# HKUDS/GPT-ST

Hardware: AMD Instinct MI355X
Metric: pretrain steps/sec at (B=32,T=12,N=170,C=64) (higher is better)
Workload: dtype f32; 1 GPU; BASELINE configs[1]: PEMS08-shape synthetic pretrain step, per-GPU B=32 T=12 N=170 C=64 base=1, epoch 200/300 (adaptive mask + KL), fwd+loss+bwd+clip+Adam, hipGraph=True, 4 full optimiser steps on 4 different resident batches per graph replay; global_batch=32, parallelism=dp1

## Files before the change

gpt-st_amd/csrc/abi.hip:

```cpp
#include "common.h"
#include "gptst_hip.h"

extern "C" int gptst_abi_version(void) { return GPTST_ABI_VERSION; }

thread_local int g_deterministic = 0;
extern "C" int gptst_set_deterministic(int on) { g_deterministic = on ? 1 : 0; return GPTST_OK; }
extern "C" int gptst_deterministic_state(void) { return g_deterministic; }

GPTST_INTERNAL int gptst_handoff_lost_capmfma(unsigned* out);
GPTST_INTERNAL int gptst_handoff_lost_hypertem(unsigned* out);
GPTST_INTERNAL int gptst_handoff_lost_masksel(unsigned* out);
extern "C" int gptst_handoff_timeouts(int* out) {
    if (!out) return GPTST_EARG;
    unsigned a = 0u, b = 0u, c = 0u;
    if (gptst_handoff_lost_capmfma(&a) || gptst_handoff_lost_hypertem(&b) || gptst_handoff_lost_masksel(&c)) return -5;
    *out = (int)(a + b + c);
    return GPTST_OK;
}

GPTST_INTERNAL int gptst_handoff_clear_capmfma(unsigned to);
GPTST_INTERNAL int gptst_handoff_clear_hypertem(unsigned to);
GPTST_INTERNAL int gptst_handoff_clear_masksel(unsigned to);
GPTST_INTERNAL int gptst_adam_skipped_clear(void);
extern "C" int gptst_handoff_reset(void) {
    if (hipDeviceSynchronize() != hipSuccess) return -5;
    return (gptst_handoff_clear_capmfma(0u) || gptst_handoff_clear_hypertem(0u) || gptst_handoff_clear_masksel(0u) || gptst_adam_skipped_clear()) ? -5 : GPTST_OK;
}
extern "C" int gptst_handoff_inject(int n) {
    if (n < 0) return GPTST_EARG;
    if (hipDeviceSynchronize() != hipSuccess) return -5;
    return gptst_handoff_clear_capmfma((unsigned)n) ? -5 : GPTST_OK;
}
```

gpt-st_amd/csrc/apply.hip:

```cpp
#include "mfma_tile.h"
#include "wgrad64.h"
#include "kl_guest.h"
#ifdef GPTST_DEBUG
__device__ long long g_ap_ts[64];
static thread_local int g_ap_dbg = 0;
extern "C" int gptst_ap_dbg(int v) { g_ap_dbg = v; return 0; }
extern "C" int gptst_ap_ts(long long* out) { return (int)hipMemcpyFromSymbol(out, HIP_SYMBOL(g_ap_ts), sizeof(long long) * 64); }
#else
static constexpr int g_ap_dbg = 0;
#endif
thread_local int g_apply_tpw = 0;
thread_local int g_apply128_minwg = 768;
thread_local int g_apply128_v1 = 0;

template <int C, int PRO, int EPI>
__global__ __launch_bounds__(256) void apply_kernel(const float* __restrict__ A, const float* __restrict__ A2,
                                                    const float* __restrict__ W, long w_gstride, int transw,
                                                    const float* __restrict__ bias, const float* __restrict__ resid,
                                                    const float* __restrict__ resid2, float* __restrict__ out, float* __restrict__ colsum, RowMap rm, int dbg) {
    using T = Tile<C>;
    int tsi = 0;
#ifdef GPTST_DEBUG
#define TS() do { if (dbg && blockIdx.x == 100 && blockIdx.y == 0 && threadIdx.x == 0) g_ap_ts[tsi] = clock64(); ++tsi; } while (0)
#else
#define TS() do { } while (0)
#endif
    TS();
    extern __shared__ __attribute__((aligned(16))) float smem[];
    float* Wl = smem;
    const int tid = threadIdx.x, lane = tid & 63, wave = tid >> 6;
    float* tile = smem + C * C + wave * T::TILE_FLOATS;
    const int g = blockIdx.x;
    const int ntiles = (rm.M + 31) / 32;
    float cs[C / 64];
#pragma unroll
    for (int u = 0; u < C / 64; ++u) cs[u] = 0.f;
    const int tstride = gridDim.y * 4;
    int t = blockIdx.y * 4 + wave;

    float4 av[T::F4_PER_LANE], ov[T::F4_PER_LANE];
    auto fetch_a = [&](int tt) {
        const int m0 = tt * 32;
#pragma unroll
        for (int it = 0; it < T::F4_PER_LANE; ++it) {
            const int f = it * 64 + lane;
            const int r = f / T::F4_PER_ROW, c4 = f % T::F4_PER_ROW;
            av[it] = f4zero(); ov[it] = make_float4(1.f, 1.f, 1.f, 1.f);
            if (tt < ntiles && m0 + r < rm.M) {
                const size_t off = ((size_t)g * rm.rs_g + (size_t)(m0 + r) * rm.rs_m) * C + 4 * c4;
                av[it] = ld4(A + off);
                if (PRO == PRO_DPRE) ov[it] = ld4(A2 + off);
            }
        }
    };
    fetch_a(t);
    TS();
    load_w_lds<C, 256>(Wl, W + (size_t)g * w_gstride, transw, tid);
    __syncthreads();
    TS();

    for (; t < ntiles; t += tstride) {
        const int m0 = t * 32;
#pragma unroll
        for (int it = 0; it < T::F4_PER_LANE; ++it) {
            const int f = it * 64 + lane;
            const int r = f / T::F4_PER_ROW, c4 = f % T::F4_PER_ROW;
            float4 v = av[it];
            if (PRO == PRO_DPRE) {
                const float4 o = ov[it];
                v.x *= lrelu_grad_from_out(o.x); v.y *= lrelu_grad_from_out(o.y);
                v.z *= lrelu_grad_from_out(o.z); v.w *= lrelu_grad_from_out(o.w);
            }
            st4(tile + r * T::PITCH + 4 * c4, v);
        }
        float4 rv[T::F4_PER_LANE], rv2[T::F4_PER_LANE];
#pragma unroll
        for (int it = 0; it < T::F4_PER_LANE; ++it) {
            const int f = it * 64 + lane;
            const int r = f / T::F4_PER_ROW, c4 = f % T::F4_PER_ROW;
            rv[it] = f4zero(); rv2[it] = f4zero();
            if ((EPI == EPI_RES_LRELU || EPI == EPI_ADD_DPRE) && m0 + r < rm.M) {
                const size_t off = ((size_t)g * rm.rs_g + (size_t)(m0 + r) * rm.rs_m) * C + 4 * c4;
                rv[it] = ld4(resid + off);
                if (EPI == EPI_ADD_DPRE) rv2[it] = ld4(resid2 + off);
            }
        }
        TS();
        if (colsum != nullptr) {
#pragma unroll
            for (int u = 0; u < C / 64; ++u) {
                float s = 0.f;
#pragma unroll 8
                for (int r = 0; r < 32; ++r) s += tile[r * T::PITCH + u * 64 + lane];
                cs[u] += s;
            }
        }
        f32x16 acc[T::NCT];
        TS();
        mfma_tile<C>(tile, Wl, acc, lane);
        TS();
        acc_to_tile<C>(tile, acc, lane);
        TS();
        if (t + tstride < ntiles) fetch_a(t + tstride);
#pragma unroll
        for (int it = 0; it < T::F4_PER_LANE; ++it) {
            const int f = it * 64 + lane;
            const int r = f / T::F4_PER_ROW, c4 = f % T::F4_PER_ROW;
            if (m0 + r < rm.M) {
                const size_t off = ((size_t)g * rm.rs_g + (size_t)(m0 + r) * rm.rs_m) * C + 4 * c4;
                float4 y = ld4(tile + r * T::PITCH + 4 * c4);
                if (bias != nullptr) y = f4add(y, ld4(bias + (size_t)g * C + 4 * c4));
                if (EPI == EPI_RES_LRELU) {
                    y = f4add(y, rv[it]);
                    y.x = lrelu(y.x); y.y = lrelu(y.y); y.z = lrelu(y.z); y.w = lrelu(y.w);
                }
                if (EPI == EPI_LRELU) { y.x = lrelu(y.x); y.y = lrelu(y.y); y.z = lrelu(y.z); y.w = lrelu(y.w); }
                if (EPI == EPI_ADD_DPRE) {
                    const float4 d = rv[it], o = rv2[it];
                    y.x = fmaf(d.x, lrelu_grad_from_out(o.x), y.x); y.y = fmaf(d.y, lrelu_grad_from_out(o.y), y.y);
                    y.z = fmaf(d.z, lrelu_grad_from_out(o.z), y.z); y.w = fmaf(d.w, lrelu_grad_from_out(o.w), y.w);
                }
                st4(out + off, y);
            }
        }
        TS();
    }
    if (colsum != nullptr) {
        __syncthreads();
#pragma unroll
        for (int u = 0; u < C / 64; ++u) tile[u * 64 + lane] = cs[u];
        __syncthreads();
        if (wave == 0) {
#pragma unroll
            for (int u = 0; u < C / 64; ++u) {
                float s = 0.f;
#pragma unroll
                for (int w = 0; w < 4; ++w) s += smem[C * C + w * T::TILE_FLOATS + u * 64 + lane];
                colsum[((size_t)blockIdx.y * rm.G + g) * C + u * 64 + lane] = s;
            }
        }
    }
}

template <int PRO, int EPI>
__global__ __launch_bounds__(256, 2) void apply64_kernel(const float* __restrict__ A, const float* __restrict__ A2,
                                                         const float* __restrict__ W, long w_gstride, int transw,
                                                         const float* __restrict__ bias, const float* __restrict__ resid,
                                                         const float* __restrict__ resid2, float* __restrict__ out,
                                                         float* __restrict__ colsum, RowMap rm, int tiles_per_wave) {
    constexpr int C = 64;
    __shared__ __attribute__((aligned(16))) float Wl[C * C];
    __shared__ __attribute__((aligned(16))) float csl[4][C];
    const int lane = threadIdx.x & 63, wave = threadIdx.x >> 6;
    const int j = lane & 15, kk = lane >> 4;
    const int g = blockIdx.x;
    const int ntiles = (rm.M + 15) / 16;
    const int t0 = (blockIdx.y * 4 + wave) * tiles_per_wave, t1 = min(ntiles, t0 + tiles_per_wave);
    const float* Wg = W + (size_t)g * w_gstride;
    float4 bias4 = f4zero();
    if (bias != nullptr) bias4 = ld4(bias + (size_t)g * C + 4 * j);
    float4 cs[4];
#pragma unroll
    for (int q = 0; q < 4; ++q) cs[q] = f4zero();
    float4 an[4], on[4];
    auto fetch = [&](int t) {
        const int m = min(t * 16 + j, rm.M - 1);
        const size_t off = ((size_t)g * rm.rs_g + (size_t)m * rm.rs_m) * C + 4 * kk;
#pragma unroll
        for (int q = 0; q < 4; ++q) {
            an[q] = ld4(A + off + 16 * q);
            if (PRO == PRO_DPRE) on[q] = ld4(A2 + off + 16 * q);
        }
    };
    if (t0 < t1) fetch(t0);
    load_w_lds<C, 256>(Wl, Wg, transw, threadIdx.x);
    __syncthreads();
    float4 bv[4][4];
#pragma unroll
    for (int q = 0; q < 4; ++q)
#pragma unroll
        for (int e = 0; e < 4; ++e) bv[q][e] = ld4(Wl + (16 * q + 4 * kk + e) * C + 4 * j);
    for (int t = t0; t < t1; ++t) {
        float4 a[4];
        const bool rowok = t * 16 + j < rm.M;
#pragma unroll
        for (int q = 0; q < 4; ++q) {
            float4 v = an[q];
            if (PRO == PRO_DPRE) {
                v.x *= lrelu_grad_from_out(on[q].x); v.y *= lrelu_grad_from_out(on[q].y);
                v.z *= lrelu_grad_from_out(on[q].z); v.w *= lrelu_grad_from_out(on[q].w);
            }
            if (!rowok) v = f4zero();
            a[q] = v;
            cs[q] = f4add(cs[q], v);
        }
        float4 rv[4], rv2[4];
        size_t orow[4];
#pragma unroll
        for (int r = 0; r < 4; ++r) {
            const int m = min(t * 16 + kk * 4 + r, rm.M - 1);
            orow[r] = ((size_t)g * rm.rs_g + (size_t)m * rm.rs_m) * C + 4 * j;
            if (EPI == EPI_RES_LRELU || EPI == EPI_ADD_DPRE) rv[r] = ld4(resid + orow[r]);
            if (EPI == EPI_ADD_DPRE) rv2[r] = ld4(resid2 + orow[r]);
        }
        if (t + 1 < t1) fetch(t + 1);
        SB();
        f32x4 acc[4];
#pragma unroll
        for (int ct = 0; ct < 4; ++ct) acc[ct] = (f32x4){0.f, 0.f, 0.f, 0.f};
#pragma unroll
        for (int q = 0; q < 4; ++q) {
            const float av[4] = {a[q].x, a[q].y, a[q].z, a[q].w};
#pragma unroll
            for (int e = 0; e < 4; ++e) {
                acc[0] = __builtin_amdgcn_mfma_f32_16x16x4f32(av[e], bv[q][e].x, acc[0], 0, 0, 0);
                acc[1] = __builtin_amdgcn_mfma_f32_16x16x4f32(av[e], bv[q][e].y, acc[1], 0, 0, 0);
                acc[2] = __builtin_amdgcn_mfma_f32_16x16x4f32(av[e], bv[q][e].z, acc[2], 0, 0, 0);
                acc[3] = __builtin_amdgcn_mfma_f32_16x16x4f32(av[e], bv[q][e].w, acc[3], 0, 0, 0);
            }
        }
        SB();
#pragma unroll
        for (int r = 0; r < 4; ++r) {
            if (t * 16 + kk * 4 + r < rm.M) {
                float4 y = f4add(make_float4(acc[0][r], acc[1][r], acc[2][r], acc[3][r]), bias4);
                if (EPI == EPI_RES_LRELU) {
                    y = f4add(y, rv[r]);
                    y.x = lrelu(y.x); y.y = lrelu(y.y); y.z = lrelu(y.z); y.w = lrelu(y.w);
                }
                if (EPI == EPI_LRELU) { y.x = lrelu(y.x); y.y = lrelu(y.y); y.z = lrelu(y.z); y.w = lrelu(y.w); }
                if (EPI == EPI_ADD_DPRE) {
                    const float4 d = rv[r], o = rv2[r];
                    y.x = fmaf(d.x, lrelu_grad_from_out(o.x), y.x); y.y = fmaf(d.y, lrelu_grad_from_out(o.y), y.y);
                    y.z = fmaf(d.z, lrelu_grad_from_out(o.z), y.z); y.w = fmaf(d.w, lrelu_grad_from_out(o.w), y.w);
                }
                st4(out + orow[r], y);
            }
        }
    }
    if (colsum != nullptr) {
#pragma unroll
        for (int q = 0; q < 4; ++q) {
            cs[q].x = group_sum<16>(cs[q].x); cs[q].y = group_sum<16>(cs[q].y);
            cs[q].z = group_sum<16>(cs[q].z); cs[q].w = group_sum<16>(cs[q].w);
            if (j == 0) st4(&csl[wave][16 * q + 4 * kk], cs[q]);
        }
        __syncthreads();
        if (wave == 0) colsum[((size_t)blockIdx.y * rm.G + g) * C + lane] = (csl[0][lane] + csl[1][lane]) + (csl[2][lane] + csl[3][lane]);
    }
}

static void apply64_geometry(const RowMap& rm, bool has_colsum, int& tpw, int& gy) {
    const int ntiles = (rm.M + 15) / 16;
    long tot = (long)rm.G * ntiles;
    tpw = (int)((tot + 4 * 512 - 1) / (4 * 512));
    if (tpw > 2) tpw = 2;
    if (has_colsum && rm.G == 1) { const int lim = (ntiles + 4 * 128 - 1) / (4 * 128); if (tpw < lim) tpw = lim; }
    if (g_apply_tpw > 0) tpw = g_apply_tpw;
    if (tpw < 1) tpw = 1;
    gy = (ntiles + 4 * tpw - 1) / (4 * tpw);
}

template <int PRO, int EPI>
static void launch_apply64_t(const float* A, const float* A2, const float* W, long gs, int transw, const float* bias, const float* resid,
                             const float* resid2, float* out, float* colsum, RowMap rm, hipStream_t st) {
    int tpw, gy;
    apply64_geometry(rm, colsum != nullptr, tpw, gy);
    hipLaunchKernelGGL((apply64_kernel<PRO, EPI>), dim3(rm.G, gy), dim3(256), 0, st, A, A2, W, gs, transw, bias, resid, resid2, out, colsum, rm, tpw);
}

static int launch_apply64(const float* A, const float* A2, const float* W, long gs, int transw, const float* bias, const float* resid,
                          const float* resid2, float* out, float* colsum, RowMap rm, int pro, int epi, hipStream_t st) {
    if (pro == PRO_NONE && epi == EPI_PLAIN) launch_apply64_t<PRO_NONE, EPI_PLAIN>(A, A2, W, gs, transw, bias, resid, resid2, out, colsum, rm, st);
    else if (pro == PRO_NONE && epi == EPI_RES_LRELU) launch_apply64_t<PRO_NONE, EPI_RES_LRELU>(A, A2, W, gs, transw, bias, resid, resid2, out, colsum, rm, st);
    else if (pro == PRO_DPRE && epi == EPI_PLAIN) launch_apply64_t<PRO_DPRE, EPI_PLAIN>(A, A2, W, gs, transw, bias, resid, resid2, out, colsum, rm, st);
    else if (pro == PRO_NONE && epi == EPI_ADD_DPRE) launch_apply64_t<PRO_NONE, EPI_ADD_DPRE>(A, A2, W, gs, transw, bias, resid, resid2, out, colsum, rm, st);
    else if (pro == PRO_NONE && epi == EPI_LRELU) launch_apply64_t<PRO_NONE, EPI_LRELU>(A, A2, W, gs, transw, bias, resid, resid2, out, colsum, rm, st);
    else return GPTST_EARG;
    GPTST_CHECK_LAUNCH();
    return GPTST_OK;
}

template <int PRO, int U>
__global__ __launch_bounds__(256, 2) void wgrad64_kernel(const float* __restrict__ A, const float* __restrict__ D,
                                                         const float* __restrict__ D2, float* __restrict__ dW, RowMap rm,
                                                         int rows_per_split, int ostride, int csa) {
    __shared__ __attribute__((aligned(16))) float smem[WGRAD64_SMEM_FLOATS];
    wgrad64_body<PRO, U>(A, D, D2, dW, rm, rows_per_split, ostride, csa, blockIdx.x, blockIdx.y, smem);
}

template <int KIND, int CHAIN>
__global__ __launch_bounds__(256, 2) void applywg64_kernel(const float* __restrict__ dOut, const float* __restrict__ Y,
                                                            const float* __restrict__ S, const float* __restrict__ W, long w_gstride,
                                                            const float* __restrict__ resid, const float* __restrict__ resid2,
                                                            float* __restrict__ dS, float* __restrict__ dW, float* __restrict__ colsum,
                                                            RowMap rm, int tiles_per_wave) {
    __shared__ __attribute__((aligned(16))) float lds[APPLYWG64_LDS_FLOATS];
    applywg64_body<KIND, CHAIN>(dOut, Y, S, W, w_gstride, resid, resid2, dS, dW, colsum, rm, tiles_per_wave, blockIdx.x, blockIdx.y, lds);
}

GPTST_INTERNAL int gptst_apply_wgrad_geometry(int mode, int BT, int N, int* tpw) {
    RowMap rm = make_rowmap(mode, BT, N);
    int gy;
    apply64_geometry(rm, false, *tpw, gy);
    return gy;
}

extern "C" int gptst_apply_wgrad_nsplit(int mode, int BT, int N) {
    RowMap rm = make_rowmap(mode, BT, N);
    int tpw, gy;
    apply64_geometry(rm, false, tpw, gy);
    return gy;
}

extern "C" int gptst_apply_wgrad(const float* dOut, const float* Y, const float* S, const float* W, float* dS, float* dW, float* colsum,
                                 int premul, int mode, int BT, int N, int C, void* stream) {
    if (!dOut || !S || !W || !dS || !dW || BT <= 0 || N <= 0 || mode < 0 || mode > 1 || (Y && premul)) return GPTST_EARG;
    if (C != 64) return GPTST_ESHAPE;
    RowMap rm = make_rowmap(mode, BT, N);
    int tpw, gy;
    apply64_geometry(rm, false, tpw, gy);
    const dim3 grid(rm.G, gy);
    hipStream_t st = (hipStream_t)stream;
    if (Y) hipLaunchKernelGGL((applywg64_kernel<0, 0>), grid, dim3(256), 0, st, dOut, Y, S, W, (long)C * C, nullptr, nullptr, dS, dW, colsum, rm, tpw);
    else if (!premul) hipLaunchKernelGGL((applywg64_kernel<0, 1>), grid, dim3(256), 0, st, dOut, Y, S, W, (long)C * C, nullptr, nullptr, dS, dW, colsum, rm, tpw);
    else hipLaunchKernelGGL((applywg64_kernel<0, 2>), grid, dim3(256), 0, st, dOut, Y, S, W, (long)C * C, nullptr, nullptr, dS, dW, colsum, rm, tpw);
    GPTST_CHECK_LAUNCH();
    return GPTST_OK;
}

extern "C" int gptst_linear_bwd_nsplit(int rows) {
    RowMap rm = make_rowmap(2, rows, 1);
    int tpw, gy;
    apply64_geometry(rm, false, tpw, gy);
    return gy;
}

extern "C" int gptst_linear_bwd(const float* dY, const float* X, const float* Wp, const float* dOut, const float* out, float* dX, float* dWp,
                                float* dbp, int premul, int rows, int C, void* stream) {
    if (!dY || !X || !Wp || !dOut || !dX || !dWp || !dbp || rows <= 0 || (out && premul)) return GPTST_EARG;
    if (C != 64) return GPTST_ESHAPE;
    RowMap rm = make_rowmap(2, rows, 1);
    int tpw, gy;
    apply64_geometry(rm, false, tpw, gy);
    hipStream_t st = (hipStream_t)stream;
    if (out) hipLaunchKernelGGL((applywg64_kernel<1, 0>), dim3(1, gy), dim3(256), 0, st, dY, nullptr, X, Wp, 0L, dOut, out, dX, dWp, dbp, rm, tpw);
    else if (!premul) hipLaunchKernelGGL((applywg64_kernel<1, 1>), dim3(1, gy), dim3(256), 0, st, dY, nullptr, X, Wp, 0L, dOut, nullptr, dX, dWp, dbp, rm, tpw);
    else hipLaunchKernelGGL((applywg64_kernel<1, 2>), dim3(1, gy), dim3(256), 0, st, dY, nullptr, X, Wp, 0L, dOut, X, dX, dWp, dbp, rm, tpw);
    GPTST_CHECK_LAUNCH();
    return GPTST_OK;
}

template <int C, int PRO>
__global__ __launch_bounds__(256) void wgrad_kernel(const float* __restrict__ A, const float* __restrict__ D,
                                                    const float* __restrict__ D2, float* __restrict__ dW,
                                                    RowMap rm, int rows_per_split) {
    constexpr int NCT = C / 32;
    constexpr int TPW = NCT * NCT / 4;
    const int lane = threadIdx.x & 63, wave = threadIdx.x >> 6;
    const int j = lane & 31, h = lane >> 5;
    const int g = blockIdx.x, sp = blockIdx.y;
    const int mbeg = sp * rows_per_split;
    const int mend = min(rm.M, mbeg + rows_per_split);
    const int it = (wave * TPW) / NCT;
    f32x16 acc[TPW];
#pragma unroll
    for (int u = 0; u < TPW; ++u)
#pragma unroll
        for (int r = 0; r < 16; ++r) acc[u][r] = 0.f;

    for (int m = mbeg + h; m < mend + h; m += 2) {
        float a = 0.f;
        float d[TPW];
#pragma unroll
        for (int u = 0; u < TPW; ++u) d[u] = 0.f;
        if (m < mend) {
            const size_t off = ((size_t)g * rm.rs_g + (size_t)m * rm.rs_m) * C;
            a = A[off + it * 32 + j];
#pragma unroll
            for (int u = 0; u < TPW; ++u) {
                const int jt = (wave * TPW + u) % NCT;
                float dv = D[off + jt * 32 + j];
                if (PRO == PRO_DPRE) dv *= lrelu_grad_from_out(D2[off + jt * 32 + j]);
                d[u] = dv;
            }
        }
#pragma unroll
        for (int u = 0; u < TPW; ++u) acc[u] = __builtin_amdgcn_mfma_f32_32x32x2f32(a, d[u], acc[u], 0, 0, 0);
    }
    float* o = dW + ((size_t)sp * rm.G + g) * C * C;
#pragma unroll
    for (int u = 0; u < TPW; ++u) {
        const int jt = (wave * TPW + u) % NCT;
#pragma unroll
        for (int r = 0; r < 16; ++r) {
            const int row = (r & 3) + 8 * (r >> 2) + 4 * h;
            o[(size_t)(it * 32 + row) * C + jt * 32 + j] = acc[u][r];
        }
    }
}

#define AP128_NW 8
// ... 375 lines not shown
```

gpt-st_amd/csrc/hypertem.hip:

```cpp
#include "mfma_tile.h"
#include "wgrad64.h"
#include "kl_guest.h"
GPTST_STAMP_TABLES(hypertem)
GPTST_HANDOFF_COUNTER(hypertem)

#define HT_T 12
#ifndef HT_OCC
#define HT_OCC 2
#endif
#ifdef GPTST_DEBUG
__device__ long long g_ht_ts[64];
static thread_local int g_ht_dbg = 0, g_ht_nt_override = 0;
extern "C" int gptst_ht_dbg(int v) { g_ht_dbg = v; return 0; }
extern "C" int gptst_ht_variant(int fwd, int bwd) { g_ht_nt_override = fwd; (void)bwd; return 0; }
extern "C" int gptst_ht_ts(long long* out) { return (int)hipMemcpyFromSymbol(out, HIP_SYMBOL(g_ht_ts), sizeof(long long) * 64); }
#define HT_DBG(d) (d)
#else
#define HT_DBG(d) 0
static constexpr int g_ht_dbg = 0, g_ht_nt_override = 0;
#endif

__device__ __forceinline__ bool ht_work_at(int L, int ntiles, int B, int& b, int& tile) {
    const int xcd = L & 7, slot = L >> 3;
    b = xcd + 8 * (slot / ntiles);
    tile = slot % ntiles;
    return b < B;
}
__device__ __forceinline__ bool ht_work(int ntiles, int B, int& b, int& tile) { return ht_work_at(blockIdx.x, ntiles, B, b, tile); }

static int ht_pick_nt(int B, int N) {
    if (g_ht_nt_override >= 4 && g_ht_nt_override <= 16) return g_ht_nt_override;
    (void)B; (void)N;
    return 16;
}

__global__ __launch_bounds__(256, HT_OCC) void hypertem_fwd_kernel(const float* __restrict__ X, const float* __restrict__ G,
                                                              const float* __restrict__ Wbt, const float* __restrict__ bbt,
                                                              float* __restrict__ R_out, float* __restrict__ out, int N, int B, int NT,
                                                              int dbg) {
    constexpr int C = 64, P = C + 4, GP = 145;
    int tsi = 0;
#ifdef GPTST_DEBUG
#define TS() do { if ((dbg & 1) && blockIdx.x == 59 && threadIdx.x == 0) g_ht_ts[tsi] = clock64(); ++tsi; } while (0)
#else
#define TS() __builtin_amdgcn_sched_barrier(0)
#endif
    TS();
    extern __shared__ __attribute__((aligned(16))) float smem[];
    float* Xs = smem;
    float* Gs = Xs + HT_T * NT * P;
    int b, tile;
    if (!ht_work((N + NT - 1) / NT, B, b, tile)) return;
    const int n0 = tile * NT;
    const int tid = threadIdx.x, lane = tid & 63, wave = tid >> 6;
    {
        const int nl = tid >> 4, c4 = tid & 15;
        const int n = min(n0 + nl, N - 1);
        float4 v[HT_T];
        float gv[9];
#pragma unroll
        for (int t = 0; t < HT_T; ++t) v[t] = ld4(X + (((size_t)b * HT_T + t) * N + n) * C + 4 * c4);
#pragma unroll
        for (int k = 0; k < 9; ++k) gv[k] = G[min(n0 * 144 + tid + k * 256, N * 144 - 1)];
        if (nl < NT) {
#pragma unroll
            for (int t = 0; t < HT_T; ++t) st4(Xs + (t * NT + nl) * P + 4 * c4, n0 + nl < N ? v[t] : f4zero());
        }
#pragma unroll
        for (int k = 0; k < 9; ++k) {
            const int i = tid + k * 256;
            if (i < NT * 144) Gs[(i / 144) * GP + i % 144] = (n0 + i / 144 < N) ? gv[k] : 0.f;
        }
    }
    __syncthreads();
    TS();
    const int j = lane & 15, kk = lane >> 4;
    const int ja = j < NT ? j : 0;
    float4 bv[C / 16][4];
    float4 b4;
#define HT_LOAD_W(tt) do {                                                                                         \
        const float* W_ = Wbt + ((size_t)b * HT_T + (tt)) * C * C;                                                 \
        _Pragma("unroll") for (int q = 0; q < C / 16; ++q)                                                         \
            _Pragma("unroll") for (int e = 0; e < 4; ++e) bv[q][e] = ld4(W_ + (size_t)(16 * q + 4 * kk + e) * C + 4 * j); \
        b4 = ld4(bbt + ((size_t)b * HT_T + (tt)) * C + 4 * j);                                                     \
    } while (0)
    HT_LOAD_W(wave);
    for (int t = wave; t < HT_T; t += 4) {
        const size_t g = (size_t)b * HT_T + t;
        TS();
        float4 a4[C / 16];
#pragma unroll
        for (int q = 0; q < C / 16; ++q) a4[q] = f4zero();
        {
            const float* gr = Gs + ja * GP + t * HT_T;
            const float* xr = Xs + ja * P + 4 * kk;
#pragma unroll
            for (int u = 0; u < HT_T; ++u) {
                const float gu = gr[u];
#pragma unroll
                for (int q = 0; q < C / 16; ++q) a4[q] = f4fma(gu, ld4(xr + u * NT * P + 16 * q), a4[q]);
            }
        }
        TS();
        f32x4 acc[C / 16];
#pragma unroll
        for (int ct = 0; ct < C / 16; ++ct) acc[ct] = (f32x4){0.f, 0.f, 0.f, 0.f};
#pragma unroll
        for (int q = 0; q < C / 16; ++q) {
            const float av[4] = {a4[q].x, a4[q].y, a4[q].z, a4[q].w};
#pragma unroll
            for (int e = 0; e < 4; ++e) {
                acc[0] = __builtin_amdgcn_mfma_f32_16x16x4f32(av[e], bv[q][e].x, acc[0], 0, 0, 0);
                acc[1] = __builtin_amdgcn_mfma_f32_16x16x4f32(av[e], bv[q][e].y, acc[1], 0, 0, 0);
                acc[2] = __builtin_amdgcn_mfma_f32_16x16x4f32(av[e], bv[q][e].z, acc[2], 0, 0, 0);
                acc[3] = __builtin_amdgcn_mfma_f32_16x16x4f32(av[e], bv[q][e].w, acc[3], 0, 0, 0);
            }
        }
        TS();
        const float4 bias = b4;
        if (t + 4 < HT_T) HT_LOAD_W(t + 4);
        TS();
        if (R_out != nullptr && j < NT && n0 + j < N) {
#pragma unroll
            for (int q = 0; q < C / 16; ++q) st4_far(R_out + (g * N + n0 + j) * C + 16 * q + 4 * kk, a4[q]);
        }
#pragma unroll
        for (int r = 0; r < 4; ++r) {
            const int nl = kk * 4 + r;
            if (nl < NT && n0 + nl < N) {
                float4 y = f4add(f4add(make_float4(acc[0][r], acc[1][r], acc[2][r], acc[3][r]), bias), ld4(Xs + (t * NT + nl) * P + 4 * j));
                y.x = lrelu(y.x); y.y = lrelu(y.y); y.z = lrelu(y.z); y.w = lrelu(y.w);
                st4(out + (g * N + n0 + nl) * C + 4 * j, y);
            }
        }
        TS();
    }
}

static size_t ht_smem(int NT) { return ((size_t)HT_T * NT * 68 + NT * 145) * sizeof(float); }

extern "C" int gptst_hypertem_fwd(const float* X, const float* G, const float* Wbt, const float* bbt, float* R_out, float* out, int B,
                                  int T, int N, int C, void* stream) {
    if (!X || !G || !Wbt || !bbt || !out || T != HT_T) return GPTST_EARG;
    if (C != 64) return GPTST_ESHAPE;
    static int done = 0;
    if (!done) { hipFuncSetAttribute((const void*)hypertem_fwd_kernel, hipFuncAttributeMaxDynamicSharedMemorySize, (int)ht_smem(16)); done = 1; }
    const int NT = ht_pick_nt(B, N);
    hipLaunchKernelGGL(hypertem_fwd_kernel, dim3(8 * ((B + 7) / 8) * ((N + NT - 1) / NT)), dim3(256), ht_smem(NT), (hipStream_t)stream, X, G, Wbt, bbt, R_out, out, N, B, NT, g_ht_dbg);
    GPTST_CHECK_LAUNCH();
    return GPTST_OK;
}

template <bool HASY, bool PREMUL, int PAIR>
__device__ __forceinline__ void hypertem_bwd_stage(const float* __restrict__ dOut, const float* __restrict__ Y,
                                                   const float* __restrict__ X, const float* __restrict__ G,
                                                   const float* __restrict__ Wbt, float* __restrict__ dX,
                                                   float* __restrict__ dbias, float* __restrict__ dG, int N, int B, int dbg, int b, int tile,
// ... 248 lines not shown
    extern __shared__ __attribute__((aligned(16))) float smem[];
    if ((int)blockIdx.x < nH) {
        hypertem_bwd_body<HASY, PREMUL>(dOut, Y, X, G, Wbt, dX, nullptr, dG, N, B, 0, blockIdx.x, smem);
    } else if (MIX) {
        int b, t;
        if (!ht_work_at(blockIdx.x - nH, HT_T, B, b, t)) return;
        wgrad64_mix_body<HASY>(X, G, dOut, Y, dWb, N, b, t, smem);
    } else {
        const int w = blockIdx.x - nH;
        wgrad64_body<HASY ? PRO_DPRE : PRO_NONE, U>(R, dOut, Y, dWb, rm, rows_per_split, 64 * 64 + 64, 2, w % rm.G, w / rm.G, smem);
    }
}

extern "C" int gptst_hypertem_ntiles(int N) { return (N + 15) / 16; }

extern "C" int gptst_hypertem_bwd(const float* dOut, const float* Y, const float* X, const float* G, const float* Wbt, float* dX,
                                  float* dbias, float* dG, int premul, int B, int T, int N, int C, void* stream) {
    if (!dOut || !X || !G || !Wbt || !dX || !dG || T != HT_T || (Y && premul)) return GPTST_EARG;
    if (C != 64) return GPTST_ESHAPE;
    const size_t smem = ht_smem(16);
    static int done = 0;
    if (!done) {
        hipFuncSetAttribute((const void*)hypertem_bwd_kernel<true, false>, hipFuncAttributeMaxDynamicSharedMemorySize, (int)smem);
        hipFuncSetAttribute((const void*)hypertem_bwd_kernel<false, false>, hipFuncAttributeMaxDynamicSharedMemorySize, (int)smem);
        hipFuncSetAttribute((const void*)hypertem_bwd_kernel<false, true>, hipFuncAttributeMaxDynamicSharedMemorySize, (int)smem);
        done = 1;
    }
    const dim3 grid(8 * ((B + 7) / 8) * ((N + 15) / 16));
    if (Y) hipLaunchKernelGGL((hypertem_bwd_kernel<true, false>), grid, dim3(256), smem, (hipStream_t)stream, dOut, Y, X, G, Wbt, dX, dbias, dG, N, B, g_ht_dbg);
    else if (premul) hipLaunchKernelGGL((hypertem_bwd_kernel<false, true>), grid, dim3(256), smem, (hipStream_t)stream, dOut, Y, X, G, Wbt, dX, dbias, dG, N, B, g_ht_dbg);
    else hipLaunchKernelGGL((hypertem_bwd_kernel<false, false>), grid, dim3(256), smem, (hipStream_t)stream, dOut, Y, X, G, Wbt, dX, dbias, dG, N, B, g_ht_dbg);
    GPTST_CHECK_LAUNCH();
    return GPTST_OK;
}

extern "C" int gptst_wgrad_nsplit(int mode, int BT, int N, int C);
template <bool HASY, bool PREMUL>
static void ht_bwd_wgrad_launch(const float* dOut, const float* Y, const float* X, const float* G, const float* Wbt, const float* R, float* dX,
                                float* dG, float* dWb, int B, int N, bool u6, int nH, int nW, RowMap rm, int rps, size_t smem, hipStream_t st) {
    static int done = 0;
    if (!done) {
        hipFuncSetAttribute((const void*)hypertem_bwd_wgrad_kernel<4, HASY, PREMUL, false>, hipFuncAttributeMaxDynamicSharedMemorySize, (int)smem);
        hipFuncSetAttribute((const void*)hypertem_bwd_wgrad_kernel<6, HASY, PREMUL, false>, hipFuncAttributeMaxDynamicSharedMemorySize, (int)smem);
        hipFuncSetAttribute((const void*)hypertem_bwd_wgrad_kernel<4, HASY, PREMUL, true>, hipFuncAttributeMaxDynamicSharedMemorySize, (int)smem);
        done = 1;
    }
    if (R == nullptr) hipLaunchKernelGGL((hypertem_bwd_wgrad_kernel<4, HASY, PREMUL, true>), dim3(nH + 8 * ((B + 7) / 8) * HT_T), dim3(256), smem, st, dOut, Y, X, G, Wbt, R, dX, dG, dWb, N, B, nH, rm, rps);
    else if (u6) hipLaunchKernelGGL((hypertem_bwd_wgrad_kernel<6, HASY, PREMUL, false>), dim3(nH + nW), dim3(256), smem, st, dOut, Y, X, G, Wbt, R, dX, dG, dWb, N, B, nH, rm, rps);
    else hipLaunchKernelGGL((hypertem_bwd_wgrad_kernel<4, HASY, PREMUL, false>), dim3(nH + nW), dim3(256), smem, st, dOut, Y, X, G, Wbt, R, dX, dG, dWb, N, B, nH, rm, rps);
}

extern "C" int gptst_hypertem_bwd_wgrad(const float* dOut, const float* Y, const float* X, const float* G, const float* Wbt, const float* R,
                                        float* dX, float* dG, float* dWb, int premul, int B, int T, int N, int C, void* stream) {
    if (!dOut || !X || !G || !Wbt || !dX || !dG || !dWb || T != HT_T || (Y && premul)) return GPTST_EARG;
    if (C != 64) return GPTST_ESHAPE;
    const size_t smem_h = ht_smem(16), smem_w = WGRAD64_SMEM_FLOATS * sizeof(float), smem = smem_h > smem_w ? smem_h : smem_w;
    const RowMap rm = make_rowmap(0, B * T, N);
    const int ns = gptst_wgrad_nsplit(0, B * T, N, 64);
    if (!R && ns != 1) return GPTST_ESHAPE;
    int rps = (rm.M + ns - 1) / ns;
    rps = (rps + 1) & ~1;
    const int rows = rps < rm.M ? rps : rm.M, steps = ((rows + 3) / 4 + 3) / 4;
    const bool u6 = (steps + 5) / 6 * 6 <= (steps + 3) / 4 * 4;
    const int nH = 8 * ((B + 7) / 8) * ((N + 15) / 16), nW = rm.G * ns;
    if (Y) ht_bwd_wgrad_launch<true, false>(dOut, Y, X, G, Wbt, R, dX, dG, dWb, B, N, u6, nH, nW, rm, rps, smem, (hipStream_t)stream);
    else if (premul) ht_bwd_wgrad_launch<false, true>(dOut, Y, X, G, Wbt, R, dX, dG, dWb, B, N, u6, nH, nW, rm, rps, smem, (hipStream_t)stream);
    else ht_bwd_wgrad_launch<false, false>(dOut, Y, X, G, Wbt, R, dX, dG, dWb, B, N, u6, nH, nW, rm, rps, smem, (hipStream_t)stream);
    GPTST_CHECK_LAUNCH();
    return GPTST_OK;
}

struct HtPairArgs {
    const float* dOut1; const float* X1; const float* G1; const float* Wbt1; const float* R1;
    const float* X0; const float* G0; const float* Wbt0; const float* R0;
    float* dXmid; float* dX0; float* dG1; float* dG0; float* dWb1; float* dWb0; unsigned* cnt;
};

template <int U>
__global__ __launch_bounds__(256, HT_OCC) void hypertem_bwd_pair_kernel(HtPairArgs a, int N, int B, int nH, RowMap rm, int rows_per_split) {
    extern __shared__ __attribute__((aligned(16))) float smem[];
    const int ntiles = (N + 15) / 16;
    if ((int)blockIdx.x < nH) {
        int b, tile;
        if (!ht_work_at(blockIdx.x, ntiles, B, b, tile)) return;
        float4 dp[HT_T];
        GPTST_WG_BEGIN(); GPTST_STAMP(0);
        hypertem_bwd_stage<false, true, 1>(a.dOut1, nullptr, a.X1, a.G1, a.Wbt1, a.dXmid, nullptr, a.dG1, N, B, 0, b, tile, smem, dp);
        asm volatile("s_waitcnt vmcnt(0)" ::: "memory");
        __syncthreads();
        if (threadIdx.x == 0) { gptst_publish_fence(); __hip_atomic_fetch_add(a.cnt + b, 1u, __ATOMIC_RELAXED, __HIP_MEMORY_SCOPE_AGENT); }
        GPTST_STAMP(5);
        hypertem_bwd_stage<false, true, 2>(nullptr, nullptr, a.X0, a.G0, a.Wbt0, a.dX0, nullptr, a.dG0, N, B, 0, b, tile, smem, dp);
        GPTST_WG_END();
        return;
    }
    GPTST_WG_BEGIN();
    const int nW = rm.G * ((rm.M + rows_per_split - 1) / rows_per_split);
    int w = blockIdx.x - nH;
    if (w < nW) {
        wgrad64_body<PRO_NONE, U>(a.R1, a.dOut1, nullptr, a.dWb1, rm, rows_per_split, 64 * 64 + 64, 2, w % rm.G, w / rm.G, smem);
        GPTST_WG_END();
        return;
    }
    w -= nW;
    const int g = w % rm.G, sp = w / rm.G;
    unsigned* s_ok = reinterpret_cast<unsigned*>(smem);
    if (threadIdx.x == 0) *s_ok = gptst_wait_ge(a.cnt + g / HT_T, (unsigned)ntiles, &g_handoff_lost_hypertem) ? 1u : 0u;
    __syncthreads();
    const bool ok = *s_ok != 0u;
    __syncthreads();
    wgrad64_body<PRO_NONE, U, true>(a.R0, a.dXmid, nullptr, a.dWb0, rm, rows_per_split, 64 * 64 + 64, 2, g, sp, smem);
    if (!ok) a.dWb0[((size_t)sp * rm.G + g) * (size_t)(64 * 64 + 64) + threadIdx.x] = __int_as_float(0x7fc00000);
    GPTST_WG_END();
}

extern "C" int gptst_hypertem_bwd_pair(const float* dOut1, const float* X1, const float* G1, const float* Wbt1, const float* R1, const float* X0,
                                       const float* G0, const float* Wbt0, const float* R0, float* dXmid, float* dX0, float* dG1, float* dG0,
                                       float* dWb1, float* dWb0, void* cnt, int B, int T, int N, int C, void* stream) {
    if (!dOut1 || !X1 || !G1 || !Wbt1 || !R1 || !X0 || !G0 || !Wbt0 || !R0 || !dXmid || !dX0 || !dG1 || !dG0 || !dWb1 || !dWb0 || !cnt || T != HT_T)
        return GPTST_EARG;
    if (C != 64 || (size_t)HT_T * N * C * 4 >= ((size_t)1 << 31)) return GPTST_ESHAPE;
    const size_t smem_h = ht_smem(16), smem_w = WGRAD64_SMEM_FLOATS * sizeof(float), smem = smem_h > smem_w ? smem_h : smem_w;
    const RowMap rm = make_rowmap(0, B * T, N);
    const int ns = gptst_wgrad_nsplit(0, B * T, N, 64);
    int rps = (rm.M + ns - 1) / ns;
    rps = (rps + 1) & ~1;
    if ((rm.M + rps - 1) / rps != ns || (size_t)B * T * N * C * 4 >= ((size_t)1 << 31)) return GPTST_ESHAPE;
    const int rows = rps < rm.M ? rps : rm.M, steps = ((rows + 3) / 4 + 3) / 4;
    const bool u6 = (steps + 5) / 6 * 6 <= (steps + 3) / 4 * 4;
    const int nH = 8 * ((B + 7) / 8) * ((N + 15) / 16), nW = rm.G * ns;
    static int done = 0;
    if (!done) {
        hipFuncSetAttribute((const void*)hypertem_bwd_pair_kernel<4>, hipFuncAttributeMaxDynamicSharedMemorySize, (int)smem);
        hipFuncSetAttribute((const void*)hypertem_bwd_pair_kernel<6>, hipFuncAttributeMaxDynamicSharedMemorySize, (int)smem);
        done = 1;
    }
    const HtPairArgs a{dOut1, X1, G1, Wbt1, R1, X0, G0, Wbt0, R0, dXmid, dX0, dG1, dG0, dWb1, dWb0, (unsigned*)cnt};
    if (u6) hipLaunchKernelGGL((hypertem_bwd_pair_kernel<6>), dim3(nH + 2 * nW), dim3(256), smem, (hipStream_t)stream, a, N, B, nH, rm, rps);
    else hipLaunchKernelGGL((hypertem_bwd_pair_kernel<4>), dim3(nH + 2 * nW), dim3(256), smem, (hipStream_t)stream, a, N, B, nH, rm, rps);
    GPTST_CHECK_LAUNCH();
    return GPTST_OK;
}

struct HtStage { const float* G; const float* Wbt; const float* bbt; float* R_out; float* out; };
struct HtChain {
    int nstage;
    const float* X;
    HtStage st[3];
};

#ifndef HTC_NW
#define HTC_NW 4
#endif
template <int NSTAGE, int GUEST>
__global__ __launch_bounds__(64 * HTC_NW, HTC_NW == 6 ? 3 : HT_OCC) void hypertem_chain_fwd_kernel(HtChain ch, int N, int B, KlGuest kg) {
    constexpr int C = 64, P = C + 4, GP = 145, NT = 16, NW = HTC_NW, NTH = 64 * NW, TPW = HT_T / NW;
    static_assert(HT_T % NW == 0 && (HT_T * NT * (C / 4)) % NTH == 0 && (NT * 144) % NTH == 0, "waves must divide the steps and the staging loops");
    constexpr int GK = NT * 144 / NTH, XK = HT_T * NT * (C / 4) / NTH;
    extern __shared__ __attribute__((aligned(16))) float smem[];
    float* Xs = smem;
    float* Gs = Xs + HT_T * NT * P;
    if constexpr (GUEST != 0) {
        static_assert(NTH == 256, "the guest bodies are written for 256 threads");
        if ((int)blockIdx.x >= kg.base) { kl_guest_run<GUEST>(kg, kg.v0 + (int)blockIdx.x - kg.base, smem); return; }
    }
    int b, tile;
    if (!ht_work((N + NT - 1) / NT, B, b, tile)) return;
    const int n0 = tile * NT;
    const int tid = threadIdx.x, lane = tid & 63, wave = tid >> 6;
    const int j = lane & 15, kk = lane >> 4;
    float gv[GK];
#define HTC_LOAD_G(Gp) _Pragma("unroll") for (int k = 0; k < GK; ++k) gv[k] = (Gp)[min(n0 * 144 + tid + k * NTH, N * 144 - 1)]
#define HTC_STORE_G() _Pragma("unroll") for (int k = 0; k < GK; ++k) { const int i = tid + k * NTH; \
        Gs[(i / 144) * GP + i % 144] = (n0 + i / 144 < N) ? gv[k] : 0.f; }
    float4 bv[C / 16][4];
    float4 b4;
#define HTC_LOAD_W(W0, b0, tt) do {                                                                                \
        const float* W_ = (W0) + ((size_t)b * HT_T + (tt)) * C * C;                                                \
        _Pragma("unroll") for (int q = 0; q < C / 16; ++q)                                                         \
            _Pragma("unroll") for (int e = 0; e < 4; ++e) bv[q][e] = ld4(W_ + (size_t)(16 * q + 4 * kk + e) * C + 4 * j); \
        b4 = ld4((b0) + ((size_t)b * HT_T + (tt)) * C + 4 * j);                                                    \
    } while (0)

    {
        float4 v[XK];
#pragma unroll
        for (int k = 0; k < XK; ++k) {
            const int i = tid + k * NTH, t = i >> 8, nl = (i & 255) >> 4, c4 = i & 15;
            v[k] = ld4(ch.X + (((size_t)b * HT_T + t) * N + min(n0 + nl, N - 1)) * C + 4 * c4);
        }
        HTC_LOAD_G(ch.st[0].G);
#pragma unroll
        for (int k = 0; k < XK; ++k) {
            const int i = tid + k * NTH, t = i >> 8, nl = (i & 255) >> 4, c4 = i & 15;
            st4(Xs + (t * NT + nl) * P + 4 * c4, n0 + nl < N ? v[k] : f4zero());
        }
        HTC_STORE_G();
    }
    __syncthreads();
    SB();

#pragma unroll
    for (int s = 0; s < NSTAGE; ++s) {
        const HtStage S = ch.st[s];
        const HtStage S1 = ch.st[s + 1 < 3 ? s + 1 : 2];
        if (s + 1 < NSTAGE) {
            float4 a4a[C / 16], a4b[C / 16], a4c[C / 16];
#pragma unroll
            for (int q = 0; q < C / 16; ++q) { a4a[q] = f4zero(); a4b[q] = f4zero(); a4c[q] = f4zero(); }
            {
                const float* gr = Gs + j * GP + wave * HT_T;
                const float* xr = Xs + j * P + 4 * kk;
#pragma unroll
                for (int u = 0; u < HT_T; ++u) {
                    float4 x[C / 16];
#pragma unroll
                    for (int q = 0; q < C / 16; ++q) x[q] = ld4(xr + u * NT * P + 16 * q);
                    const float g0 = gr[u], g1 = gr[NW * HT_T + u], g2 = TPW == 3 ? gr[2 * NW * HT_T + u] : 0.f;
#pragma unroll
                    for (int q = 0; q < C / 16; ++q) {
                        a4a[q] = f4fma(g0, x[q], a4a[q]);
                        a4b[q] = f4fma(g1, x[q], a4b[q]);
                        if (TPW == 3) a4c[q] = f4fma(g2, x[q], a4c[q]);
                    }
                    if (TPW == 3 ? u % 3 == 2 : u % 2 == 1) SB();
                }
            }
            HTC_LOAD_W(S.Wbt, S.bbt, wave);
            HTC_LOAD_G(S1.G);
            __syncthreads();
            SB();
#pragma nounroll
            for (int ti = 0; ti < TPW; ++ti) {
                const int t = wave + NW * ti;
                const size_t g = (size_t)b * HT_T + t;
                float4 m4[C / 16];
#pragma unroll
                for (int q = 0; q < C / 16; ++q) { m4[q] = a4a[q]; a4a[q] = a4b[q]; a4b[q] = a4c[q]; }
                f32x4 acc[C / 16];
#pragma unroll
                for (int ct = 0; ct < C / 16; ++ct) acc[ct] = (f32x4){0.f, 0.f, 0.f, 0.f};
#pragma unroll
                for (int q = 0; q < C / 16; ++q) {
                    const float av[4] = {m4[q].x, m4[q].y, m4[q].z, m4[q].w};
#pragma unroll
                    for (int e = 0; e < 4; ++e) {
                        acc[0] = __builtin_amdgcn_mfma_f32_16x16x4f32(av[e], bv[q][e].x, acc[0], 0, 0, 0);
                        acc[1] = __builtin_amdgcn_mfma_f32_16x16x4f32(av[e], bv[q][e].y, acc[1], 0, 0, 0);
                        acc[2] = __builtin_amdgcn_mfma_f32_16x16x4f32(av[e], bv[q][e].z, acc[2], 0, 0, 0);
                        acc[3] = __builtin_amdgcn_mfma_f32_16x16x4f32(av[e], bv[q][e].w, acc[3], 0, 0, 0);
                    }
                }
                SB();
                const float4 bias = b4;
                if (ti < TPW - 1) HTC_LOAD_W(S.Wbt, S.bbt, t + NW);
                SB();
                if (S.R_out != nullptr && n0 + j < N) {
#pragma unroll
                    for (int q = 0; q < C / 16; ++q) st4_far(S.R_out + (g * N + n0 + j) * C + 16 * q + 4 * kk, m4[q]);
                }
#pragma unroll
                for (int r = 0; r < 4; ++r) {
                    const int nl = kk * 4 + r;
                    float* xs = Xs + (t * NT + nl) * P + 4 * j;
                    float4 y = f4add(f4add(make_float4(acc[0][r], acc[1][r], acc[2][r], acc[3][r]), bias), ld4(xs));
                    y.x = lrelu(y.x); y.y = lrelu(y.y); y.z = lrelu(y.z); y.w = lrelu(y.w);
                    if (n0 + nl < N) st4(S.out + (g * N + n0 + nl) * C + 4 * j, y);
                    else y = f4zero();
                    st4(xs, y);
                }
                SB();
            }
            HTC_STORE_G();
            __syncthreads();
            SB();
        } else {
            HTC_LOAD_W(S.Wbt, S.bbt, wave);
            for (int t = wave; t < HT_T; t += NW) {
                const size_t g = (size_t)b * HT_T + t;
                SB();
                float4 a4[C / 16];
#pragma unroll
                for (int q = 0; q < C / 16; ++q) a4[q] = f4zero();
                {
                    const float* gr = Gs + j * GP + t * HT_T;
                    const float* xr = Xs + j * P + 4 * kk;
#pragma unroll
                    for (int u = 0; u < HT_T; ++u) {
                        const float gu = gr[u];
#pragma unroll
                        for (int q = 0; q < C / 16; ++q) a4[q] = f4fma(gu, ld4(xr + u * NT * P + 16 * q), a4[q]);
                    }
                }
                SB();
                f32x4 acc[C / 16];
#pragma unroll
                for (int ct = 0; ct < C / 16; ++ct) acc[ct] = (f32x4){0.f, 0.f, 0.f, 0.f};
#pragma unroll
                for (int q = 0; q < C / 16; ++q) {
                    const float av[4] = {a4[q].x, a4[q].y, a4[q].z, a4[q].w};
#pragma unroll
                    for (int e = 0; e < 4; ++e) {
                        acc[0] = __builtin_amdgcn_mfma_f32_16x16x4f32(av[e], bv[q][e].x, acc[0], 0, 0, 0);
                        acc[1] = __builtin_amdgcn_mfma_f32_16x16x4f32(av[e], bv[q][e].y, acc[1], 0, 0, 0);
                        acc[2] = __builtin_amdgcn_mfma_f32_16x16x4f32(av[e], bv[q][e].z, acc[2], 0, 0, 0);
                        acc[3] = __builtin_amdgcn_mfma_f32_16x16x4f32(av[e], bv[q][e].w, acc[3], 0, 0, 0);
                    }
                }
                SB();
                const float4 bias = b4;
                if (t + NW < HT_T) HTC_LOAD_W(S.Wbt, S.bbt, t + NW);
                SB();
                if (S.R_out != nullptr && n0 + j < N) {
#pragma unroll
                    for (int q = 0; q < C / 16; ++q) st4_far(S.R_out + (g * N + n0 + j) * C + 16 * q + 4 * kk, a4[q]);
                }
#pragma unroll
                for (int r = 0; r < 4; ++r) {
                    const int nl = kk * 4 + r;
                    if (n0 + nl < N) {
                        float4 y = f4add(f4add(make_float4(acc[0][r], acc[1][r], acc[2][r], acc[3][r]), bias), ld4(Xs + (t * NT + nl) * P + 4 * j));
                        y.x = lrelu(y.x); y.y = lrelu(y.y); y.z = lrelu(y.z); y.w = lrelu(y.w);
                        st4(S.out + (g * N + n0 + nl) * C + 4 * j, y);
                    }
                }
            }
        }
    }
#undef HTC_LOAD_G
#undef HTC_STORE_G
#undef HTC_LOAD_W
}

static int ht_chain_args(HtChain& ch, const float* X, int nstage, const void* Gs, const void* Wbts, const void* bbts, const void* Rs, const void* outs,
                         int B, int T, int N, int C) {
    if (!X || nstage < 1 || nstage > 3 || !Gs || !Wbts || !bbts || !Rs || !outs || T != HT_T || B <= 0 || N <= 0) return GPTST_EARG;
    if (C != 64) return GPTST_ESHAPE;
    ch.nstage = nstage; ch.X = X;
    for (int s = 0; s < 3; ++s) {
        const int k = s < nstage ? s : nstage - 1;
        ch.st[s] = HtStage{((const float* const*)Gs)[k], ((const float* const*)Wbts)[k], ((const float* const*)bbts)[k],
                           ((float* const*)Rs)[k], ((float* const*)outs)[k]};
        if (!ch.st[s].G || !ch.st[s].Wbt || !ch.st[s].bbt || !ch.st[s].out) return GPTST_EARG;
    }
    return GPTST_OK;
}

static int ht_chain_grid(int B, int N) { return 8 * ((B + 7) / 8) * ((N + 15) / 16); }

extern "C" int gptst_hypertem_chain_fwd(const float* X, int nstage, const void* Gs, const void* Wbts, const void* bbts, const void* Rs,
                                        const void* outs, int B, int T, int N, int C, void* stream) {
    HtChain ch;
    const int rc = ht_chain_args(ch, X, nstage, Gs, Wbts, bbts, Rs, outs, B, T, N, C);
    if (rc != GPTST_OK) return rc;
    const dim3 grid(ht_chain_grid(B, N));
    const int smem = (int)ht_smem(16);
    hipStream_t st = (hipStream_t)stream;
    const KlGuest none{};
#define HTC_LAUNCH(NS_) do {                                                                                                          \
        static int done_ = 0;                                                                                                          \
        if (!done_) { (void)hipFuncSetAttribute((const void*)hypertem_chain_fwd_kernel<NS_, 0>, hipFuncAttributeMaxDynamicSharedMemorySize, smem); done_ = 1; } \
        hipLaunchKernelGGL((hypertem_chain_fwd_kernel<NS_, 0>), grid, dim3(64 * HTC_NW), smem, st, ch, N, B, none);                          \
    } while (0)
    if (nstage == 1) HTC_LAUNCH(1); else if (nstage == 2) HTC_LAUNCH(2); else HTC_LAUNCH(3);
#undef HTC_LAUNCH
    GPTST_CHECK_LAUNCH();
    return GPTST_OK;
}

GPTST_INTERNAL int gptst_tail_geometry(int rows, int* rows_per_block);
GPTST_INTERNAL int gptst_apply_wgrad_geometry(int mode, int BT, int N, int* tpw);

extern "C" int gptst_kl_guest_blocks(int stage, int B, int T, int N) {
    if (B <= 0 || T <= 0 || N <= 0) return GPTST_EARG;
    int aux;
    if (stage == 1) return gptst_tail_geometry(B * T * N, &aux);
    if (stage == 2) return B * T * gptst_apply_wgrad_geometry(0, B * T, N, &aux);
    if (stage == 3) return N;
    return GPTST_EARG;
}

extern "C" int gptst_hypertem_chain_fwd_kl(const float* X, int nstage, const void* Gs, const void* Wbts, const void* bbts, const void* Rs,
                                           const void* outs, int B, int T, int N, int C, int stage, const void* ops, int v0, int v1, int HS,
                                           int lda, float w, void* stream) {
    HtChain ch;
    const int rc = ht_chain_args(ch, X, nstage, Gs, Wbts, bbts, Rs, outs, B, T, N, C);
    if (rc != GPTST_OK) return rc;
    if (!ops || stage < 1 || stage > 3) return GPTST_EARG;
    if (nstage != 2 || HTC_NW != 4 || HS <= 0 || HS > TL_MAXJ) return GPTST_ESHAPE;
    const int nv = gptst_kl_guest_blocks(stage, B, T, N);
    if (v0 < 0 || v1 <= v0 || v1 > nv) return GPTST_EARG;
    const float* const* p = (const float* const*)ops;
    const int np = stage == 1 ? 7 : stage == 2 ? 6 : 7;
    for (int i = 0; i < np; ++i) if (!p[i]) return GPTST_EARG;
    KlGuest kg{};
    kg.base = ht_chain_grid(B, N);
    kg.v0 = v0;
    if (stage == 1) {
        TailArgs& t = kg.tail;
        t.X = p[0]; t.W = p[1]; t.prob = p[2]; t.c = p[3]; t.dX = (float*)p[4]; t.part = (float*)p[5]; t.sws = (float*)p[6];
        t.rows = B * T * N; t.J = HS; t.N = N; t.w = w; t.premul = 1;
        gptst_tail_geometry(t.rows, &t.rows_per_block);
    } else if (stage == 2) {
        kg.dOut = p[0]; kg.S = p[1]; kg.W = p[2]; kg.dS = (float*)p[3]; kg.dW = (float*)p[4]; kg.colsum = (float*)p[5];
        kg.rm = make_rowmap(0, B * T, N);
        gptst_apply_wgrad_geometry(0, B * T, N, &kg.tpw);
    } else {
        if (lda <= 0) return GPTST_EARG;
        kg.dPre = p[0]; kg.src = p[1]; kg.lda = lda; kg.w1 = p[2]; kg.b1 = p[3]; kg.Wn = p[4]; kg.dWb = (float*)p[5]; kg.dinp = (float*)p[6];
        kg.BT = B * T; kg.N = N;
    }
    const dim3 grid(kg.base + (v1 - v0));
    const size_t sg = kl_guest_lds_bytes(stage), sh = ht_smem(16);
    const int smem = (int)(sg > sh ? sg : sh);
    hipStream_t st = (hipStream_t)stream;
#define HTC_LAUNCH(G_) do {                                                                                                           \
        static int done_ = 0;                                                                                                          \
        if (!done_) { (void)hipFuncSetAttribute((const void*)hypertem_chain_fwd_kernel<2, G_>, hipFuncAttributeMaxDynamicSharedMemorySize, smem); done_ = 1; } \
        hipLaunchKernelGGL((hypertem_chain_fwd_kernel<2, G_>), grid, dim3(64 * HTC_NW), smem, st, ch, N, B, kg);                           \
    } while (0)
    if (stage == 1) HTC_LAUNCH(1); else if (stage == 2) HTC_LAUNCH(2); else HTC_LAUNCH(3);
#undef HTC_LAUNCH
    GPTST_CHECK_LAUNCH();
    return GPTST_OK;
}
```

gpt-st_amd/csrc/loss_adam.hip:

```cpp
#include "common.h"

__global__ __launch_bounds__(256) void mae_fwd_kernel(const float* __restrict__ out, const float* __restrict__ src, int lda,
                                                      const float* __restrict__ mask, float sigma, float mu, float thresh, int rows,
                                                      int J, float* __restrict__ stats) {
    __shared__ float red[2][4];
    float ls = 0.f, cnt = 0.f;
    for (size_t e = (size_t)blockIdx.x * 256 + threadIdx.x; e < (size_t)rows * J; e += (size_t)gridDim.x * 256) {
        const size_t i = e / J; const int j = (int)(e % J);
        const float M = 1.f - mask[e];
        const float p = inverse_transform(out[e], sigma, mu) * M;
        const float y = inverse_transform(src[i * lda + j], sigma, mu) * M;
        if (y > thresh) { ls += fabsf(y - p); cnt += 1.f; }
    }
    ls = group_sum<64>(ls); cnt = group_sum<64>(cnt);
    if ((threadIdx.x & 63) == 0) { red[0][threadIdx.x >> 6] = ls; red[1][threadIdx.x >> 6] = cnt; }
    __syncthreads();
    if (threadIdx.x == 0) {
        atomicAdd(stats + 0, red[0][0] + red[0][1] + red[0][2] + red[0][3]);
        atomicAdd(stats + 1, red[1][0] + red[1][1] + red[1][2] + red[1][3]);
    }
}

__global__ __launch_bounds__(256) void mae_bwd_kernel(const float* __restrict__ out, const float* __restrict__ src, int lda,
                                                      const float* __restrict__ mask, float sigma, float mu, float thresh, int rows,
                                                      int J, const float* __restrict__ stats, int normalize, float* __restrict__ dOut) {
    const float inv = normalize ? 1.f / fmaxf(stats[1], 1.f) : 1.f;
    for (size_t e = (size_t)blockIdx.x * 256 + threadIdx.x; e < (size_t)rows * J; e += (size_t)gridDim.x * 256) {
        const size_t i = e / J; const int j = (int)(e % J);
        const float M = 1.f - mask[e];
        const float p = inverse_transform(out[e], sigma, mu) * M;
        const float y = inverse_transform(src[i * lda + j], sigma, mu) * M;
        float g = 0.f;
        if (y > thresh) {
            const float d = p - y;
            g = (d > 0.f ? 1.f : (d < 0.f ? -1.f : 0.f)) * M * sigma * inv;
        }
        dOut[e] = g;
    }
}

__global__ __launch_bounds__(256) void kl_kernel(const float* __restrict__ prob, const float* __restrict__ c, int rows, int N, int HS,
                                                 float w, float* __restrict__ dlogit, float* __restrict__ stats) {
    __shared__ float red[4];
    float kl = 0.f;
    for (size_t i = (size_t)blockIdx.x * 256 + threadIdx.x; i < (size_t)rows; i += (size_t)gridDim.x * 256) {
        const size_t bt = i / N, n = i % N;
        const float* cp = c + bt * HS * N + n;
        float se = 0.f;
        for (int h = 0; h < HS; ++h) {
            const float e = cp[(size_t)h * N], p = prob[i * HS + h];
            se += e;
            if (e > 0.f) kl += e * (logf(e) - logf(p));
        }
        if (dlogit != nullptr)
            for (int h = 0; h < HS; ++h) dlogit[i * HS + h] = w * (prob[i * HS + h] * se - cp[(size_t)h * N]);
    }
    kl = group_sum<64>(kl);
    if ((threadIdx.x & 63) == 0) red[threadIdx.x >> 6] = kl;
    __syncthreads();
    if (threadIdx.x == 0) atomicAdd(stats + 2, red[0] + red[1] + red[2] + red[3]);
}

__device__ __forceinline__ float seg_scale(const float* hyper, const float* stats, bool segA) {
    if (segA) return hyper[9] != 0.f ? 1.f / fmaxf(stats[1], 1.f) : 1.f;
    return hyper[10];
}

#define GN_NB 256

__global__ __launch_bounds__(256) void gradnorm_kernel(const float* __restrict__ g, long nA, long nB, const float* __restrict__ hyper,
                                                       float* __restrict__ stats, float* __restrict__ ws, const float* __restrict__ sws,
                                                       int sws_rows) {
    __shared__ float red[2][4];
    __shared__ float reds[3][4];
    const bool actB = hyper[8] != 0.f;
    const long n4 = (nA + (actB ? nB : 0)) / 4, nA4 = nA / 4;
    const long stride = (long)gridDim.x * 256;
    float sA = 0.f, sB = 0.f;
    for (long i0 = (long)blockIdx.x * 256 + threadIdx.x; i0 < n4; i0 += 4 * stride) {
        float4 v[4];
#pragma unroll
        for (int u = 0; u < 4; ++u) {
            const long i = i0 + u * stride;
            v[u] = i < n4 ? ld4(g + 4 * i) : f4zero();
        }
#pragma unroll
        for (int u = 0; u < 4; ++u) {
            const float q = fmaf(v[u].x, v[u].x, fmaf(v[u].y, v[u].y, fmaf(v[u].z, v[u].z, v[u].w * v[u].w)));
            if ((i0 + u * stride) < nA4) sA += q; else sB += q;
        }
    }
    sA = group_sum<64>(sA); sB = group_sum<64>(sB);
    if ((threadIdx.x & 63) == 0) { red[0][threadIdx.x >> 6] = sA; red[1][threadIdx.x >> 6] = sB; }
    __syncthreads();
    if (threadIdx.x < 2) ws[2 * blockIdx.x + threadIdx.x] = (red[threadIdx.x][0] + red[threadIdx.x][1]) + (red[threadIdx.x][2] + red[threadIdx.x][3]);
    if (sws != nullptr && blockIdx.x == 0) {
        float s[3] = {0.f, 0.f, 0.f};
        for (int r = threadIdx.x; r < sws_rows; r += 256) {
            const float4 v = ld4(sws + 4 * (size_t)r);
            s[0] += v.x; s[1] += v.y; s[2] += v.z;
        }
#pragma unroll
        for (int k = 0; k < 3; ++k) {
            s[k] = group_sum<64>(s[k]);
            if ((threadIdx.x & 63) == 0) reds[k][threadIdx.x >> 6] = s[k];
        }
        __syncthreads();
        if (threadIdx.x < 3) stats[threadIdx.x] += (reds[threadIdx.x][0] + reds[threadIdx.x][1]) + (reds[threadIdx.x][2] + reds[threadIdx.x][3]);
    }
}

__device__ unsigned g_adam_skipped = 0u;
GPTST_INTERNAL int gptst_adam_skipped_clear(void) {
    const unsigned z = 0u;
    return hipMemcpyToSymbol(HIP_SYMBOL(g_adam_skipped), &z, sizeof(unsigned)) == hipSuccess ? 0 : 1;
}

__global__ __launch_bounds__(256) void adam_kernel(float* __restrict__ p, const float* __restrict__ g, float* __restrict__ m,
                                                   float* __restrict__ v, long nA, long nB, const float* __restrict__ hyper,
                                                   float* __restrict__ stats, const float* __restrict__ ws, int nws, float* __restrict__ stats_out,
                                                   const unsigned* __restrict__ lost0, const unsigned* __restrict__ lost1, const unsigned* __restrict__ lost2) {
    __shared__ float red[4];
    __shared__ float redB[4];
    const unsigned nlost = (lost0 != nullptr ? *lost0 : 0u) + (lost1 != nullptr ? *lost1 : 0u) + (lost2 != nullptr ? *lost2 : 0u) +
                           ((lost0 != nullptr && stats[5] > 0.f) ? (unsigned)stats[5] : 0u);
    {
        float sA = (int)threadIdx.x < nws ? ws[2 * threadIdx.x] : 0.f, sB = (int)threadIdx.x < nws ? ws[2 * threadIdx.x + 1] : 0.f;
        sA = group_sum<64>(sA); sB = group_sum<64>(sB);
        if ((threadIdx.x & 63) == 0) { red[threadIdx.x >> 6] = sA; redB[threadIdx.x >> 6] = sB; }
        __syncthreads();
    }
    const float ua = seg_scale(hyper, stats, true), ub = seg_scale(hyper, stats, false);
    const float gsq = hyper[13] != 0.f ? stats[3]
                    : stats[3] + (ua * ua * ((red[0] + red[1]) + (red[2] + red[3])) + ub * ub * ((redB[0] + redB[1]) + (redB[2] + redB[3])));
    const bool actB = hyper[8] != 0.f;
    const long n = nA + (actB ? nB : 0);
    const float b1 = hyper[4], b2 = hyper[5], eps = hyper[6], maxn = hyper[7];
    const float omb1 = hyper[11] != 0.f ? hyper[11] : 1.f - b1, omb2 = hyper[12] != 0.f ? hyper[12] : 1.f - b2;
    float clip = 1.f;
    if (maxn > 0.f) clip = fminf(1.f, maxn / (sqrtf(gsq) + 1e-6f));
    const float sa = seg_scale(hyper, stats, true) * clip, sb = seg_scale(hyper, stats, false) * clip;
    for (long i = 4 * ((long)blockIdx.x * 256 + threadIdx.x); i < n && nlost == 0u; i += 4 * (long)gridDim.x * 256) {
        const bool A = i < nA;
        const float sc = A ? sa : sb, step = A ? hyper[0] : hyper[2], bc2 = A ? hyper[1] : hyper[3];
        const float4 g4 = ld4(g + i), p4 = ld4(p + i);
        float4 m4 = ld4(m + i), v4 = ld4(v + i);
        const float gv[4] = {g4.x, g4.y, g4.z, g4.w}, pv[4] = {p4.x, p4.y, p4.z, p4.w};
        float mv[4] = {m4.x, m4.y, m4.z, m4.w}, vv[4] = {v4.x, v4.y, v4.z, v4.w}, po[4];
#pragma unroll
        for (int e = 0; e < 4; ++e) {
            const float gr = gv[e] * sc;
            float mi = mv[e], vi = vv[e];
            mi = mi + (gr - mi) * omb1;
            vi = vi * b2 + omb2 * gr * gr;
            const float denom = sqrtf(vi) / bc2 + eps;
            po[e] = pv[e] - step * (mi / denom);
            mv[e] = mi; vv[e] = vi;
        }
        st4(p + i, make_float4(po[0], po[1], po[2], po[3]));
        st4(m + i, make_float4(mv[0], mv[1], mv[2], mv[3]));
        st4(v + i, make_float4(vv[0], vv[1], vv[2], vv[3]));
    }
    if (blockIdx.x == 0 && threadIdx.x == 0) stats[4] = gsq;
    if (blockIdx.x == 0) {
        __shared__ unsigned s_skipped;
        if (threadIdx.x == 0) s_skipped = nlost != 0u ? (g_adam_skipped += 1u) : g_adam_skipped;
        __syncthreads();
        if (stats_out != nullptr && threadIdx.x < 8)
            stats_out[threadIdx.x] = threadIdx.x == 4 ? gsq : threadIdx.x == 5 ? (float)nlost : threadIdx.x == 6 ? (float)s_skipped : stats[threadIdx.x];
    }
}

extern "C" int gptst_mae_fwd(const float* out, const float* src, int lda, const float* mask, float sigma, float mu, float thresh,
                             int rows, int J, float* stats, void* stream) {
    if (!out || !src || !mask || !stats) return GPTST_EARG;
    int nb = (int)(((size_t)rows * J + 255) / 256); if (nb > 64) nb = 64;
    hipLaunchKernelGGL(mae_fwd_kernel, dim3(nb), dim3(256), 0, (hipStream_t)stream, out, src, lda, mask, sigma, mu, thresh, rows, J, stats);
    GPTST_CHECK_LAUNCH();
    return GPTST_OK;
}

extern "C" int gptst_mae_bwd(const float* out, const float* src, int lda, const float* mask, float sigma, float mu, float thresh,
                             int rows, int J, const float* stats, int normalize, float* dOut, void* stream) {
    if (!out || !src || !mask || !stats || !dOut) return GPTST_EARG;
    int nb = (int)(((size_t)rows * J + 255) / 256); if (nb > 1024) nb = 1024;
    hipLaunchKernelGGL(mae_bwd_kernel, dim3(nb), dim3(256), 0, (hipStream_t)stream, out, src, lda, mask, sigma, mu, thresh, rows, J, stats,
                       normalize, dOut);
    GPTST_CHECK_LAUNCH();
    return GPTST_OK;
}

extern "C" int gptst_kl(const float* prob, const float* c, int rows, int N, int HS, float w, float* dlogit, float* stats, void* stream) {
    if (!prob || !c || !stats) return GPTST_EARG;
    int nb = (rows + 255) / 256;
    hipLaunchKernelGGL(kl_kernel, dim3(nb), dim3(256), 0, (hipStream_t)stream, prob, c, rows, N, HS, w, dlogit, stats);
    GPTST_CHECK_LAUNCH();
    return GPTST_OK;
}

extern "C" int gptst_clip_adam_ws_floats(void) { return 2 * GN_NB; }

GPTST_INTERNAL const unsigned* gptst_handoff_word_capmfma(void);
GPTST_INTERNAL const unsigned* gptst_handoff_word_hypertem(void);
GPTST_INTERNAL const unsigned* gptst_handoff_word_masksel(void);
static int g_handoff_guard = 1;
extern "C" int gptst_set_handoff_guard(int on) { g_handoff_guard = on ? 1 : 0; return GPTST_OK; }

extern "C" int gptst_clip_adam(float* p, const float* g, float* m, float* v, long nA, long nB, const float* hyper, float* stats,
                               float* ws, float* stats_out, const float* sws, int sws_rows, void* stream) {
    if (!p || !g || !m || !v || !hyper || !stats || !ws || (sws && sws_rows <= 0)) return GPTST_EARG;
    if ((nA & 3) || (nB & 3) || (((uintptr_t)p | (uintptr_t)g | (uintptr_t)m | (uintptr_t)v) & 15)) return GPTST_EARG;
    long n = nA + nB;
    int nb = (int)((n / 4 + 255) / 256); if (nb > 1024) nb = 1024; if (nb < 1) nb = 1;
    const int nbn = nb > GN_NB ? GN_NB : nb;
    hipLaunchKernelGGL(gradnorm_kernel, dim3(nbn), dim3(256), 0, (hipStream_t)stream, g, nA, nB, hyper, stats, ws, sws, sws_rows);
    static const unsigned* w0 = gptst_handoff_word_capmfma();
    static const unsigned* w1 = gptst_handoff_word_hypertem();
    static const unsigned* w2 = gptst_handoff_word_masksel();
    hipLaunchKernelGGL(adam_kernel, dim3(nb), dim3(256), 0, (hipStream_t)stream, p, g, m, v, nA, nB, hyper, stats, (const float*)ws, nbn, stats_out,
                       g_handoff_guard ? w0 : nullptr, g_handoff_guard ? w1 : nullptr, g_handoff_guard ? w2 : nullptr);
    GPTST_CHECK_LAUNCH();
    return GPTST_OK;
}
```

gpt-st_amd/csrc/tails.hip:

```cpp
#include "kl_guest.h"

#define TL_NB 512

template <int KIND, int C>
__global__ __launch_bounds__(256) void tail_kernel(TailArgs t) {
    constexpr int LPR = C / 4, RPB = 256 / LPR;
    __shared__ __attribute__((aligned(16))) float Ws[TL_MAXJ * C];
    __shared__ float4 red[RPB][LPR];
    __shared__ float redb[RPB];
    __shared__ float reds[3][4];
    const int J = t.J;
    for (int i = threadIdx.x; i < J * C / 4; i += 256) st4(Ws + 4 * i, ld4(t.W + 4 * i));
    __syncthreads();
    const int c4 = threadIdx.x % LPR, slot = threadIdx.x / LPR;
    const size_t r0 = (size_t)blockIdx.x * t.rows_per_block;
    const size_t r1 = min((size_t)t.rows, r0 + t.rows_per_block);
    float4 accW[TL_MAXJ];
    float accb[TL_MAXJ];
#pragma unroll
    for (int j = 0; j < TL_MAXJ; ++j) { accW[j] = f4zero(); accb[j] = 0.f; }
    float s0 = 0.f, s1 = 0.f;
    constexpr int UR = 4;
    for (size_t i0 = r0 + slot; i0 < r1; i0 += UR * RPB) {
      float4 xs[UR];
#pragma unroll
      for (int u = 0; u < UR; ++u) { const size_t i = i0 + (size_t)u * RPB; xs[u] = i < r1 ? ld4(t.X + i * C + 4 * c4) : f4zero(); }
      SB();
#pragma unroll
      for (int u = 0; u < UR; ++u) {
        const size_t i = i0 + (size_t)u * RPB;
        if (i >= r1) continue;
        const float4 x = xs[u];
        float a[TL_MAXJ];
        float a_own = 0.f;
        const int gl = (threadIdx.x & 63) & ~(LPR - 1);
        if (KIND == 0) {
            float o_all[TL_MAXJ];
#pragma unroll
            for (int j = 0; j < TL_MAXJ; ++j) {
                o_all[j] = 0.f;
                if (j < J) o_all[j] = group_sum<LPR>(f4dot(x, ld4(Ws + j * C + 4 * c4)));
            }
            float o = 0.f;
#pragma unroll
            for (int j = 0; j < TL_MAXJ; ++j) if (j == c4) o = o_all[j];
            if (c4 < J) {
                o += t.b ? t.b[c4] : 0.f;
                const size_t e = i * J + c4;
                const float M = 1.f - t.mask[e];
                const float p = inverse_transform(o, t.sigma, t.mu) * M;
                const float y = inverse_transform(t.src[i * t.lda + c4], t.sigma, t.mu) * M;
                if (y > t.thresh) {
                    const float d = p - y;
                    s0 += fabsf(d); s1 += 1.f;
                    a_own = (d > 0.f ? 1.f : (d < 0.f ? -1.f : 0.f)) * M * t.sigma;
                }
                t.out[e] = o;
            }
        } else {
            const size_t bt = i / t.N, n = i % t.N;
            float e_ = 0.f, p_ = 1.f;
            if (c4 < J) { e_ = t.c[(bt * J + c4) * t.N + n]; p_ = t.prob[i * J + c4]; }
            const float se = group_sum<LPR>(e_);
            if (c4 < J && e_ > 0.f) s0 += e_ * (logf(e_) - logf(p_));
            a_own = c4 < J ? t.w * (p_ * se - e_) : 0.f;
        }
#pragma unroll
        for (int j = 0; j < TL_MAXJ; ++j) a[j] = j < J ? __shfl(a_own, gl + j, 64) : 0.f;
        float4 dx = f4zero();
#pragma unroll
        for (int j = 0; j < TL_MAXJ; ++j)
            if (j < J) {
                dx = f4fma(a[j], ld4(Ws + j * C + 4 * c4), dx);
                accW[j] = f4fma(a[j], x, accW[j]);
                accb[j] += a[j];
            }
        if (t.premul) {
            dx.x *= lrelu_grad_from_out(x.x); dx.y *= lrelu_grad_from_out(x.y); dx.z *= lrelu_grad_from_out(x.z); dx.w *= lrelu_grad_from_out(x.w);
        }
        st4(t.dX + i * C + 4 * c4, dx);
      }
    }
    float* mine = t.part + (size_t)blockIdx.x * (J * C + J);
#pragma unroll
    for (int j = 0; j < TL_MAXJ; ++j) {
        if (j >= J) continue;
        red[slot][c4] = accW[j];
        if (c4 == 0) redb[slot] = accb[j];
        __syncthreads();
        if (slot == 0) {
            float4 s = red[0][c4];
            for (int q = 1; q < RPB; ++q) s = f4add(s, red[q][c4]);
            st4(mine + j * C + 4 * c4, s);
            if (c4 == 0) {
                float sb = redb[0];
                for (int q = 1; q < RPB; ++q) sb += redb[q];
                mine[J * C + j] = sb;
            }
        }
        __syncthreads();
    }
    s0 = group_sum<64>(s0); s1 = group_sum<64>(s1);
    if ((threadIdx.x & 63) == 0) { reds[0][threadIdx.x >> 6] = s0; reds[1][threadIdx.x >> 6] = s1; }
    __syncthreads();
    if (threadIdx.x == 0) {
        float* w = t.sws + 4 * (size_t)blockIdx.x;
        const float v0 = (reds[0][0] + reds[0][1]) + (reds[0][2] + reds[0][3]), v1 = (reds[1][0] + reds[1][1]) + (reds[1][2] + reds[1][3]);
        if (KIND == 0) { w[0] = v0; w[1] = v1; } else { w[2] = v0; }
    }
}

template <int KIND, int C>
__global__ __launch_bounds__(256) void tail_mfma_kernel(TailArgs t) {
    __shared__ __attribute__((aligned(16))) float lds[tail_mfma_lds_floats<C>()];
    tail_mfma_body<KIND, C>(t, blockIdx.x, lds);
}

__global__ __launch_bounds__(256) void stats_fold_kernel(const float* __restrict__ sws, int rows, float* __restrict__ stats,
                                                         const unsigned* __restrict__ lost0, const unsigned* __restrict__ lost1,
                                                         const unsigned* __restrict__ lost2) {
    __shared__ float red[3][4];
    if (threadIdx.x == 255) stats[5] = (float)((lost0 != nullptr ? *lost0 : 0u) + (lost1 != nullptr ? *lost1 : 0u) + (lost2 != nullptr ? *lost2 : 0u));
    float s[3] = {0.f, 0.f, 0.f};
    for (int r = threadIdx.x; r < rows; r += 256) {
        const float4 v = ld4(sws + 4 * (size_t)r);
        s[0] += v.x; s[1] += v.y; s[2] += v.z;
    }
#pragma unroll
    for (int k = 0; k < 3; ++k) {
        s[k] = group_sum<64>(s[k]);
        if ((threadIdx.x & 63) == 0) red[k][threadIdx.x >> 6] = s[k];
    }
    __syncthreads();
    if (threadIdx.x < 3) stats[threadIdx.x] += (red[threadIdx.x][0] + red[threadIdx.x][1]) + (red[threadIdx.x][2] + red[threadIdx.x][3]);
}

thread_local int g_tl_nb = TL_NB;
thread_local int g_tl_mfma = 1;
static void tl_geometry(int rows, int& nb, int& rpb) {
    int want = g_tl_nb;
    if (g_tl_nb == TL_NB && rows > TL_NB * 512) { want = rows / 512; if (want > 4096) want = 4096; }
    rpb = (rows + want - 1) / want; if (rpb < 16) rpb = 16;
    nb = (rows + rpb - 1) / rpb;
}

extern "C" int gptst_tail_parts(int rows) { int nb, rpb; tl_geometry(rows, nb, rpb); return nb; }
GPTST_INTERNAL int gptst_tail_geometry(int rows, int* rows_per_block) { int nb; tl_geometry(rows, nb, *rows_per_block); return nb; }

GPTST_INTERNAL const unsigned* gptst_handoff_word_capmfma(void);
GPTST_INTERNAL const unsigned* gptst_handoff_word_hypertem(void);
GPTST_INTERNAL const unsigned* gptst_handoff_word_masksel(void);
extern "C" int gptst_stats_fold(const float* sws, int rows, float* stats, void* stream) {
    if (!sws || !stats || rows <= 0) return GPTST_EARG;
    static const unsigned* w0 = gptst_handoff_word_capmfma();
    static const unsigned* w1 = gptst_handoff_word_hypertem();
    static const unsigned* w2 = gptst_handoff_word_masksel();
    hipLaunchKernelGGL(stats_fold_kernel, dim3(1), dim3(256), 0, (hipStream_t)stream, sws, rows, stats, w0, w1, w2);
    GPTST_CHECK_LAUNCH();
    return GPTST_OK;
}

extern "C" int gptst_tail_mae(const float* dec, const float* W, const float* b, const float* src, int lda, const float* mask, float sigma,
                              float mu, float thresh, float* out, float* d_dec, float* part, float* sws, int premul, int rows, int J, int C,
                              void* stream) {
    if (!dec || !W || !src || !mask || !out || !d_dec || !part || !sws || rows <= 0 || J <= 0) return GPTST_EARG;
    if ((C != 64 && C != 128) || J > TL_MAXJ) return GPTST_ESHAPE;
    TailArgs t{};
    t.X = dec; t.W = W; t.b = b; t.dX = d_dec; t.part = part; t.sws = sws; t.rows = rows; t.J = J;
    t.src = src; t.mask = mask; t.out = out; t.lda = lda; t.sigma = sigma; t.mu = mu; t.thresh = thresh; t.premul = premul;
    int nb; tl_geometry(rows, nb, t.rows_per_block);
    if (C == 64 && g_tl_mfma) hipLaunchKernelGGL((tail_mfma_kernel<0, 64>), dim3(nb), dim3(256), 0, (hipStream_t)stream, t);
    else if (C == 64) hipLaunchKernelGGL((tail_kernel<0, 64>), dim3(nb), dim3(256), 0, (hipStream_t)stream, t);
    else if (g_tl_mfma) hipLaunchKernelGGL((tail_mfma_kernel<0, 128>), dim3(nb), dim3(256), 0, (hipStream_t)stream, t);
    else hipLaunchKernelGGL((tail_kernel<0, 128>), dim3(nb), dim3(256), 0, (hipStream_t)stream, t);
    GPTST_CHECK_LAUNCH();
    return GPTST_OK;
}

extern "C" int gptst_tail_kl(const float* h2, const float* W3, const float* prob, const float* c, float w, float* d_h2, float* part,
                             float* sws, int premul, int rows, int N, int HS, int C, void* stream) {
    if (!h2 || !W3 || !prob || !c || !d_h2 || !part || !sws || rows <= 0 || HS <= 0 || N <= 0) return GPTST_EARG;
    if ((C != 64 && C != 128) || HS > TL_MAXJ) return GPTST_ESHAPE;
    TailArgs t{};
    t.X = h2; t.W = W3; t.dX = d_h2; t.part = part; t.sws = sws; t.rows = rows; t.J = HS;
    t.prob = prob; t.c = c; t.N = N; t.w = w; t.premul = premul;
    int nb; tl_geometry(rows, nb, t.rows_per_block);
    if (C == 64 && g_tl_mfma) hipLaunchKernelGGL((tail_mfma_kernel<1, 64>), dim3(nb), dim3(256), 0, (hipStream_t)stream, t);
    else if (C == 64) hipLaunchKernelGGL((tail_kernel<1, 64>), dim3(nb), dim3(256), 0, (hipStream_t)stream, t);
    else if (g_tl_mfma) hipLaunchKernelGGL((tail_mfma_kernel<1, 128>), dim3(nb), dim3(256), 0, (hipStream_t)stream, t);
    else hipLaunchKernelGGL((tail_kernel<1, 128>), dim3(nb), dim3(256), 0, (hipStream_t)stream, t);
    GPTST_CHECK_LAUNCH();
    return GPTST_OK;
}
```

gpt-st_amd/engine.py:

```python
import contextlib
import gc
import os
import threading
from typing import Any, NamedTuple

import torch

from . import _C, ops
from .ops import (EPI_ADD_DPRE, EPI_ADD_PREMUL, EPI_LRELU, EPI_PREMUL, EPI_PLAIN, EPI_RES_LRELU, MODE_NODE, MODE_SHARED, MODE_TIME, PRO_DPRE, PRO_NONE)

TF_NAMES = ("ln_day", "ln_week", "ln1", "ln2", "ln")


class ZeroArena:

    def __init__(self, device):
        self.device, self.buf, self.off, self.need = device, None, 0, 0

    def begin(self, zero=True):
        pending = None
        if self.buf is None or self.buf.numel() < self.need:
            self.buf = torch.zeros(max(self.need, 1), device=self.device) if self.need else None
        elif self.buf is not None:
            if zero:
# ... 213 lines not shown
    v = lambda a: a.view(B, T, N, C)
    assert not chain or chain_ok(dims)
    if _ht_fused_bwd(dims):
        dx, dWb, ns, _ = ops.hypertem_bwd_wgrad(v(dout), None if chain else v(out), v(x), G, Wbt, v(R) if R is not None else None, dG=dG_out,
                                                premul=chain and premul)
        return dx.view(-1, C), _wb_parts(dWb, C, ns)
    hp = _wgrad_parts(R, dout, None if chain else out, MODE_TIME, dims)
    if C == 64:
        dx, _, _ = ops.hypertem_bwd(v(dout), v(out), v(x), G, Wbt, dG=dG_out, want_dbias=False)
    elif chain:
        dR = ops.apply(dout, Wbt, MODE_TIME, BT, N, transw=True)
        dx, _ = ops.tmix_bwd_chain(v(dR), v(x), G, v(dout), premul=premul, dG=dG_out[0])
    else:
        dR = ops.apply(dout, Wbt, MODE_TIME, BT, N, A2=out, transw=True, pro=PRO_DPRE)
        dx, _ = ops.tmix_bwd(v(dR), v(x), G, v(dout), v(out), dG=dG_out[0])
    return dx.view(-1, C), hp


CARRY_RED = os.environ.get("GPTST_CARRY_RED", "1") == "1"
CARRY_MB = float(os.environ.get("GPTST_CARRY_MB", "25"))
CARRY_KL = os.environ.get("GPTST_CARRY_KL", "1") == "1"
TAIL_ROLES = os.environ.get("GPTST_TAIL_ROLES", "1") == "1"
PAIR_UNDER_DP = os.environ.get("GPTST_PAIR_UNDER_DP", "1") == "1"
PAIR_BWD = os.environ.get("GPTST_PAIR_BWD", "1") == "1"


@contextlib.contextmanager
def no_handoffs():
    from . import _C
    keep = (CTX.NO_HANDOFFS, _C.lib().value("gptst_mask_cooperative_state"))
    CTX.NO_HANDOFFS = True
    _C.lib().call("gptst_mask_cooperative", 0)
    try:
        yield
    finally:
        CTX.NO_HANDOFFS = keep[0]
        _C.lib().call("gptst_mask_cooperative", keep[1])


def pair_bwd_on():
    return PAIR_BWD and not CTX.NO_HANDOFFS


def cross_role():
    return 0 if CTX.NO_HANDOFFS else CROSS_ROLE


TAIL_MAX_WG = 512


def tail_roles_ok(red, dims, sv_e):
    B, T, N, C = dims
    return bool(TAIL_ROLES and red.want_tail and CARRY_RED and not red.no_carry and red.on_bucket is None and CTX.NODE_REDUCE is None
                and cross_role() and FUSE_CROSS and CAP_LIN and C == 64 and T == 12 and sv_e is not None and isinstance(sv_e.h1, EncIn)
                and B * T + 4 * B <= TAIL_MAX_WG)


def _ht_pair_shape_ok(dims):
    B, T, N, C = dims
    if T != 12 or C != 64:
        return False
    ns = ops.wgrad_nsplit(MODE_TIME, B * T, N, C)
    rps = (-(-N // ns) + 1) & ~1
    return -(-N // rps) == ns


def ht_pair_ok(saved1, saved0, dims):
    return (pair_bwd_on() and dims[3] == 64 and not isinstance(saved1, EncIn) and saved1.R is not None and saved0.R is not None
            and _ht_fused_bwd(dims) and _ht_pair_shape_ok(dims))


class PendingH1:

    def __init__(self, saved, dd, dG, dWb):
        self.saved, self.dd, self.dG, self.dWb = saved, dd, dG, dWb


def ht_pair_bwd(saved1, saved0, dout, dG1, dG0, dims, dWb1=None):
    B, T, N, C = dims
    if not ht_pair_ok(saved1, saved0, dims):
        assert dWb1 is None
        return None
    s1, s0 = saved1, saved0
    v = lambda a: a.view(B, T, N, C)
    r = ops.hypertem_bwd_pair(v(dout), v(s1.x), s1.G, s1.Wbt, v(s1.R), v(s0.x), s0.G, s0.Wbt, v(s0.R), dG1, dG0, _zeros(dout, B), dWb1=dWb1)
    assert r is not None or dWb1 is None
    if r is None:
        return None
    dmid, dx0, dWb1, dWb0, ns = r
    return dx0.view(-1, C), _wb_parts(dWb1, C, ns), _wb_parts(dWb0, C, ns)


FUSE_CROSS = os.environ.get("GPTST_FUSE_CROSS", "1") == "1"
CAP_LIN = os.environ.get("GPTST_CAP_LIN", "1") == "1"
CROSS_ROLE = int(os.environ.get("GPTST_CROSS_ROLE", "1"))


class CapSaved(NamedTuple):
    x: Any
    out: Any
    rec: Any
    c: Any
    s: Any
    v: Any
    Ht: Any
    Rt: Any
    dyn: Any
    Wn: Any
    Y: Any


class CapParts(NamedTuple):
    wn: WgradParts
    ddyn: Any
    dlogit: Any


def cap_head_fwd(p, pfx, x, dadj, dyn, dims, num_route, HS, HT):
    B, T, N, C = dims
    c, s, Y = ops.cap_route_fwd(x.view(B, T, N, C), p[pfx + "ln_p.weight"], p[pfx + "ln_p.bias"], dadj, HS, num_route,
                                reduce_nodes=CTX.NODE_REDUCE, want_Y=True)
    fused = ops.cap_cross_rec_fwd(s, dyn, p[pfx + "mask_template"], c, B, T, N, HS, HT) if (FUSE_CROSS and CTX.NODE_REDUCE is None) else None
    if fused is not None:
        v, Ht, Rt, rec = fused
    else:
        v, Ht, Rt = ops.cap_cross_fwd(s, dyn, p[pfx + "mask_template"], B, T, HS, HT)
        rec = ops.cap_rec_fwd(c, v, N, C)
    return rec, c, (s, v, Ht, Rt, Y)


def cap_core_fwd(p, pfx, x, dadj, dyn, Wn, bn, dims, num_route, HS, HT):
    B, T, N, C = dims
    rec, c, (s, v, Ht, Rt, Y) = cap_head_fwd(p, pfx, x, dadj, dyn, dims, num_route, HS, HT)
    out = ops.apply(rec, Wn, MODE_NODE, B * T, N, bias=bn, resid=x, epi=EPI_RES_LRELU)
    return out, c, CapSaved(x, out, rec, c, s, v, Ht, Rt, dyn, Wn, Y)


CHAIN_FWD = os.environ.get("GPTST_CHAIN_FWD", "1") == "1"


def chain_fwd_ok(dims):
    return CHAIN_FWD and dims[3] == 64 and not DROP_R


def ht_chain_fwd(x, stages, dims, kl=None):
    B, T, N, C = dims
    res = ops.hypertem_chain_fwd(x.view(B, T, N, C), stages, guest=kl.guest() if kl is not None else None)
    saved, xin = [], x
    for (G, Wbt, _b), (R, o) in zip(stages, res):
        o = o.view(-1, C)
        saved.append(HtSaved(xin, R.view(-1, C), o, G, Wbt))
        xin = o
    return saved, xin


def cap_core_bwd(p, g, pfx, saved, dout, dims, HS, HT, red, chain=False):
    B, T, N, C = dims
    x, out, rec, c, s, v, Ht, Rt, dyn, Wn, Y = saved
    BT, dev = B * T, x.device
    assert not chain or chain_ok(dims)
    drec, wn = _genlin_bwd(dout, out, rec, Wn, MODE_NODE, dims, chain)
    dc1, dv = ops.cap_rec_bwd(drec, c, v, reduce_nodes=CTX.NODE_REDUCE)
    gw, gb = g[pfx + "ln_p.weight"], g[pfx + "ln_p.bias"]
    if FUSE_CROSS and CAP_LIN and C == 64 and CTX.NODE_REDUCE is None and Y is None:
        carry = red.take_carry(CARRY_MB) if cross_role() and _C.lib().value("gptst_cap_route_roles_ok", B, T, N, C, HS, HT) == 1 else None
        lin = ops.cap_cross_route_lin_bwd(x.view(B, T, N, C), p[pfx + "ln_p.weight"], p[pfx + "ln_p.bias"], c, dc1, dv, s, Rt, Ht, dyn,
                                          p[pfx + "mask_template"], dout, None if chain else out, chain, B, T, HS, HT,
                                          flags=_zeros(x, 4 * B) if cross_role() else None, jobs=carry)
        red.untake(carry)
        if lin is not None:
            dx, dWp, dbp, dlogit, ddyn = lin
            red.jobs.bwd_pool(_ones(dev, dWp.shape[0]), dWp, gw.view(1, C * C))
            red.jobs.bwd_pool(_ones(dev, dbp.shape[0]), dbp, gb.view(1, C))
            return dx, CapParts(wn, ddyn, dlogit)
    fused = None
    if FUSE_CROSS and CTX.NODE_REDUCE is None and Y is None:
        fused = ops.cap_cross_route_bwd(x.view(B, T, N, C), p[pfx + "ln_p.weight"], p[pfx + "ln_p.bias"], c, dc1, dv, s, Rt, Ht, dyn,
                                        p[pfx + "mask_template"], B, T, HS, HT, flags=_zeros(x, 4 * B) if cross_role() else None)
    if fused is not None:
        dY, dlogit, ddyn = fused
    else:
        dS, ddyn = ops.cap_cross_bwd(dv, s, Rt, Ht, dyn, p[pfx + "mask_template"], B, T, HS, HT)
        dY, dlogit = ops.cap_route_bwd(x.view(B, T, N, C), p[pfx + "ln_p.weight"], p[pfx + "ln_p.bias"], c, dc1, dS, Y=Y)
    if C == 64:
        dx, dWp, dbp, ns2 = ops.linear_bwd(dY, x, p[pfx + "ln_p.weight"], dout, None if chain else out, premul=chain)
        red.jobs.bwd_pool(_ones(dev, ns2), dWp, gw.view(1, C * C))
        red.jobs.bwd_pool(_ones(dev, ns2), dbp, gb.view(1, C))
    else:
        if chain:
            dx = ops.apply(dY, p[pfx + "ln_p.weight"], MODE_SHARED, BT, N, resid=dout, resid2=x, epi=EPI_ADD_PREMUL)
        else:
            dx = ops.apply(dY, p[pfx + "ln_p.weight"], MODE_SHARED, BT, N, resid=dout, resid2=out, epi=EPI_ADD_DPRE)
        dWp, ns2 = ops.wgrad(dY, x, MODE_SHARED, BT, N, colsum_a=True)
        wp = _wb_parts(dWp, C, ns2)
        red.jobs.bwd_pool(_ones(dev, ns2), wp.dW, gw.view(1, C * C))
        red.jobs.bwd_pool(_ones(dev, ns2), wp.db, gb.view(1, C))
    return dx, CapParts(wn, ddyn, dlogit)


_ONES = {}


def _ones(dev, n=1):
    if (dev, n) not in _ONES:
        _ONES[(dev, n)] = torch.ones(n, 1, device=dev)
    return _ONES[(dev, n)]


class CondLinSaved(NamedTuple):
    x: Any
    out: Any
    W: Any


def condlin_fwd(x, Wg, bg, mode, dims):
    B, T, N, C = dims
    out = ops.apply(x, Wg, mode, B * T, N, bias=bg, epi=EPI_LRELU)
    return out, CondLinSaved(x, out, Wg)


def condlin_bwd(saved, dout, emb, wpool, bpool, g_wpool, g_bpool, d_emb, mode, dims, red, chain=False, premul=False, carried=None):
    assert not chain or chain_ok(dims)
    dx, w = carried if carried is not None else _genlin_bwd(dout, saved.out, saved.x, saved.W, mode, dims, chain, premul)
    queue_generated(red.jobs, emb, w, wpool, bpool, g_wpool, g_bpool, d_emb)
    return dx


def queue_generated(J, emb, parts, wpool, bpool, g_wpool, g_bpool, d_emb):
    K = emb.shape[1]
    cols = wpool.numel() // K
    dW = parts.dW if parts.dW.dim() == 2 else parts.dW.view(-1, cols)
    J.bwd_pool(emb, dW, g_wpool.view(K, cols), nsplit=parts.ns)
    J.bwd_pool(emb, parts.db, g_bpool, nsplit=parts.ns)
    J.bwd_emb(dW, wpool.view(K, cols), d_emb, nsplit=parts.ns)
    J.bwd_emb(parts.db, bpool, d_emb, nsplit=parts.ns)


def queue_ht(J, p, g, h, hp, time_eb, d_te):
    queue_generated(J, time_eb, hp, p[h + "weights_pool"], p[h + "bias_pool"], g[h + "weights_pool"], g[h + "bias_pool"], d_te)


def queue_cap(J, p, g, c, cp, node, spg, time):
    queue_generated(J, node[0], cp.wn, p[c + "weights_spa"], p[c + "bias_spa"], g[c + "weights_spa"], g[c + "bias_spa"], node[1])
    for (emb, d_emb), name, dy in ((spg, "t_adj", cp.ddyn), (time, "adj", cp.dlogit)):
        R, K = emb.shape
        dy = dy.view(R, -1)
        J.bwd_pool(emb, dy, g[c + name].view(K, -1))
        J.bwd_emb(dy, p[c + name].view(K, -1), d_emb)


ENC, DEC = "encoder.STHCN_encode.", "decoder.STHCN_decode."
GUIDE_TF = "encoder.teb4mask."


def _sthcn_names(pfx):
    return [pfx + "hyperTem%d." % i for i in (1, 2, 3, 4)], [pfx + "cap1.", pfx + "cap2."]


class SthcnGen(NamedTuple):
    emb: Any
    A_all: Any
    G_all: Any
    Wb: Any
    Wn: Any
    dadj: Any
    dyn: Any
    hts: Any
    cps: Any
    d: int
    Hm: int
    ds: int
    HS: int
    HT: int
    slot: Any

    def ht(self, i):
        return (self.G_all[i],) + self.Wb[i]


class SthcnSaved(NamedTuple):
    h1: Any
    h2: Any
    h3: Any
    h4: Any
    c1: Any
    c2: Any
    emb: Any
    gen: SthcnGen
    slot: Any


class GenAll(NamedTuple):
    sthcn: Any
    guide: Any
    pending: Any


def _sthcn_gen_jobs(p, pfx, emb, jobs, A_all, dims, G_all, slot=None):
    B, T, N, C = dims
    time_eb, teb, tes = emb
    ne, nes = p[pfx + "node_embeddings"], p[pfx + "node_embeddings_spg"]
    hts, cps = _sthcn_names(pfx)
    adj0 = p[hts[0] + "adj"]
    d, Hm = adj0.shape[0], adj0.shape[1]
    cadj, tadj = p[cps[0] + "adj"], p[cps[0] + "t_adj"]
    ds, HS, HT = cadj.shape[0], cadj.shape[1], tadj.shape[1]
    for i, h in enumerate(hts):
        jobs.fwd(ne, p[h + "adj"].view(d, Hm * T), out=A_all[i])
        jobs.gram(ne, p[h + "adj"].view(d, Hm * T), out=G_all[i], A=A_all[i])
    Wb = [(jobs.fwd(time_eb, p[h + "weights_pool"]), jobs.fwd(time_eb, p[h + "bias_pool"])) for h in hts]
    Wn = [(jobs.fwd(nes, p[c + "weights_spa"]), jobs.fwd(nes, p[c + "bias_spa"])) for c in cps]
    dadj = [jobs.fwd(teb, p[c + "adj"].view(ds, HS * N)) for c in cps]
    dyn = [jobs.fwd(tes, p[c + "t_adj"].view(ds, HT * T * HS)).view(B, HT, T * HS) for c in cps]
    return SthcnGen(emb, A_all, G_all, Wb, Wn, dadj, dyn, hts, cps, d, Hm, ds, HS, HT, slot)


def gen_all(p, tidx, dims, which=(ENC, DEC), guide=True, defer=False):
    B, T, N, C = dims
    tfj = []
    for pfx in which:
        tfj += [_tf_job(p, pfx + "time_feature1.", tidx), _tf_job(p, pfx + "time_feature1_.", tidx),
                _tf_job(p, pfx + "time_feature2.", tidx, spg=True)]
    if guide:
        tfj.append(_tf_job(p, GUIDE_TF, tidx))
    embs = ops.timefeat_jobs_fwd(tfj, tidx)
    jobs = ops.PoolJobs()
    now = ops.PoolJobs() if defer else jobs
    sthcn, gd = {}, None
    L = 4 * len(which)
    if guide:
        gj = now
        m = "encoder.MLP_RL."
        t4m = embs[-1]
        gd = (t4m, gj.fwd(p["encoder.neb4mask"], p[m + "weights_pool_spa"]), gj.fwd(p["encoder.neb4mask"], p[m + "bias_pool_spa"]),
              gj.fwd(t4m, p[m + "weights_pool_tem"]), gj.fwd(t4m, p[m + "bias_pool_tem"]))
    if L:
        adj0 = p[which[0] + "hyperTem1.adj"]
        Hm = adj0.shape[1]
        A_all = torch.empty(L, N, Hm * T, device=tidx.device)
        G_all = torch.empty(L, N, T, T, device=tidx.device)
        for k, pfx in enumerate(which):
            sthcn[pfx] = _sthcn_gen_jobs(p, pfx, embs[3 * k:3 * k + 3], jobs, A_all[4 * k:4 * k + 4], dims, G_all[4 * k:4 * k + 4], (k, len(which)))
    now.launch()
    return GenAll(sthcn, gd, jobs if defer else None)


def sthcn_fwd(p, pfx, tidx, x, dims, num_route, gen=None, head=None, next_gen=None, kl=None):
    if gen is None:
        gen = gen_all(p, tidx, dims, which=(pfx,), guide=False).sthcn[pfx]
    ht = gen.ht
    cap = lambda i, x: cap_core_fwd(p, gen.cps[i], x, gen.dadj[i], gen.dyn[i], *gen.Wn[i], dims, num_route, gen.HS, gen.HT)
    pairs = chain_fwd_ok(dims)
    nhead = None
    x, h1 = head if head is not None else hypertem_core_fwd(x, *ht(0), dims)
    x, c1, sc1 = cap(0, x)
    if pairs:
        if kl is not None and kl.c1 is None:
            kl.c1 = c1
        (h2, h3), x = ht_chain_fwd(x, [ht(1), ht(2)], dims, kl)
    else:
        x, h2 = hypertem_core_fwd(x, *ht(1), dims)
        x, h3 = hypertem_core_fwd(x, *ht(2), dims)
    x, _, sc2 = cap(1, x)
    if pairs and next_gen is not None:
        (h4, h1n), xn = ht_chain_fwd(x, [ht(3), next_gen.ht(0)], dims, kl)
        x, nhead = h4.out, (xn, h1n)
    else:
        x, h4 = hypertem_core_fwd(x, *ht(3), dims)
    return x, c1, SthcnSaved(h1, h2, h3, h4, sc1, sc2, gen.emb, gen, gen.slot), nhead


def _grad_buffers(red, slot, N, T, HmT, ref, nsG):
    if slot is None:
        return torch.empty(4, nsG, N, T, T, device=ref.device), torch.empty(4, N, HmT, device=ref.device)
    k, n = slot
    if red._dG is None or red._dG.shape[0] != 4 * n:
        red._dG = torch.empty(4 * n, nsG, N, T, T, device=ref.device)
        red._dA = torch.empty(4 * n, N, HmT, device=ref.device)
    return red._dG[4 * k:4 * k + 4], red._dA[4 * k:4 * k + 4]


def sthcn_bwd(p, g, pfx, tidx, sv, dout, dims, red, chain=False, premul_in=False, defer_h1=False, after_pending=None):
    B, T, N, C = dims
    time_eb, teb, tes = sv.emb
    gn = sv.gen
    A_all, hts, cps, d, Hm, ds, HS, HT = gn.A_all, gn.hts, gn.cps, gn.d, gn.Hm, gn.ds, gn.HS, gn.HT
    ne, nes = p[pfx + "node_embeddings"], p[pfx + "node_embeddings_spg"]
    dne, dnes = g[pfx + "node_embeddings"], g[pfx + "node_embeddings_spg"]
    d_te, d_teb, d_tes = _zeros(time_eb, *time_eb.shape), _zeros(teb, *teb.shape), _zeros(tes, *tes.shape)
    nsG = graph_grad_splits(dims)
    dG_all, dA_all = _grad_buffers(red, sv.slot, N, T, Hm * T, dout, nsG)
    J = red.jobs
    e_te, e_node, e_spg, e_teb = (time_eb, d_te), (nes, dnes), (tes, d_tes), (teb, d_teb)

    if isinstance(dout, PendingH1):
        up = dout
        dd, _, hp4 = ht_pair_bwd(up.saved, sv.h4, up.dd, up.dG, dG_all[3], dims, dWb1=up.dWb)
        red.keep.append(up)
        if after_pending is not None:
            after_pending()
    else:
        dd, hp4 = hypertem_core_bwd(sv.h4, dout, dG_all[3], dims, chain, True)
    queue_ht(J, p, g, hts[3], hp4, *e_te)
    dd, cp2 = cap_core_bwd(p, g, cps[1], sv.c2, dd, dims, HS, HT, red, chain)
    queue_cap(J, p, g, cps[1], cp2, e_node, e_spg, e_teb)
    pair = ht_pair_bwd(sv.h3, sv.h2, dd, dG_all[2], dG_all[1], dims) if chain and pair_bwd_on() else None
    if pair is not None:
        dd, hp3, hp2 = pair
    else:
        dd, hp3 = hypertem_core_bwd(sv.h3, dd, dG_all[2], dims, chain, True)
        dd, hp2 = hypertem_core_bwd(sv.h2, dd, dG_all[1], dims, chain, True)
    queue_ht(J, p, g, hts[2], hp3, *e_te)
    queue_ht(J, p, g, hts[1], hp2, *e_te)
    dd, cp1 = cap_core_bwd(p, g, cps[0], sv.c1, dd, dims, HS, HT, red, chain)
    queue_cap(J, p, g, cps[0], cp1, e_node, e_spg, e_teb)
    if isinstance(sv.h1, EncIn):
        assert chain
        e = sv.h1
        w, bi = p["encoder.dim_in_flow.weight"], p["encoder.dim_in_flow.bias"]
        carry = red.take_all() if red.tail else None
        if nsG == B:
            dWb, _, dinp = ops.encin_ht1_bwd(dd.view(B, T, N, C), e.source, e.mask, e.fill, w, bi, e.Wbt, e.ab, e.wv, dG=dG_all[0], jobs=carry)
        else:
            dWb, dGb, dinp = ops.encin_ht1_bwd(dd.view(B, T, N, C), e.source, e.mask, e.fill, w, bi, e.Wbt, e.ab, e.wv)
            torch.sum(dGb, 0, out=dG_all[0][0])
        hp1 = _wb_parts(dWb, C)
        wb = _wb_view(g["encoder.dim_in_flow.weight"], g["encoder.dim_in_flow.bias"])
        if wb is not None:
            red.jobs.bwd_pool(_ones(dd.device, dinp.shape[0]), dinp, wb)
        else:
            g["encoder.dim_in_flow.weight"].add_(dinp[:, :C].sum(0).view(C, 1))
            g["encoder.dim_in_flow.bias"].add_(dinp[:, C:].sum(0))
        red.keep.append((dinp, dWb))
        dd = None
    elif defer_h1:
        assert chain and premul_in
        ns = ops.wgrad_nsplit(MODE_TIME, B * T, N, C)
        dWb = torch.empty(ns * B * T, C * C + C, device=dd.device, dtype=torch.float32)
        hp1 = _wb_parts(dWb, C, ns)
        dd = PendingH1(sv.h1, dd, dG_all[0], dWb)
    else:
        dd, hp1 = hypertem_core_bwd(sv.h1, dd, dG_all[0], dims, chain, premul_in)
    queue_ht(J, p, g, hts[0], hp1, *e_te)
    red.gram(A_all.view(4 * N, Hm, T), dG_all, dA_all.view(4 * N, Hm, T), N, nsG)
    for i, h in enumerate(hts):
        red.late.bwd_pool(ne, dA_all[i], g[h + "adj"].view(d, Hm * T))
        red.late.bwd_emb(dA_all[i], p[h + "adj"].view(d, Hm * T), dne)
    red.timefeat(p, g, pfx + "time_feature1.", tidx, d_te)
    red.timefeat(p, g, pfx + "time_feature1_.", tidx, d_teb)
    red.timefeat(p, g, pfx + "time_feature2.", tidx, d_tes, spg=True)
    red.keep.append((sv, hp1, hp2, hp3, hp4, cp1, cp2, dout))
    return dd


class EncIn:

    def __init__(self, source, mask, fill, Wbt, ab, wv):
        self.source, self.mask, self.fill, self.Wbt, self.ab, self.wv = source, mask, fill, Wbt, ab, wv


ENCIN = os.environ.get("GPTST_ENCIN", "1") == "1"


def encin_ok(dims, base):
    return ENCIN and base == 1 and dims[3] in (64, 128) and dims[1] == 12 and chain_ok(dims)


GUIDEIN = os.environ.get("GPTST_GUIDEIN", "1") == "1"
GUIDE_HEAD = os.environ.get("GPTST_GUIDE_HEAD", "1") == "1"


class LowRankIn(NamedTuple):
    Wspa: Any


class GuideSaved(NamedTuple):
    t4m: Any
    spa: Any
    tem: Any
    h2: Any
    label: Any


def guide_fwd(p, source, tidx, dims, base, gen=None, lowrank_in=False):
    B, T, N, C = dims
    if gen is None:
        gen = gen_all(p, tidx, dims, which=(), guide=True).guide
    t4m, Wspa, bspa, Wtem, btem = gen
    m = "encoder.MLP_RL."
    if lowrank_in and GUIDEIN and GUIDE_HEAD and base == 1 and C == 64:
        r = ops.guide_head_fwd(source, p[m + "ln1.weight"], p[m + "ln1.bias"], Wspa, bspa, Wtem, btem, p[m + "ln3.weight"], p[m + "ln3.bias"])
        if r is not None:
            h1, h2, prob, label = r
            return prob, GuideSaved(t4m, LowRankIn(Wspa), CondLinSaved(h1, h2, Wtem), h2, label)
    if lowrank_in and GUIDEIN and base == 1 and C in (64, 128):
        h1 = ops.guide_in_fwd(source, p[m + "ln1.weight"], p[m + "ln1.bias"], Wspa, bspa)
        s1 = LowRankIn(Wspa)
    else:
        h0 = ops.lin_in(source, base + 2, base, p[m + "ln1.weight"], p[m + "ln1.bias"], C)
        h1, s1 = condlin_fwd(h0, Wspa, bspa, MODE_NODE, dims)
    h2, s2 = condlin_fwd(h1, Wtem, btem, MODE_TIME, dims)
    prob, label = ops.rowdot(h2, p[m + "ln3.weight"], p[m + "ln3.bias"], softmax=True, want_label=True)
    return prob, GuideSaved(t4m, s1, s2, h2, label)


def _wb_view(gw, gb):
    n = gw.numel() + gb.numel()
    if gb.data_ptr() != gw.data_ptr() + 4 * gw.numel():
        return None
    return torch.as_strided(gw, (1, n), (n, 1))


def fused_tails_ok(p, C, base, HS):
    return (C in (64, 128) and base <= ops.TAIL_MAXJ and HS <= ops.TAIL_MAXJ
            and _wb_view(p["decoder.dim_flow_out.weight"], p["decoder.dim_flow_out.bias"]) is not None
            and _wb_view(p["encoder.MLP_RL.ln3.weight"], p["encoder.MLP_RL.ln3.bias"]) is not None)


def loss_tail(p, g, dec, source, mask, base, sigma, mu, thresh, sws, red, chain=False):
    wo = "decoder.dim_flow_out."
    out, dd, part = ops.tail_mae(dec, p[wo + "weight"], p[wo + "bias"], source, base + 2, mask, sigma, mu, thresh, sws, premul=chain)
    red.jobs.bwd_pool(_ones(dec.device, part.shape[0]), part, _wb_view(g[wo + "weight"], g[wo + "bias"]))
    red.keep.append((part, dd))
    return out, dd


def kl_head(p, g, sv_g, prob, c1, N, w, sws, red, chain=False, carried=None):
    m = "encoder.MLP_RL."
    dh2, part = carried if carried is not None else ops.tail_kl(sv_g.h2, p[m + "ln3.weight"], prob, c1, N, w, sws, premul=chain)
    red.jobs.bwd_pool(_ones(prob.device, part.shape[0]), part, _wb_view(g[m + "ln3.weight"], g[m + "ln3.bias"]))
    red.keep.append((part, dh2))
    return dh2


def _linear_out_bwd(p, g, pfx, h, dy, C, chain, d_h=None):
    J = dy.shape[1]
    dh = ops.lin_in(dy, J, J, p[pfx + "weight"], None, C, wlayout=1)
    ops.rowouter(dy, J, J, h, g[pfx + "weight"], 1, asum=g[pfx + "bias"])
    if d_h is not None:
        dh = dh + d_h
    if chain:
        dh = dh * torch.where(h > 0, 1.0, 0.01)
    return dh


def guide_bwd(p, g, source, tidx, saved, dlogit, dims, base, red, dh2=None, chain=False, carried=None):
    B, T, N, C = dims
    carried = carried or KlOut()
    t4m, s1, s2, h2 = saved.t4m, saved.spa, saved.tem, saved.h2
    m = "encoder.MLP_RL."
    if dh2 is None:
        dh2 = _linear_out_bwd(p, g, m + "ln3.", h2, dlogit, C, chain)
    d_t4m = _zeros(t4m, *t4m.shape)
    dh1 = condlin_bwd(s2, dh2, t4m, p[m + "weights_pool_tem"], p[m + "bias_pool_tem"], g[m + "weights_pool_tem"],
                      g[m + "bias_pool_tem"], d_t4m, MODE_TIME, dims, red, chain, True, carried=carried.tem)
    if isinstance(s1, LowRankIn):
        assert chain
        neb, wpool, bpool = p["encoder.neb4mask"], p[m + "weights_pool_spa"], p[m + "bias_pool_spa"]
        dWb, dinp = carried.inp if carried.inp is not None else ops.guide_in_bwd(dh1, source, p[m + "ln1.weight"], p[m + "ln1.bias"], s1.Wspa)
        queue_generated(red.jobs, neb, _wb_parts(dWb, C), wpool, bpool, g[m + "weights_pool_spa"], g[m + "bias_pool_spa"], g["encoder.neb4mask"])
        wb = _wb_view(g[m + "ln1.weight"], g[m + "ln1.bias"])
        if wb is not None:
            red.jobs.bwd_pool(_ones(dh1.device, N), dinp, wb)
        else:
            g[m + "ln1.weight"].add_(dinp[:, :C].sum(0).view(C, 1))
            g[m + "ln1.bias"].add_(dinp[:, C:].sum(0))
        red.keep.append((dWb, dinp))
        dh0 = None
    else:
        dh0 = condlin_bwd(s1, dh1, p["encoder.neb4mask"], p[m + "weights_pool_spa"], p[m + "bias_pool_spa"],
                          g[m + "weights_pool_spa"], g[m + "bias_pool_spa"], g["encoder.neb4mask"], MODE_NODE, dims, red, chain, False)
        _in_proj_grads(source, base, dh0, g[m + "ln1.weight"], g[m + "ln1.bias"], None, 0.0, red)
    red.timefeat(p, g, GUIDE_TF, tidx, d_t4m)
    red.keep.append((saved, dlogit, dh2, dh1, dh0))


def kl_carry_ok(dims, HS, sv_g):
    B, T, N, C = dims
    return (CARRY_KL and C == 64 and T == 12 and HS <= ops.TAIL_MAXJ and chain_fwd_ok(dims) and chain_ok(dims)
            and sv_g is not None and isinstance(sv_g.spa, LowRankIn))


class KlOut:

    def __init__(self):
        self.head = None
        self.tem = None
        self.inp = None


class KlCarry:

    def __init__(self, p, sv_g, prob, source, dims, w, sws):
        self.p, self.sv_g, self.prob, self.source, self.dims, self.w, self.sws = p, sv_g, prob, source, dims, w, sws
        self.c1 = None
        self.stage = 0
        self.out = KlOut()

    def guest(self):
        if self.c1 is None or self.stage == 3:
            return None
        B, T, N, C = self.dims
        m = "encoder.MLP_RL."
        p, sv_g, dev = self.p, self.sv_g, self.prob.device
        HS = self.prob.shape[1]
        st = self.stage + 1
        f = dict(device=dev, dtype=torch.float32)
        if st == 1:
            h2, W3 = sv_g.h2, p[m + "ln3.weight"]
            dh2 = torch.empty_like(h2)
            part = torch.empty(ops.tail_parts(B * T * N), HS * C + HS, **f)
            self.out.head = (dh2, part)
            ts = [h2, W3, self.prob, self.c1, dh2, part, self.sws]
        elif st == 2:
            h1, Wtem = sv_g.tem.x, sv_g.tem.W
            dh2, _ = self.out.head
            ns = _C.lib().value("gptst_apply_wgrad_nsplit", MODE_TIME, B * T, N)
            dh1, dW, db = torch.empty_like(h1), torch.empty(ns * B * T, C * C, **f), torch.empty(ns * B * T, C, **f)
            self.out.tem = (dh1, WgradParts(dW, ns, db))
            ts = [dh2, h1, Wtem, dh1, dW, db]
        else:
            dh1, _ = self.out.tem
            dWb, dinp = torch.empty(N, C * C + C, **f), torch.empty(N, 2 * C, **f)
            self.out.inp = (dWb, dinp)
            ts = [dh1, self.source, p[m + "ln1.weight"], p[m + "ln1.bias"], sv_g.spa.Wspa, dWb, dinp]
        self.stage = st
        return (st, ts, 0, ops.kl_guest_blocks(st, B, T, N), HS, self.source.shape[-1], self.w)


def _in_proj_grads(source, base, dY, gW, gb, mask, fill, red):
    wb = _wb_view(gW, gb)
    if base == 1 and wb is not None:
        C = dY.shape[1]
        part = ops.rowouter_part(source, base + 2, base, dY, mask=mask, fill=fill)
        red.jobs.bwd_pool(_ones(dY.device, part.shape[0]), part[:, :2 * C], wb)
        red.keep.append(part)
    else:
        ops.rowouter(source, base + 2, base, dY, gW, 0, csum=gb, mask=mask, fill=fill)


class Forward(NamedTuple):
    emb: Any
    c1: Any
    dec: Any
    out: Any
    sv_e: Any
    sv_d: Any


def autoencoder_fwd(p, source, mask, dims, base, num_route, scaler_zeros, gen=None, tidx=None, lowrank_in=False, kl=None, head=True,
                    decoder=True, join=True):
    B, T, N, C = dims
    if tidx is None:
        tidx = source[:, :, 0, base:base + 2].contiguous()
    gen_e, gen_d = (gen.sthcn[ENC], gen.sthcn[DEC] if decoder else None) if gen is not None else (None, None)
    first = None
    if lowrank_in and gen_e is not None and encin_ok(dims, base):
        w, bi = p["encoder.dim_in_flow.weight"], p["encoder.dim_in_flow.bias"]
        G1, Wbt1, bbt1 = gen_e.ht(0)
        o1, ab, wv = ops.encin_ht1_fwd(source, base, mask, 0.0 if mask is None else scaler_zeros, w, bi, G1, Wbt1, bbt1)
        first = (o1.view(-1, C), EncIn(source, mask, 0.0 if mask is None else scaler_zeros, Wbt1, ab, wv))
        x0 = None
    else:
        x0 = ops.lin_in(source, base + 2, base, p["encoder.dim_in_flow.weight"], p["encoder.dim_in_flow.bias"], C,
                        mask=mask, fill=scaler_zeros)
    emb, c1, sv_e, dec_h1 = sthcn_fwd(p, ENC, tidx, x0, dims, num_route, gen=gen_e, head=first, next_gen=gen_d if join else None, kl=kl)
    if not decoder:
        return Forward(emb, c1, None, None, sv_e, None)
    dec, _, sv_d, _ = sthcn_fwd(p, DEC, tidx, emb, dims, num_route, gen=gen_d, head=dec_h1, kl=kl)
    out = ops.rowdot(dec, p["decoder.dim_flow_out.weight"], p["decoder.dim_flow_out.bias"]) if head else None
    return Forward(emb, c1, dec, out, sv_e, sv_d)


def model_bwd(p, g, source, mask, tidx, sv_e, sv_d, dec, d_out, d_dec, dims, base, scaler_zeros, red, dd=None, chain=False):
    B, T, N, C = dims
    if dd is None:
        dd = _linear_out_bwd(p, g, "decoder.dim_flow_out.", dec, d_out, C, chain, d_h=d_dec)
    defer = (chain and (red.on_bucket is None or PAIR_UNDER_DP) and not isinstance(sv_d.h1, EncIn)
             and ht_pair_ok(sv_d.h1, sv_e.h4, dims))
    late = defer and red.on_bucket is not None
    d_emb = sthcn_bwd(p, g, DEC, tidx, sv_d, dd, dims, red, chain, True, defer_h1=defer)
    if not late:
        red.flush_async(tidx)
    d_x0 = sthcn_bwd(p, g, ENC, tidx, sv_e, d_emb, dims, red, chain, False,
                     after_pending=(lambda: red.flush_async(tidx)) if late else None)
    red.flush_async(tidx)
    if d_x0 is not None:
        _in_proj_grads(source, base, d_x0, g["encoder.dim_in_flow.weight"], g["encoder.dim_in_flow.bias"], mask, scaler_zeros, red)


def encoder_bwd(p, g, source, tidx, sv_e, d_emb, dims, base, red):
    d_x0 = sthcn_bwd(p, g, ENC, tidx, sv_e, d_emb, dims, red, chain=False, premul_in=False)
    _in_proj_grads(source, base, d_x0, g["encoder.dim_in_flow.weight"], g["encoder.dim_in_flow.bias"], None, 0.0, red)


def step_bwd(p, g, source, mask, tidx, fw, prob, sv_g, dims, base, scaler_zeros, red, loss, stats, sws=None, with_kl=False, kl=None):
    B, T, N, C = dims
    sigma, mu, thresh = loss
    if sws is not None:
        chain = chain_ok(dims)
        done = kl.out if kl is not None else KlOut()
        _, dd = loss_tail(p, g, fw.dec, source, mask, base, sigma, mu, thresh, sws, red, chain=chain)
        red.tail = chain and tail_roles_ok(red, dims, fw.sv_e)
        kl_first = red.tail and with_kl and None not in (done.head, done.tem, done.inp)
        if kl_first:
            dh2 = kl_head(p, g, sv_g, prob, fw.c1, N, 0.1, sws, red, chain=chain, carried=done.head)
            guide_bwd(p, g, source, tidx, sv_g, None, dims, base, red, dh2=dh2, chain=chain, carried=done)
        model_bwd(p, g, source, mask, tidx, fw.sv_e, fw.sv_d, fw.dec, None, None, dims, base, scaler_zeros, red, dd=dd, chain=chain)
        if with_kl and not kl_first:
            dh2 = kl_head(p, g, sv_g, prob, fw.c1, N, 0.1, sws, red, chain=chain, carried=done.head)
            guide_bwd(p, g, source, tidx, sv_g, None, dims, base, red, dh2=dh2, chain=chain, carried=done)
    else:
        M = B * T * N
        ops.mae_fwd(fw.out, source, base + 2, mask, sigma, mu, thresh, M, base, stats)
        d_out = ops.mae_bwd(fw.out, source, base + 2, mask, sigma, mu, thresh, M, base, stats, normalize=False)
        model_bwd(p, g, source, mask, tidx, fw.sv_e, fw.sv_d, fw.dec, d_out, None, dims, base, scaler_zeros, red)
        if with_kl:
            dlogit = ops.kl(prob, fw.c1, N, 0.1, stats)
            guide_bwd(p, g, source, tidx, sv_g, dlogit, dims, base, red)


def module_bwd(p, g, source, mask, tidx, fw, prob, sv_g, dims, base, scaler_zeros, red, d_out, d_dec=None, d_prob=None, chain=False):
    model_bwd(p, g, source, mask, tidx, fw.sv_e, fw.sv_d, fw.dec, d_out, d_dec, dims, base, scaler_zeros, red, chain=chain)
    if d_prob is not None:
        dlogit = (prob * (d_prob - (d_prob * prob).sum(-1, keepdim=True))).contiguous()
        guide_bwd(p, g, source, tidx, sv_g, dlogit, dims, base, red, chain=chain)


def warm_up(fn):
    s = torch.cuda.Stream()
    s.wait_stream(torch.cuda.current_stream())
    with torch.cuda.stream(s):
        for _ in range(2):
            fn()
    torch.cuda.current_stream().wait_stream(s)
    torch.cuda.synchronize()


_GC_LOCK, _GC_HELD = threading.Lock(), [0, False]


@contextlib.contextmanager
def quiet_gc():
    with _GC_LOCK:
        if _GC_HELD[0] == 0:
            gc.collect()
            _GC_HELD[1] = gc.isenabled()
            gc.disable()
        _GC_HELD[0] += 1
    try:
        yield
    finally:
        with _GC_LOCK:
            _GC_HELD[0] -= 1
            if _GC_HELD[0] == 0 and _GC_HELD[1]:
                gc.enable()
```

gpt-st_amd/ops.py:

```python
import contextlib
import ctypes
import math
from typing import Any, NamedTuple

import torch

from . import _C

MODE_TIME, MODE_NODE, MODE_SHARED = 0, 1, 2
PRO_NONE, PRO_DPRE = 0, 1
EPI_PLAIN, EPI_RES_LRELU, EPI_ADD_DPRE, EPI_LRELU, EPI_ADD_PREMUL, EPI_PREMUL = 0, 1, 2, 3, 4, 5

_p = _C.ptr


TIMER = None
LAST_CALL = {}


CALL_LOCK = None


def _call(name, *args, tag="", nbytes=0, entry=None):
    fn = entry or name
# ... 137 lines not shown

    def bwd_pool(self, emb, dW, dpool, nsplit=1):
        _chk(emb, dpool)
        R, K = emb.shape
        cols = dpool.numel() // K
        self.jobs.append(PoolJob(self.BWD_POOL, emb, dW, None, dpool, R, K, cols, nsplit, self._ldx(dW, cols)))

    def bwd_emb(self, dW, pool, demb, nsplit=1):
        _chk(pool, demb)
        R, K = demb.shape
        cols = pool.numel() // K
        self.jobs.append(PoolJob(self.BWD_EMB, None, dW, pool, demb, R, K, cols, nsplit, self._ldx(dW, cols)))

    @staticmethod
    def columns(js, fields=PoolJob._fields):
        return [len(js)] + [(_ptrs0 if f in ("emb", "dW", "pool", "out") else _ints)([getattr(j, f) for j in js])
                            for f in PoolJob._fields if f in fields]

    def take_reductions(self):
        assert not self.post and all(j.kind in (self.BWD_POOL, self.BWD_EMB) for j in self.jobs)
        js, self.jobs = self.jobs, []
        return self.columns(js), "+jobs%d" % len(js), _nb(*[t for j in js for t in (j.emb, j.dW, j.pool, j.out)]), js

    def launch(self):
        js, self.jobs = self.jobs, []
        post, self.post = self.post, []
        if js:
            _call("gptst_pool_jobs", *self.columns(js), nbytes=_nb(*[t for j in js for t in (j.emb, j.dW, j.pool, j.out)]))
        for A, G, rows, Hm in post:
            _call("gptst_gram_fwd", _p(A), _p(G), rows, Hm)


def _ptrs0(ts):
    return (ctypes.c_void_p * len(ts))(*[(t.data_ptr() if t is not None else None) for t in ts])


def apply(A, W, mode, BT, N, bias=None, resid=None, A2=None, transw=False, pro=PRO_NONE, epi=EPI_PLAIN, colsum=None,
          out=None, resid2=None):
    _chk(A, W, bias, resid, A2, resid2)
    C = A.shape[-1]
    if out is None:
        out = torch.empty_like(A)
    cs, ns = None, 0
    if colsum is not None:
        G = BT if mode == MODE_TIME else (N if mode == MODE_NODE else 1)
        ns = _C.lib().value("gptst_apply_nsplit", mode, BT, N, C)
        cs = torch.empty(ns * G, C, device=A.device, dtype=torch.float32)
    _call("gptst_apply", _p(A), _p(A2), _p(W), int(W.dim() == 3), int(transw), _p(bias), _p(resid), _p(resid2), _p(out), _p(cs),
          mode, pro, epi, BT, N, C, tag="mode%d pro%d epi%d" % (mode, pro, epi), nbytes=_nb(A, A2, W, bias, resid, resid2, out))
    if colsum is True:
        return out, cs, ns
    if colsum is not None:
        colsum.add_(cs.view(ns, -1, C).sum(0).view_as(colsum))
    return out


def apply_wgrad(dOut, Y, S, W, mode, BT, N, premul=False):
    _chk(dOut, Y, S, W)
    C = dOut.shape[-1]
    G = BT if mode == MODE_TIME else N
    ns = _C.lib().value("gptst_apply_wgrad_nsplit", mode, BT, N)
    dS = torch.empty_like(dOut)
    dW = torch.empty(ns * G, C * C, device=dOut.device, dtype=torch.float32)
    db = torch.empty(ns * G, C, device=dOut.device, dtype=torch.float32)
    _call("gptst_apply_wgrad", _p(dOut), _p(Y), _p(S), _p(W), _p(dS), _p(dW), _p(db), int(premul), mode, BT, N, C, tag="mode%d" % mode,
          nbytes=_nb(dOut, Y, S, W, dS, dW))
    return dS, dW, db, ns


def linear_bwd(dY, X, Wp, dOut, out, premul=False):
    _chk(dY, X, Wp, dOut, out)
    rows, C = dY.shape
    ns = _C.lib().value("gptst_linear_bwd_nsplit", rows)
    dX = torch.empty_like(dY)
    dWp = torch.empty(ns, C * C, device=dY.device, dtype=torch.float32)
    dbp = torch.empty(ns, C, device=dY.device, dtype=torch.float32)
    _call("gptst_linear_bwd", _p(dY), _p(X), _p(Wp), _p(dOut), _p(out), _p(dX), _p(dWp), _p(dbp), int(premul), rows, C,
          nbytes=_nb(dY, X, dOut, out, dX, dWp))
    return dX, dWp, dbp, ns


def wgrad_nsplit(mode, BT, N, C=64):
    return _C.lib().value("gptst_wgrad_nsplit", mode, BT, N, C)


def wgrad(A, D, mode, BT, N, D2=None, pro=PRO_NONE, colsum_a=False, colsum_d=False):
    _chk(A, D, D2)
    C = A.shape[-1]
    ns = wgrad_nsplit(mode, BT, N, C)
    G = BT if mode == MODE_TIME else (N if mode == MODE_NODE else 1)
    if colsum_a or colsum_d:
        dW = torch.empty(ns * G, C * C + C, device=A.device, dtype=torch.float32)
        _call("gptst_wgrad_colsum", _p(A), _p(D), _p(D2), _p(dW), mode, pro, 1 if colsum_a else 2, BT, N, C,
              tag="mode%d pro%d cs" % (mode, pro), nbytes=_nb(A, D, D2, dW))
    else:
        dW = torch.empty(ns * G, C, C, device=A.device, dtype=torch.float32)
        _call("gptst_wgrad", _p(A), _p(D), _p(D2), _p(dW), mode, pro, BT, N, C, tag="mode%d pro%d" % (mode, pro), nbytes=_nb(A, D, D2, dW))
    return dW, ns


def gram_fwd(A):
    N, Hm, T = A.shape
    G = torch.empty(N, T, T, device=A.device, dtype=torch.float32)
    _call("gptst_gram_fwd", _p(A), _p(G), N, Hm)
    return G


def gram_bwd(A, dG, out=None, layers=1, nsplit=1, jobs=None):
    LN, Hm, T = A.shape
    dA = out if out is not None else torch.empty_like(A)
    if jobs is not None and jobs.jobs:
        cols, tag, nb, held = jobs.take_reductions()
        _call("gptst_gram_bwd", _p(A), _p(dG), _p(dA), layers, LN // layers, Hm, nsplit, *cols, tag=tag, nbytes=nb, entry="gptst_gram_bwd_jobs")
        del held
    else:
        _call("gptst_gram_bwd", _p(A), _p(dG), _p(dA), layers, LN // layers, Hm, nsplit)
    return dA


def tmix(X, G, dOut=None, Y=None):
    _chk(X, G, dOut, Y)
    B, T, N, C = X.shape
    out = torch.empty_like(X)
    _call("gptst_tmix", _p(X), _p(G), _p(dOut), _p(Y), _p(out), B, T, N, C, tag="bwd" if dOut is not None else "fwd",
          nbytes=_nb(X, G, dOut, Y, out))
    return out


def hypertem_fwd(X, G, Wbt, bbt, want_R=True):
    _chk(X, G, Wbt, bbt)
    B, T, N, C = X.shape
    R = torch.empty_like(X) if want_R else None
    out = torch.empty_like(X)
    _call("gptst_hypertem_fwd", _p(X), _p(G), _p(Wbt), _p(bbt), _p(R), _p(out), B, T, N, C, nbytes=_nb(X, G, Wbt, bbt, R, out))
    return R, out


def hypertem_chain_fwd(X, stages, want_R=True, guest=None):
    B, T, N, C = X.shape
    _chk(X, *[t for st in stages for t in st])
    f = lambda: torch.empty(B, T, N, C, device=X.device, dtype=torch.float32)
    Rs = [f() if want_R else None for _ in stages]
    outs = [f() for _ in stages]
    chain = (_p(X), len(stages), _ptrs0([st[0] for st in stages]), _ptrs0([st[1] for st in stages]), _ptrs0([st[2] for st in stages]),
             _ptrs0(Rs), _ptrs0(outs), B, T, N, C)
    if guest is None:
        _call("gptst_hypertem_chain_fwd", *chain, tag="x%d" % len(stages), nbytes=_nb(X, *Rs, *outs))
    else:
        stage, ts, v0, v1, HS, lda, w = guest
        _chk(*ts)
        _call("gptst_hypertem_chain_fwd_kl", *chain, stage, _ptrs0(ts), v0, v1, HS, lda, float(w), tag="x%d+kl%d" % (len(stages), stage),
              nbytes=_nb(X, *Rs, *outs))
    return list(zip(Rs, outs))


def kl_guest_blocks(stage, B, T, N):
    return _C.lib().value("gptst_kl_guest_blocks", stage, B, T, N)


def encin_ht1_fwd(source, base, mask, fill, w, bi, G, Wbt, bbt):
    B, T, N, F = source.shape
    C = Wbt.shape[-1]
    assert base == 1
    _chk(source, mask, w, bi, G, Wbt, bbt)
    f = dict(device=source.device, dtype=torch.float32)
    out, ab, wv = torch.empty(B, T, N, C, **f), torch.empty(B * T * N, 2, **f), torch.empty(B * T, 2 * C, **f)
    _call("gptst_encin_ht1_fwd", _p(source), F, _p(mask), float(fill), _p(w), _p(bi), _p(G), _p(Wbt), _p(bbt), _p(out), _p(ab), _p(wv), B, T, N, C,
          nbytes=_nb(Wbt, out))
    return out, ab, wv


def encin_ht1_bwd(dPre, source, mask, fill, w, bi, Wbt, ab, wv, dG=None, jobs=None):
    B, T, N, F = source.shape
    C = Wbt.shape[-1]
    _chk(dPre, source, mask, w, bi, Wbt, ab, wv, dG)
    f = dict(device=source.device, dtype=torch.float32)
    dWb, dinp = torch.empty(B * T, C * C + C, **f), torch.empty(B * T, 2 * C, **f)
    if dG is None:
        dG = torch.empty(B, N, T, T, **f)
    host = (_p(dPre), _p(source), F, _p(mask), float(fill), _p(w), _p(bi), _p(Wbt), _p(ab), _p(wv), _p(dWb), _p(dG), _p(dinp), B, T, N, C)
    if jobs is not None and jobs.jobs:
        cols, tag, nb, held = jobs.take_reductions()
        _call("gptst_encin_ht1_bwd", *host, *cols, tag=tag, nbytes=_nb(dPre, Wbt, dWb, dG) + nb, entry="gptst_encin_ht1_bwd_jobs")
        del held
    else:
        _call("gptst_encin_ht1_bwd", *host, nbytes=_nb(dPre, Wbt, dWb, dG))
    return dWb, dG, dinp


def guide_in_fwd(source, w1, b1, Wn, bn):
    B, T, N, F = source.shape
    C = Wn.shape[-1]
    _chk(source, w1, b1, Wn, bn)
    h1 = torch.empty(B * T * N, C, device=source.device, dtype=torch.float32)
    _call("gptst_guide_in_fwd", _p(source), F, _p(w1), _p(b1), _p(Wn), _p(bn), _p(h1), B * T, N, C, nbytes=_nb(Wn, h1))
    return h1


def guide_head_fwd(source, w1, b1, Wn, bn, Wbt, bbt, W3, b3):
    B, T, N, F = source.shape
    C, J = Wn.shape[-1], W3.shape[0]
    if C != 64 or J > 16:
        return None
    _chk(source, w1, b1, Wn, bn, Wbt, bbt, W3, b3)
    dev = source.device
    f = dict(device=dev, dtype=torch.float32)
    uc = torch.empty(N, 2 * C, **f)
    h1, h2 = torch.empty(B * T * N, C, **f), torch.empty(B * T * N, C, **f)
    prob = torch.empty(B * T * N, J, **f)
    label = torch.empty(B * T * N, device=dev, dtype=torch.int32)
    _call("gptst_guide_head_fwd", _p(source), F, _p(w1), _p(b1), _p(Wn), _p(bn), _p(Wbt), _p(bbt), _p(W3), _p(b3), _p(uc), _p(h1), _p(h2), _p(prob),
          _p(label), B * T, N, C, J, nbytes=_nb(Wbt, h1, h2, prob))
    return h1, h2, prob, label


def guide_in_bwd(dPre, source, w1, b1, Wn):
    B, T, N, F = source.shape
    C = Wn.shape[-1]
    _chk(dPre, source, w1, b1, Wn)
    f = dict(device=source.device, dtype=torch.float32)
    dWb, dinp = torch.empty(N, C * C + C, **f), torch.empty(N, 2 * C, **f)
    _call("gptst_guide_in_bwd", _p(dPre), _p(source), F, _p(w1), _p(b1), _p(Wn), _p(dWb), _p(dinp), B * T, N, C, nbytes=_nb(dPre, Wn, dWb))
    return dWb, dinp


def hypertem_ntiles(N):
    return _C.lib().value("gptst_hypertem_ntiles", N)


def hypertem_bwd(dOut, Y, X, G, Wbt, dG=None, want_dbias=True, premul=False):
    _chk(dOut, Y, X, G, Wbt, dG)
    B, T, N, C = X.shape
    dX = torch.empty_like(X)
    nt = hypertem_ntiles(N)
    dbias = torch.empty(nt * B * T, C, device=X.device, dtype=torch.float32) if want_dbias else None
    if dG is None:
        dG = torch.empty(B, N, T, T, device=X.device, dtype=torch.float32)
    _call("gptst_hypertem_bwd", _p(dOut), _p(Y), _p(X), _p(G), _p(Wbt), _p(dX), _p(dbias), _p(dG), int(premul), B, T, N, C,
          nbytes=_nb(dOut, Y, X, G, Wbt, dX))
    return dX, dbias, dG


def hypertem_bwd_wgrad(dOut, Y, X, G, Wbt, R, dG=None, premul=False):
    _chk(dOut, Y, X, G, Wbt, R, dG)
    B, T, N, C = X.shape
    dX = torch.empty_like(X)
    if dG is None:
        dG = torch.empty(B, N, T, T, device=X.device, dtype=torch.float32)
    ns = wgrad_nsplit(MODE_TIME, B * T, N, C)
    dWb = torch.empty(ns * B * T, C * C + C, device=X.device, dtype=torch.float32)
    _call("gptst_hypertem_bwd_wgrad", _p(dOut), _p(Y), _p(X), _p(G), _p(Wbt), _p(R), _p(dX), _p(dG), _p(dWb), int(premul), B, T, N, C,
          nbytes=_nb(dOut, Y, X, G, Wbt, R, dX, dWb))
    return dX, dWb, ns, dG


def hypertem_bwd_pair(dOut1, X1, G1, Wbt1, R1, X0, G0, Wbt0, R0, dG1, dG0, cnt, dWb1=None):
    _chk(dOut1, X1, G1, Wbt1, R1, X0, G0, Wbt0, R0, dG1, dG0, cnt, dWb1)
    B, T, N, C = X1.shape
    if C != 64:
        return None
    dXmid, dX0 = torch.empty_like(X1), torch.empty_like(X0)
    ns = wgrad_nsplit(MODE_TIME, B * T, N, C)
    dWb0 = torch.empty(ns * B * T, C * C + C, device=X1.device, dtype=torch.float32)
    if dWb1 is None:
        dWb1 = torch.empty_like(dWb0)
    assert dWb1.shape == dWb0.shape
    try:
        _call("gptst_hypertem_bwd_pair", _p(dOut1), _p(X1), _p(G1), _p(Wbt1), _p(R1), _p(X0), _p(G0), _p(Wbt0), _p(R0), _p(dXmid), _p(dX0),
              _p(dG1), _p(dG0), _p(dWb1), _p(dWb0), _p(cnt), B, T, N, C, nbytes=_nb(dOut1, X1, R1, X0, R0, dXmid, dX0, dWb0, dWb1))
    except _C.GptstError as e:
        if e.code != _C.ESHAPE:
            raise
        return None
    return dXmid, dX0, dWb1, dWb0, ns


def tmix_bwd(dR, X, G, dOut, Y, dG=None):
    _chk(dR, X, G, dOut, Y, dG)
    B, T, N, C = X.shape
    dX = torch.empty_like(X)
    if dG is None:
        dG = torch.empty(N, T, T, device=X.device, dtype=torch.float32)
    _call("gptst_tmix_bwd", _p(dR), _p(X), _p(G), _p(dOut), _p(Y), _p(dX), _p(dG), B, T, N, C, nbytes=_nb(dR, X, dOut, Y, dX))
    return dX, dG


def tmix_bwd_chain(dR, X, G, dPre, premul=False, dG=None):
    _chk(dR, X, G, dPre, dG)
    B, T, N, C = X.shape
    dX = torch.empty_like(X)
    if dG is None:
        dG = torch.empty(N, T, T, device=X.device, dtype=torch.float32)
    _call("gptst_tmix_bwd_chain", _p(dR), _p(X), _p(G), _p(dPre), int(bool(premul)), _p(dX), _p(dG), B, T, N, C, nbytes=_nb(dR, X, dPre, dX))
    return dX, dG


def tmix_dgraph(dR, X, out=None):
    _chk(dR, X, out)
    B, T, N, C = X.shape
    dG = out if out is not None else torch.empty(N, T, T, device=X.device, dtype=torch.float32)
    _call("gptst_tmix_dgraph", _p(dR), _p(X), _p(dG), B, T, N, C, nbytes=_nb(dR, X, dG))
    return dG


FORCE_CAP_BIG = False

# ... 919 lines not shown
```

gpt-st_amd/step.py:

```python
import contextlib
import dataclasses
import itertools
import os
import random
from typing import Any, NamedTuple

import torch

from . import engine, ops

DEFER_GEN = os.environ.get("GPTST_DEFER_GEN", "1") == "1"
U24 = os.environ.get("GPTST_MASK_U24", "1") == "1"


class Part1(NamedTuple):
    tidx: Any
    gen: Any
    red: Any
    prob: Any
    sv_g: Any


@dataclasses.dataclass(eq=False)
class Enqueued:
# ... 4 lines not shown
    src: Any
    stats: Any
    replay: int
    group: int
    slot: Any
    row: Any = None


class PretrainStep:
    RING = 8
    DETERMINISTIC_MODE = True
    FORCED_MASK = True

    def __init__(self, model, args, scaler_mean, scaler_std, batch_size, use_graph=True, dp=None, seed=0, global_mask=True,
                 deterministic=None):
        self.model, self.args = model, args
        self.mean, self.std = float(scaler_mean), float(scaler_std)
        self.B, self.T, self.N = batch_size, args.lag, args.num_nodes
        self.C, self.base, self.HS = args.hidden_dim, args.input_base_dim, args.HS
        self.dims = (self.B, self.T, self.N, self.C)
        self.dev = model.flat.device
        assert self.dev.type == "cuda", "PretrainStep needs the model on an MI355X (no CPU fallback)"
        self.use_graph, self.dp = use_graph, dp
        self.deterministic = self.DETERMINISTIC_MODE and ((os.environ.get("GPTST_DETERMINISTIC", "0") == "1") if deterministic is None else bool(deterministic))
        n = model.flat.numel()
        self.gbuf = torch.zeros(n + 8, device=self.dev)
        self.gflat, self.stats = self.gbuf[:n], self.gbuf[n:]
        self.g = model.views_of(self.gflat)
        self.m, self.v = torch.zeros(n, device=self.dev), torch.zeros(n, device=self.dev)
        M = self.B * self.T * self.N
        self.src = torch.zeros(self.B, self.T, self.N, self.base + 2, device=self.dev)
        self.noise = torch.zeros(M * self.base, device=self.dev)
        self.noise_ar = torch.zeros(2 * M, device=self.dev)
        self.noise_a, self.noise_r = self.noise_ar[:M], self.noise_ar[M:]
        self.hc = torch.zeros(16 + self.HS + 4, dtype=torch.int32, device=self.dev)
        self.hyper = self.hc[:16].view(torch.float32)
        self.ctrl = self.hc[16:16 + self.HS + 2]
        self.rng_words = self.hc[16 + self.HS + 2:]
        self.noise_seed = 1234567 + seed
        self._ring = ops.PinnedRing(self.hc.numel(), slots=self.RING)
        self.phase_kl = False
        self._gK, self._group_failed = 0, False
        self.stats_out = torch.zeros(8, device=self.dev)
        self.mask_buf = torch.ones(M * self.base, device=self.dev)
        self.last_mask = None
        self.force_mask = False
        self.tA = self.tB = 0
        self.lr = args.lr_init
        self.rng = random.Random(seed)
        self.graphs = {}
        self._g_graphs = {}
        self._graph_comm_failed = False
        self._ctx_keep = []
        self._sws = None
        self.inject_noise = False
        self.global_count_scale = False
        self.node_reduce = None
        self.join_enc_dec = True
        self.safe_mode = False
        self.lost_steps = 0
        self.lost_batches = 0
        self._ledger = []
        self._holder = {}
        self._ids = itertools.count()
        self.arena = engine.ZeroArena(self.dev)
        self.fused_tails = os.environ.get("GPTST_FUSED_TAILS", "1") == "1" and engine.fused_tails_ok(model.param_views(), self.C, self.base, self.HS)
        self.W = dp.world if dp is not None else 1
        self.gmask = bool(global_mask) and dp is not None and self.W > 1
        if self.gmask:
            Mg = M * self.W
            self.noise_g = torch.zeros(Mg * self.base, device=self.dev)
            self.noise_ar_g = torch.zeros(2 * Mg, device=self.dev)
            self.noise_a_g, self.noise_r_g = self.noise_ar_g[:Mg], self.noise_ar_g[Mg:]
            self.label_l = torch.zeros(M, dtype=torch.int32, device=self.dev)
            self.label_g = torch.zeros(Mg, dtype=torch.int32, device=self.dev)
        self.always_guide = os.environ.get("GPTST_ALWAYS_GUIDE", "0") == "1"
        self.dp_overlap = (os.environ.get("GPTST_DP_OVERLAP", "0") != "0" and dp is not None and getattr(dp, "capturable", False)
                           and (self.W > 1 or os.environ.get("GPTST_FORCE_DP", "0") == "1"))
        self.dec_lo, self.dec_hi = self._decoder_bucket(model)
        self.rank_weight = 1.0
        self.fork_side = torch.cuda.Stream() if self.dp_overlap else None

    def _needs_exchange(self, phase):
        return self.gmask and phase == 1 and not self.force_mask

    @staticmethod
    def _decoder_bucket(model):
        offs = [(o, model.state_dict()[k].numel()) for k, o in model._offs.items() if k.startswith("decoder.") and o < model.nA]
        lo = min(o for o, _ in offs)
        hi = max(o + (n + 3) // 4 * 4 for o, n in offs)
        assert hi == model.nA and all(o >= lo for o, _ in offs), (lo, hi, model.nA)
        assert not any(lo <= o < hi for k, o in model._offs.items() if not k.startswith("decoder.")), "decoder bucket is not contiguous"
        return lo, hi

    def _allreduce(self, sl):
        if self.rank_weight != 1.0:
            assert not self.use_graph, "a rank weight is baked into a captured graph: tail rounds use eager steppers"
            lost = self.stats[5:6].clone()
            sl.mul_(self.rank_weight)
            self.stats[5:6].copy_(lost)
        self.dp.allreduce_(sl)

    def _bucket_ready(self, k):
        if k == 0:
            self._allreduce(self.gbuf[self.dec_lo:self.dec_hi])
            self._dec_reduced = True

    def _dp_in_graph(self):
        return self.dp is not None and getattr(self.dp, "capturable", False) and not self._graph_comm_failed

    def _part1(self, phase):
        p, dims, base = self.model.param_views(), self.dims, self.base
        engine.CTX.ARENA, engine.CTX.NODE_REDUCE = self.arena, self.node_reduce
        src = self.src
        noise = None if self.inject_noise or self.force_mask else self._noise_buffer(phase)
        tidx = ops.step_begin(self.gbuf, self.arena.begin(zero=False), src, base, noise=noise, rng=self.rng_words)
        need_guide = self._need_guide(phase)
        gen = engine.gen_all(p, tidx, dims, guide=need_guide, defer=DEFER_GEN)
        red = engine.Reductions()
        red.no_carry = self.deterministic
        red.want_tail = True
        self._dec_reduced = False
        if self.dp_overlap and self._dp_in_graph():
            red.on_bucket = self._bucket_ready
            red.bucket_inline, red.fork_side = True, self.fork_side
        lowrank = self.fused_tails and engine.chain_ok(dims)
        prob, sv_g = engine.guide_fwd(p, src, tidx, dims, base, gen=gen.guide, lowrank_in=lowrank) if need_guide else (None, None)
        if self._needs_exchange(phase):
            self.label_l.copy_(sv_g.label)
        return Part1(tidx, gen, red, prob, sv_g)

    def _part2(self, phase, ctx):
        if not self.safe_mode:
            return self._part2_impl(phase, ctx)
        with engine.no_handoffs():
            return self._part2_impl(phase, ctx)

    def _part2_impl(self, phase, ctx):
        mdl, p, g, dims, base = self.model, self.model.param_views(), self.g, self.dims, self.base
        a = self.args
        src, tidx, gen, red, prob, sv_g = self.src, ctx.tidx, ctx.gen, ctx.red, ctx.prob, ctx.sv_g
        engine.CTX.ARENA, engine.CTX.NODE_REDUCE = self.arena, self.node_reduce
        pend = gen.pending
        mask = self._make_mask(phase, prob, sv_g.label if sv_g is not None else None, pend)
        if pend is not None:
            pend.launch()
        self.last_mask = mask
        fused = self.fused_tails
        kl, sws = None, None
        if phase == 1 and self._carry_kl(sv_g):
            sws = self._tail_sws()
            kl = engine.KlCarry(p, sv_g, prob, src, dims, 0.1, sws)
        fw = engine.autoencoder_fwd(p, src, mask, dims, base, mdl.num_route, mdl.scaler_zeros, gen=gen, tidx=tidx,
                                    lowrank_in=fused and engine.chain_ok(dims), kl=kl, head=not fused, join=self.join_enc_dec)
        if fused and sws is None:
            sws = self._tail_sws()
        engine.step_bwd(p, g, src, mask, tidx, fw, prob, sv_g, dims, base, mdl.scaler_zeros, red, (self.std, self.mean, a.mape_thresh),
                        self.stats, sws=sws, with_kl=phase == 1, kl=kl)
        self._fold_stats(sws)
        red.flush(tidx)
        engine.CTX.ARENA = engine.CTX.NODE_REDUCE = None
        self._after_backward(phase)

    def _noise_buffer(self, phase):
        if self.gmask:
            return self.noise_g if phase == 0 else self.noise_ar_g
        return self.noise if phase == 0 else self.noise_ar

    def _need_guide(self, phase):
        return phase == 1 or self.always_guide

    def _make_mask(self, phase, prob, label, pend):
        a = self.args
        if self.force_mask:
            return self.mask_buf
        noise = self._noise_buffer(phase)
        if phase == 0:
            mask = ops.mask_random(noise, int(noise.numel() * a.mask_ratio), ws=self._mask_ws(), u24=U24, jobs=pend)
        else:
            noise_a, noise_r = noise.chunk(2)
            mask = ops.mask_adaptive(self._mask_labels(label), None, self.ctrl[:self.HS], self.ctrl[self.HS:], noise_a, noise_r,
                                     a.ada_type == "all", self.base, ws=self._mask_ws(), u24=U24, jobs=pend)[2]
        return self._mask_cut(mask)

    def _mask_labels(self, label):
        return self.label_g if self.gmask else label

    def _mask_cut(self, mask):
        if not self.gmask:
            return mask
        self.last_mask_global = mask
        return self.dp.rows_of(mask, self.B * self.T * self.N * self.base)

    def _fold_stats(self, sws):
        if sws is None:
            return
        if self.dp is None:
            self._sws = sws
        else:
            ops.stats_fold(sws, self.stats)

    def _after_backward(self, phase):
        if self.dp is None:
            self._optim()
        elif self._dp_in_graph():
            if self._dec_reduced:
                self._allreduce(self.gbuf[:self.dec_lo])
                self._allreduce(self.gbuf[self.dec_hi:])
            else:
                self._allreduce(self.gbuf)
            self._optim()

    def _tail_sws(self):
        return self.arena.zeros(ops.tail_parts(self.B * self.T * self.N), 4)

    def _carry_kl(self, sv_g):
        return (self.fused_tails and self.dp is None and not self.global_count_scale and not self.deterministic and not self.safe_mode
                and not self.always_guide and engine.CTX.NODE_REDUCE is None and engine.kl_carry_ok(self.dims, self.HS, sv_g))

    def _mask_ws(self):
        return self.arena.zeros(ops.mask_ws_floats())

    def _exchange_labels(self):
        self.dp.gather_labels(self.label_l, out=self.label_g)

    def _optim(self):
        sws, self._sws = self._sws, None
        ops.clip_adam(self.model.flat, self.gflat, self.m, self.v, self.model.nA, self.model.nB, self.hyper, self.stats,
                      stats_out=self.stats_out, sws=sws)

    @contextlib.contextmanager
    def _launch_mode(self):
        if self.DETERMINISTIC_MODE:
            ops.set_deterministic(self.deterministic)
        try:
            yield
        finally:
            if self.DETERMINISTIC_MODE:
                ops.set_deterministic(False)
            engine.CTX.ARENA = engine.CTX.NODE_REDUCE = None

    def _enqueue(self, phase):
        ctx = self._part1(phase)
        if self._needs_exchange(phase):
            self._exchange_labels()
        self._part2(phase, ctx)

    def _body(self, phase):
        with self._launch_mode():
            self._enqueue(phase)

    def _phase(self, epoch):
        return 0 if epoch <= self.args.change_epoch else 1

    def _fill(self, row, phase, epoch, list_c):
        a, HS = self.args, self.HS
        self.tA += 1
        if phase == 1:
            self.tB += 1
        self.phase_kl = phase == 1
        tA = self.tA
        row[:13].view("float32")[:] = ops.adam_scalars(self.lr, tA, self.tB, 0.9, 0.999, 1e-8, float(a.max_grad_norm) if a.grad_norm else 0.0,
                                                       kl=phase == 1, sum_loss=True)
        row[16 + HS + 2:16 + HS + 4] = (self.noise_seed & 0x7FFFFFFF, tA & 0x7FFFFFFF)
        if phase == 0:
            return None
        if list_c is None:
            list_c = list(range(HS))
            self.rng.shuffle(list_c)
        list_c = [int(v) for v in list_c]
        ada, rnd = self.model.adaptive_counts(self.B * self.T * self.N * (self.W if self.gmask else 1), epoch)
        ada, rnd = self._budgets(ada, rnd, epoch)
        row[16:16 + HS + 2] = list_c + [int(ada), int(rnd)]
        return list_c

    def _budgets(self, ada, rnd, epoch):
        return ada, rnd

    def _graphed(self):
        return self.use_graph

    def step(self, source, epoch, noise=None, noise_a=None, noise_r=None, list_c=None, forced_mask=None, _sub=None):
        phase = self._phase(epoch)
        forced = forced_mask is not None
        if forced and not self.FORCED_MASK:
            raise ValueError("%s does not teacher-force masks" % type(self).__name__)
        if source is not self.src:
            self.src.copy_(source, non_blocking=True)
        inject = noise is not None or noise_a is not None
        if inject:
            buf = self._noise_buffer(phase)
            if phase == 0:
                buf.copy_(noise.reshape(-1), non_blocking=True)
            else:
                na, nr = buf.chunk(2)
                na.copy_(noise_a.reshape(-1), non_blocking=True)
                nr.copy_(noise_r.reshape(-1), non_blocking=True)
        if forced:
            self.mask_buf.copy_(forced_mask.reshape(-1), non_blocking=True)
        list_c = self._fill(self._ring.next(), phase, epoch, list_c)
        self._ring.send(self.hc)
        key = (phase, inject, forced)
        if not self._graphed():
            self.inject_noise, self.force_mask = inject, forced
            self._body(phase)
        else:
            if key not in self.graphs:
# ... 285 lines not shown
```

include/gptst_hip.h:

```cpp
#ifndef GPTST_HIP_H
#define GPTST_HIP_H
#include <stdint.h>

#ifdef __cplusplus
extern "C" {
#endif
#if defined(__GNUC__)
#pragma GCC visibility push(default)
#endif

#define GPTST_ABI_VERSION 26
int gptst_abi_version(void);
int gptst_set_deterministic(int on);
int gptst_deterministic_state(void);
int gptst_handoff_timeouts(int* out);
int gptst_handoff_reset(void);
int gptst_mask_cooperative(int on);
int gptst_mask_cooperative_state(void);
int gptst_set_handoff_guard(int on);

int gptst_poolgen_fwd(const float* emb, const float* pool, float* out, int cols, const float* pool2, float* out2,
                      int cols2, int R, int K, void* stream);
int gptst_poolgen_bwd_pool(const float* emb, const float* dW, float* dpool, int cols, const float* dW2, float* dpool2,
                           int cols2, int R, int nsplit, int K, void* stream);
int gptst_poolgen_bwd_emb(const float* dW, const float* pool, int cols, const float* dW2, const float* pool2, int cols2,
                          float* demb, int R, int nsplit, int K, void* stream);

int gptst_poolgen_fwd_multi(const float* emb, int nprob, const void* pools, const void* outs, const int* cols, int R, int K,
                            void* stream);
int gptst_poolgen_bwd_pool_multi(const float* emb, int nprob, const void* dWs, const void* dpools, const int* cols, const int* nsplit,
                                 int R, int K, void* stream);
int gptst_poolgen_bwd_emb_multi(int nprob, const void* dWs, const void* pools, const int* cols, const int* nsplit, float* demb, int R,
                                int K, void* stream);

int gptst_pool_jobs(int njobs, const int* kind, const void* const* emb, const void* const* x, const void* const* pool,
                    const void* const* out, const int* R, const int* K, const int* cols, const int* nsplit, const int* ldx, void* stream);
int gptst_pool_jobs_gram_rows(int K, int cols);

int gptst_apply_nsplit(int mode, int BT, int N, int C);
int gptst_apply(const float* A, const float* A2, const float* W, int w_per_group, int transw, const float* bias,
                const float* resid, const float* resid2, float* out, float* colsum, int mode, int pro, int epi, int BT,
                int N, int C, void* stream);
int gptst_wgrad_nsplit(int mode, int BT, int N, int C);
int gptst_wgrad(const float* A, const float* D, const float* D2, float* dW, int mode, int pro, int BT, int N, int C,
                void* stream);
int gptst_wgrad_colsum(const float* A, const float* D, const float* D2, float* dW, int mode, int pro, int which, int BT, int N, int C,
                       void* stream);

int gptst_apply_wgrad_nsplit(int mode, int BT, int N);
int gptst_apply_wgrad(const float* dOut, const float* Y, const float* S, const float* W, float* dS, float* dW, float* colsum, int premul,
                      int mode, int BT, int N, int C, void* stream);

int gptst_linear_bwd_nsplit(int rows);
int gptst_linear_bwd(const float* dY, const float* X, const float* Wp, const float* dOut, const float* out, float* dX, float* dWp, float* dbp,
                     int premul, int rows, int C, void* stream);

int gptst_gram_fwd(const float* A, float* G, int N, int Hm, void* stream);
int gptst_gram_bwd(const float* A, const float* dG, float* dA, int L, int N, int Hm, int nsplit, void* stream);
int gptst_gram_bwd_jobs(const float* A, const float* dG, float* dA, int L, int N, int Hm, int nsplit,
                        int njobs, const int* jkind, const void* const* jemb, const void* const* jx, const void* const* jpool,
                        const void* const* jout, const int* jR, const int* jK, const int* jcols, const int* jnsplit, const int* jldx,
                        void* stream);
int gptst_tmix(const float* X, const float* G, const float* dOut, const float* Y, float* out, int B, int T, int N, int C,
               void* stream);
int gptst_tmix_dgraph(const float* dR, const float* X, float* dG, int B, int T, int N, int C, void* stream);
int gptst_tmix_bwd(const float* dR, const float* X, const float* G, const float* dOut, const float* Y, float* dX, float* dG, int B, int T,
                   int N, int C, void* stream);
int gptst_tmix_bwd_chain(const float* dR, const float* X, const float* G, const float* dPre, int premul, float* dX, float* dG, int B, int T,
                         int N, int C, void* stream);

int gptst_hypertem_fwd(const float* X, const float* G, const float* Wbt, const float* bbt, float* R_out, float* out, int B, int T,
                       int N, int C, void* stream);
int gptst_hypertem_chain_fwd(const float* X, int nstage, const void* Gs, const void* Wbts, const void* bbts, const void* Rs, const void* outs,
                             int B, int T, int N, int C, void* stream);
int gptst_hypertem_chain_fwd_kl(const float* X, int nstage, const void* Gs, const void* Wbts, const void* bbts, const void* Rs, const void* outs,
                                int B, int T, int N, int C, int stage, const void* ops, int v0, int v1, int HS, int lda, float w, void* stream);
int gptst_kl_guest_blocks(int stage, int B, int T, int N);

int gptst_encin_ht1_fwd(const float* src, int lda, const float* mask, float fill, const float* w, const float* bi, const float* G,
                        const float* Wbt, const float* bbt, float* out, float* ab, float* wv, int B, int T, int N, int C, void* stream);
int gptst_encin_ht1_bwd(const float* dPre, const float* src, int lda, const float* mask, float fill, const float* w, const float* bi,
                        const float* Wbt, const float* ab, const float* wv, float* dWb, float* dG, float* dinp, int B, int T, int N, int C,
                        void* stream);
int gptst_encin_ht1_bwd_jobs(const float* dPre, const float* src, int lda, const float* mask, float fill, const float* w, const float* bi,
                             const float* Wbt, const float* ab, const float* wv, float* dWb, float* dG, float* dinp, int B, int T, int N, int C,
                             int njobs, const int* jkind, const void* const* jemb, const void* const* jx, const void* const* jpool,
                             const void* const* jout, const int* jR, const int* jK, const int* jcols, const int* jnsplit, const int* jldx,
                             void* stream);

int gptst_guide_in_fwd(const float* src, int lda, const float* w1, const float* b1, const float* Wn, const float* bn, float* h1, int BT, int N,
                       int C, void* stream);
int gptst_guide_in_bwd(const float* dPre, const float* src, int lda, const float* w1, const float* b1, const float* Wn, float* dWb, float* dinp,
                       int BT, int N, int C, void* stream);
int gptst_guide_uc_floats(int N, int C);
int gptst_guide_head_fwd(const float* src, int lda, const float* w1, const float* b1, const float* Wn, const float* bn, const float* Wbt,
                         const float* bbt, const float* W3, const float* b3, float* uc, float* h1, float* h2, float* prob, int* label,
                         int BT, int N, int C, int J, void* stream);

int gptst_hypertem_ntiles(int N);
int gptst_hypertem_bwd(const float* dOut, const float* Y, const float* X, const float* G, const float* Wbt, float* dX, float* dbias,
                       float* dG, int premul, int B, int T, int N, int C, void* stream);
int gptst_hypertem_bwd_wgrad(const float* dOut, const float* Y, const float* X, const float* G, const float* Wbt, const float* R, float* dX,
                             float* dG, float* dWb, int premul, int B, int T, int N, int C, void* stream);
int gptst_hypertem_bwd_pair(const float* dOut1, const float* X1, const float* G1, const float* Wbt1, const float* R1, const float* X0,
                            const float* G0, const float* Wbt0, const float* R0, float* dXmid, float* dX0, float* dG1, float* dG0,
                            float* dWb1, float* dWb0, void* cnt, int B, int T, int N, int C, void* stream);

int gptst_cap_route_fwd(const float* X, const float* Wp, const float* bp, const float* dadj, float* c_out, float* s_out, int BT, int N,
                        int C, int HS, int R, void* stream);
int gptst_cap_cross_fwd(const float* s, const float* dyn, const float* tmpl, float* v, float* Ht, float* Rt, int B, int T, int C,
                        int HS, int HT, void* stream);
int gptst_cap_cross_ws_floats(int B, int T, int C, int HS, int HT);
int gptst_cap_cross_bwd(const float* dv, const float* s, const float* Rt, const float* Ht, const float* dyn, const float* tmpl,
                        float* dS, float* ddyn, float* ws, int B, int T, int C, int HS, int HT, void* stream);
int gptst_cap_rec_fwd(const float* c, const float* v, float* rec, int BT, int N, int C, int HS, void* stream);
int gptst_cap_cross_rec_fwd(const float* s, const float* dyn, const float* tmpl, const float* c, float* v, float* Ht, float* Rt, float* rec,
                            int B, int T, int N, int C, int HS, int HT, void* stream);
int gptst_cap_rec_bwd(const float* drec, const float* c, const float* v, float* dc1, float* dv, int BT, int N, int C, int HS,
                      void* stream);
int gptst_cap_route_bwd(const float* X, const float* Wp, const float* bp, const float* c, const float* dc1, const float* dS,
                        float* dY, float* dlogit, int BT, int N, int C, int HS, void* stream);
int gptst_cap_cross_route_bwd(const float* X, const float* Wp, const float* bp, const float* c, const float* dc1, const float* dv,
                              const float* s, const float* Rt, const float* Ht, const float* dyn, const float* tmpl, float* dY,
                              float* dlogit, float* ddyn, float* dS_ws, void* flags, int B, int T, int N, int C, int HS, int HT, void* stream);
int gptst_cap_cross_route_lin_bwd(const float* X, const float* Wp, const float* bp, const float* c, const float* dc1, const float* dv,
                                  const float* s, const float* Rt, const float* Ht, const float* dyn, const float* tmpl,
                                  const float* dPre, const float* out, int premul, float* dX, float* dWp, float* dbp, float* dlogit,
                                  float* ddyn, float* dS_ws, void* flags, int B, int T, int N, int C, int HS, int HT, void* stream);
int gptst_cap_route_roles_ok(int B, int T, int N, int C, int HS, int HT);
int gptst_cap_cross_route_lin_bwd_jobs(const float* X, const float* Wp, const float* bp, const float* c, const float* dc1, const float* dv,
                                       const float* s, const float* Rt, const float* Ht, const float* dyn, const float* tmpl,
                                       const float* dPre, const float* out, int premul, float* dX, float* dWp, float* dbp, float* dlogit,
                                       float* ddyn, float* dS_ws, void* flags, int B, int T, int N, int C, int HS, int HT,
                                       int njobs, const int* jkind, const void* const* jemb, const void* const* jx, const void* const* jpool,
                                       const void* const* jout, const int* jR, const int* jK, const int* jcols, const int* jnsplit, const int* jldx,
                                       void* stream);
int gptst_cap_split_units(int BT, int N, int C, int HS);
int gptst_cap_cross_route_lin_bwd_split(const float* X, const float* Wp, const float* bp, const float* c, const float* dc1, const float* dv,
                                        const float* s, const float* Rt, const float* Ht, const float* dyn, const float* tmpl,
                                        const float* dPre, const float* out, int premul, float* dX, float* dWp, float* dbp, float* dlogit,
                                        float* ddyn, float* dS_ws, void* flags, int B, int T, int N, int C, int HS, int HT, int nsplit,
                                        int njobs, const int* jkind, const void* const* jemb, const void* const* jx, const void* const* jpool,
                                        const void* const* jout, const int* jR, const int* jK, const int* jcols, const int* jnsplit, const int* jldx,
                                        void* stream);

int gptst_cap_fits_lds(int N, int C, int HS);
int gptst_capbig_squash_rows(float* Y, long rows, int C, void* stream);
int gptst_capbig_softmax(const float* bl, const float* l0, float* cs, int BT, int HS, int N, int use_bl, int use_l0, void* stream);
int gptst_capbig_type1(const float* cs, const float* P, float* S, int BT, int HS, int N, int C, void* stream);
int gptst_capbig_post(const float* S, const float* V0, float* out, long rows, int C, int post, void* stream);
int gptst_capbig_type2(const float* V, const float* P, float* bl, int BT, int HS, int N, int C, void* stream);
int gptst_capbig_rec_fwd(const float* c, const float* v, float* rec, int BT, int HS, int N, int C, void* stream);
int gptst_capbig_rec_bwd_dc(const float* drec, const float* v, float* dc1, int BT, int HS, int N, int C, void* stream);
int gptst_capbig_route_bwd_rows(const float* Y, const float* c, const float* dc1, const float* dS, float* dY, float* dlogit, int BT,
                                int HS, int N, int C, void* stream);

int gptst_capflow_supported(int HS, int C);
int gptst_capflow_nparts(int N);
int gptst_capflow_squash(const float* Y, const float* dadj, float* P, float* part, int BT, int HS, int N, int C, void* stream);
int gptst_capflow_route(const float* rows, const float* V, const float* bl_in, float* bl_out, const float* l0, const float* c_in,
                        float* c_out, float* part, int BT, int HS, int N, int C, void* stream);
int gptst_capflow_post(const float* part, int nparts, int prow, float* V0, float* Vout, int mode, int BT, int HS, int C, void* stream);
int gptst_capflow_rec_fwd(const float* c, const float* v, float* rec, int BT, int HS, int N, int C, void* stream);
int gptst_capflow_route_bwd(const float* Y, const float* c, const float* dc1, const float* dS, float* dY, float* dlogit, int BT,
                            int HS, int N, int C, void* stream);

int gptst_metrics_accum(const float* out, const float* src, int lda, const float* vis, float sigma, float mu, int has_mae_thresh,
                        float mae_thresh, float mape_thresh, int B, int T, int N, int D, double* sums_t, double* sums_tn, void* stream);

int gptst_mask_ws_bytes(void);
int gptst_mask_random(const float* noise, int M, int k, float* mask, void* ws, int ws_zeroed, void* stream);
int gptst_mask_labels(const float* prob, int rows, int HS, int* label, int* counts, void* stream);
int gptst_mask_adaptive(const int* label, const int* counts, const int* list_c, const int* nums, const float* noise_a,
                        const float* noise_r, int ada_all, int M, int HS, int base, float* m_ada, float* m_rnd, float* mask,
                        void* ws, int ws_zeroed, void* stream);

int gptst_mask_random_u24(const float* noise, int M, int k, float* mask, void* ws, int ws_zeroed, void* stream);
int gptst_mask_adaptive_u24(const int* label, const int* counts, const int* list_c, const int* nums, const float* noise_a, const float* noise_r,
                            int ada_all, int M, int HS, int base, float* m_ada, float* m_rnd, float* mask, void* ws, int ws_zeroed, void* stream);
int gptst_mask_u24_fwd_jobs(int adaptive, const int* label, const int* counts, const int* list_c, const int* nums, const float* noise_a,
                            const float* noise_r, int ada_all, int M, int HS, int base, int k, float* m_ada, float* m_rnd, float* mask, void* ws,
                            int ws_zeroed, int njobs, const int* kind, const void* const* emb, const void* const* pool, const void* const* out,
                            const int* R, const int* K, const int* cols, void* stream);

int gptst_lin_in(const float* a, int lda, const float* mask, float fill, const float* W, int wlayout, const float* b, float* Y,
                 int rows, int J, int C, void* stream);
int gptst_rowdot(const float* X, const float* W, const float* b, float* Z, int rows, int J, int C, int do_softmax, int* label,
                 void* stream);
int gptst_fusion_gate_fwd(const float* F, const float* src, int lda, int base, const float* Ws, const float* bs, const float* Wh,
                          const float* bh, const float* Wo, const float* bo, const float* Wt, const float* bt, float* out, float* z,
                          int rows, int C, void* stream);
int gptst_fusion_gate_bwd(const float* dOut, const float* F, const float* z, const float* src, int lda, int base, const float* Wo,
                          const float* Wt, const float* bt, float* dpre, float* dxd, float* Hm, float* xt, int rows, int C, void* stream);
int gptst_fusion_gate_bwd_df(const float* dOut, const float* F, const float* z, const float* src, int lda, int base, const float* Wo,
                             const float* Wt, const float* bt, const float* Ws, float* dpre, float* dxd, float* Hm, float* xt, float* dF,
                             int rows, int C, void* stream);
int gptst_stgcn_tapgemm(const float* X, int ldx, int ci, int ntap, int dt0, int dt1, int dt2, int dt3, const float* W, const float* bias,
                        const float* R, int ldr, int res_w, float* Y, int co, float* S, float* A, int act, int rows, int T, int N,
                        void* stream);
int gptst_stgcn_gate_bwd(const float* dOut, const float* out, const float* S, const float* A, float* dPre, int act, int rows, int co,
                         void* stream);
int gptst_stgcn_wgrad_nsplit(int rows, int cw, int Ktot);
int gptst_stgcn_wgrad(const float* D, int cw, const float* X, int ldx, int ci, int ntap, int dt0, int dt1, int dt2, int dt3, float* part,
                      float* bpart, int nsplit, int rows, int T, int N, void* stream);
int gptst_stgcn_nodemix(const float* L, int Np, int ks, const float* In, float* Out, const float* R, int c, int reduce, int units, int N,
                        void* stream);
int gptst_stgcn_ln_fwd(const float* X, const float* gamma, const float* beta, float* Y, float* mean, float* rstd, int units, int M,
                       float eps, void* stream);
int gptst_stgcn_ln_bwd(const float* dY, const float* X, const float* gamma, const float* mean, const float* rstd, float* dX, int units,
                       int M, void* stream);
int gptst_stgcn_ln_nsplit(int units);
int gptst_stgcn_ln_bwd_param(const float* dY, const float* X, const float* mean, const float* rstd, float* pg, float* pb, int nsplit,
                             int units, int M, void* stream);
int gptst_tgcn_lds_bytes(int N, int Hp, int B);
int gptst_tgcn_fwd_gates(const float* L, int Np, const float* W0h, const float* h, const float* Gx0, float* u, float* r, float* q,
                         float* z, int ldz, int zoff, int B, int T, int N, int Hp, int t, int tiles, void* stream);
int gptst_tgcn_fwd_state(const float* L, int Np, const float* W1h, const float* q, const float* Gx1, const float* u, const float* h,
                         float* h_out, float* c, float* z, int ldz, int zoff, int B, int T, int N, int Hp, int t, int tiles,
                         void* stream);
int gptst_tgcn_bwd_cand(const float* LT, int Np, const float* W1hT, const float* dh, const float* u, const float* c, const float* r,
                        const float* h, float* dpre1, float* dpre0, float* dh_part, int B, int T, int N, int Hp, int t, int tiles,
                        void* stream);
int gptst_tgcn_bwd_state(const float* LT, int Np, const float* W0hT, const float* dpre0, const float* dh_part, float* dh_out, int B,
                         int T, int N, int Hp, int t, int tiles, void* stream);
int gptst_mtgnn_tapgemm(const float* X, int ldx, int ci, const float* XM, int ntap, const int* offs, const float* W, const float* bias,
                        const float* R, int ldr, int Tr, int roff, const float* OM, float* Y, int co, float* Tn, float* S, int gated,
                        int B, int Tsrc, int Tdst, int N, void* stream);
int gptst_mtgnn_gate_bwd(const float* dG, const float* Tn, const float* S, const float* OM, float* dPre, int rows, int co, void* stream);
int gptst_mtgnn_wgrad(const float* D, int cw, const float* X, int ldx, int ci, const float* XM, int ntap, const int* offs, float* part,
                      float* bpart, int nsplit, int B, int Tsrc, int Tdst, int N, void* stream);
// ... 137 lines not shown
```

Before: 935.5 steps/s.

## Fuse capsule node-apply GEMM with hypertem chain via counter handoff in one launch

New measurement: 935.3 steps/s. Within noise of the previous version (-0.0%).

```diff
diff --git a/gpt-st_amd/csrc/abi.hip b/gpt-st_amd/csrc/abi.hip
--- a/gpt-st_amd/csrc/abi.hip
+++ b/gpt-st_amd/csrc/abi.hip
@@ -10,21 +10,24 @@
 GPTST_INTERNAL int gptst_handoff_lost_capmfma(unsigned* out);
 GPTST_INTERNAL int gptst_handoff_lost_hypertem(unsigned* out);
 GPTST_INTERNAL int gptst_handoff_lost_masksel(unsigned* out);
+GPTST_INTERNAL int gptst_handoff_lost_nodechain(unsigned* out);
 extern "C" int gptst_handoff_timeouts(int* out) {
     if (!out) return GPTST_EARG;
-    unsigned a = 0u, b = 0u, c = 0u;
-    if (gptst_handoff_lost_capmfma(&a) || gptst_handoff_lost_hypertem(&b) || gptst_handoff_lost_masksel(&c)) return -5;
-    *out = (int)(a + b + c);
+    unsigned a = 0u, b = 0u, c = 0u, d = 0u;
+    if (gptst_handoff_lost_capmfma(&a) || gptst_handoff_lost_hypertem(&b) || gptst_handoff_lost_masksel(&c) || gptst_handoff_lost_nodechain(&d)) return -5;
+    *out = (int)(a + b + c + d);
     return GPTST_OK;
 }
 
 GPTST_INTERNAL int gptst_handoff_clear_capmfma(unsigned to);
 GPTST_INTERNAL int gptst_handoff_clear_hypertem(unsigned to);
 GPTST_INTERNAL int gptst_handoff_clear_masksel(unsigned to);
+GPTST_INTERNAL int gptst_handoff_clear_nodechain(unsigned to);
 GPTST_INTERNAL int gptst_adam_skipped_clear(void);
 extern "C" int gptst_handoff_reset(void) {
     if (hipDeviceSynchronize() != hipSuccess) return -5;
-    return (gptst_handoff_clear_capmfma(0u) || gptst_handoff_clear_hypertem(0u) || gptst_handoff_clear_masksel(0u) || gptst_adam_skipped_clear()) ? -5 : GPTST_OK;
+    return (gptst_handoff_clear_capmfma(0u) || gptst_handoff_clear_hypertem(0u) || gptst_handoff_clear_masksel(0u) || gptst_handoff_clear_nodechain(0u) ||
+            gptst_adam_skipped_clear()) ? -5 : GPTST_OK;
 }
 extern "C" int gptst_handoff_inject(int n) {
     if (n < 0) return GPTST_EARG;
diff --git a/gpt-st_amd/csrc/apply.hip b/gpt-st_amd/csrc/apply.hip
--- a/gpt-st_amd/csrc/apply.hip
+++ b/gpt-st_amd/csrc/apply.hip
@@ -1,5 +1,6 @@
 #include "mfma_tile.h"
 #include "wgrad64.h"
+#include "apply64_dev.h"
 #include "kl_guest.h"
 #ifdef GPTST_DEBUG
 __device__ long long g_ap_ts[64];
@@ -148,106 +149,8 @@
                                                          const float* __restrict__ bias, const float* __restrict__ resid,
                                                          const float* __restrict__ resid2, float* __restrict__ out,
                                                          float* __restrict__ colsum, RowMap rm, int tiles_per_wave) {
-    constexpr int C = 64;
-    __shared__ __attribute__((aligned(16))) float Wl[C * C];
-    __shared__ __attribute__((aligned(16))) float csl[4][C];
-    const int lane = threadIdx.x & 63, wave = threadIdx.x >> 6;
-    const int j = lane & 15, kk = lane >> 4;
-    const int g = blockIdx.x;
-    const int ntiles = (rm.M + 15) / 16;
-    const int t0 = (blockIdx.y * 4 + wave) * tiles_per_wave, t1 = min(ntiles, t0 + tiles_per_wave);
-    const float* Wg = W + (size_t)g * w_gstride;
-    float4 bias4 = f4zero();
-    if (bias != nullptr) bias4 = ld4(bias + (size_t)g * C + 4 * j);
-    float4 cs[4];
-#pragma unroll
-    for (int q = 0; q < 4; ++q) cs[q] = f4zero();
-    float4 an[4], on[4];
-    auto fetch = [&](int t) {
-        const int m = min(t * 16 + j, rm.M - 1);
-        const size_t off = ((size_t)g * rm.rs_g + (size_t)m * rm.rs_m) * C + 4 * kk;
-#pragma unroll
-        for (int q = 0; q < 4; ++q) {
-            an[q] = ld4(A + off + 16 * q);
-            if (PRO == PRO_DPRE) on[q] = ld4(A2 + off + 16 * q);
-        }
-    };
-    if (t0 < t1) fetch(t0);
-    load_w_lds<C, 256>(Wl, Wg, transw, threadIdx.x);
-    __syncthreads();
-    float4 bv[4][4];
-#pragma unroll
-    for (int q = 0; q < 4; ++q)
-#pragma unroll
-        for (int e = 0; e < 4; ++e) bv[q][e] = ld4(Wl + (16 * q + 4 * kk + e) * C + 4 * j);
-    for (int t = t0; t < t1; ++t) {
-        float4 a[4];
-        const bool rowok = t * 16 + j < rm.M;
-#pragma unroll
-        for (int q = 0; q < 4; ++q) {
-            float4 v = an[q];
-            if (PRO == PRO_DPRE) {
-                v.x *= lrelu_grad_from_out(on[q].x); v.y *= lrelu_grad_from_out(on[q].y);
-                v.z *= lrelu_grad_from_out(on[q].z); v.w *= lrelu_grad_from_out(on[q].w);
-            }
-            if (!rowok) v = f4zero();
-            a[q] = v;
-            cs[q] = f4add(cs[q], v);
-        }
-        float4 rv[4], rv2[4];
-        size_t orow[4];
-#pragma unroll
-        for (int r = 0; r < 4; ++r) {
-            const int m = min(t * 16 + kk * 4 + r, rm.M - 1);
-            orow[r] = ((size_t)g * rm.rs_g + (size_t)m * rm.rs_m) * C + 4 * j;
-            if (EPI == EPI_RES_LRELU || EPI == EPI_ADD_DPRE) rv[r] = ld4(resid + orow[r]);
-            if (EPI == EPI_ADD_DPRE) rv2[r] = ld4(resid2 + orow[r]);
-        }
-        if (t + 1 < t1) fetch(t + 1);
-        SB();
-        f32x4 acc[4];
-#pragma unroll
-        for (int ct = 0; ct < 4; ++ct) acc[ct] = (f32x4){0.f, 0.f, 0.f, 0.f};
-#pragma unroll
-        for (int q = 0; q < 4; ++q) {
-            const float av[4] = {a[q].x, a[q].y, a[q].z, a[q].w};
-#pragma unroll
-            for (int e = 0; e < 4; ++e) {
-                acc[0] = __builtin_amdgcn_mfma_f32_16x16x4f32(av[e], bv[q][e].x, acc[0], 0, 0, 0);
-                acc[1] = __builtin_amdgcn_mfma_f32_16x16x4f32(av[e], bv[q][e].y, acc[1], 0, 0, 0);
-                acc[2] = __builtin_amdgcn_mfma_f32_16x16x4f32(av[e], bv[q][e].z, acc[2], 0, 0, 0);
-                acc[3] = __builtin_amdgcn_mfma_f32_16x16x4f32(av[e], bv[q][e].w, acc[3], 0, 0, 0);
-            }
-        }
-        SB();
-#pragma unroll
-        for (int r = 0; r < 4; ++r) {
-            if (t * 16 + kk * 4 + r < rm.M) {
-                float4 y = f4add(make_float4(acc[0][r], acc[1][r], acc[2][r], acc[3][r]), bias4);
-                if (EPI == EPI_RES_LRELU) {
-                    y = f4add(y, rv[r]);
-                    y.x = lrelu(y.x); y.y = lrelu(y.y); y.z = lrelu(y.z); y.w = lrelu(y.w);
-                }
-                if (EPI == EPI_LRELU) { y.x = lrelu(y.x); y.y = lrelu(y.y); y.z = lrelu(y.z); y.w = lrelu(y.w); }
-                if (EPI == EPI_ADD_DPRE) {
-                    const float4 d = rv[r], o = rv2[r];
-                    y.x = fmaf(d.x, lrelu_grad_from_out(o.x), y.x); y.y = fmaf(d.y, lrelu_grad_from_out(o.y), y.y);
-                    y.z = fmaf(d.z, lrelu_grad_from_out(o.z), y.z); y.w = fmaf(d.w, lrelu_grad_from_out(o.w), y.w);
-                }
-                st4(out + orow[r], y);
-            }
-        }
-    }
-    if (colsum != nullptr) {
-#pragma unroll
-        for (int q = 0; q < 4; ++q) {
-            cs[q].x = group_sum<16>(cs[q].x); cs[q].y = group_sum<16>(cs[q].y);
-            cs[q].z = group_sum<16>(cs[q].z); cs[q].w = group_sum<16>(cs[q].w);
-            if (j == 0) st4(&csl[wave][16 * q + 4 * kk], cs[q]);
-        }
-        __syncthreads();
-        if (wave == 0) colsum[((size_t)blockIdx.y * rm.G + g) * C + lane] = (csl[0][lane] + csl[1][lane]) + (csl[2][lane] + csl[3][lane]);
-    }
+    __shared__ __attribute__((aligned(16))) float lds[APPLY64_LDS_FLOATS];
+    apply64_body<PRO, EPI, false>(A, A2, W, w_gstride, transw, bias, resid, resid2, out, colsum, rm, tiles_per_wave, blockIdx.x, blockIdx.y, lds);
 }
 
 static void apply64_geometry(const RowMap& rm, bool has_colsum, int& tpw, int& gy) {
diff --git a/gpt-st_amd/csrc/apply64_dev.h b/gpt-st_amd/csrc/apply64_dev.h
--- /dev/null
+++ b/gpt-st_amd/csrc/apply64_dev.h
@@ -0,0 +1,118 @@
+#pragma once
+#include "mfma_tile.h"
+#include "wgrad64.h"
+
+constexpr int APPLY64_LDS_FLOATS = 64 * 64 + 4 * 64;
+
+template <int PRO, int EPI, bool PUB>
+__device__ __forceinline__ void apply64_body(const float* __restrict__ A, const float* __restrict__ A2,
+                                             const float* __restrict__ W, long w_gstride, int transw,
+                                             const float* __restrict__ bias, const float* __restrict__ resid,
+                                             const float* __restrict__ resid2, float* __restrict__ out,
+                                             float* __restrict__ colsum, RowMap rm, int tiles_per_wave, int g, int y,
+                                             float* __restrict__ lds) {
+    constexpr int C = 64;
+    float* Wl = lds;
+    float (*csl)[C] = reinterpret_cast<float (*)[C]>(lds + C * C);
+    const int lane = threadIdx.x & 63, wave = threadIdx.x >> 6;
+    const int j = lane & 15, kk = lane >> 4;
+    const int ntiles = (rm.M + 15) / 16;
+    const int t0 = (y * 4 + wave) * tiles_per_wave, t1 = min(ntiles, t0 + tiles_per_wave);
+    const float* Wg = W + (size_t)g * w_gstride;
+    float4 bias4 = f4zero();
+    if (bias != nullptr) bias4 = ld4(bias + (size_t)g * C + 4 * j);
+    float4 cs[4];
+#pragma unroll
+    for (int q = 0; q < 4; ++q) cs[q] = f4zero();
+    float4 an[4], on[4];
+    auto fetch = [&](int t) {
+        const int m = min(t * 16 + j, rm.M - 1);
+        const size_t off = ((size_t)g * rm.rs_g + (size_t)m * rm.rs_m) * C + 4 * kk;
+#pragma unroll
+        for (int q = 0; q < 4; ++q) {
+            an[q] = ld4(A + off + 16 * q);
+            if (PRO == PRO_DPRE) on[q] = ld4(A2 + off + 16 * q);
+        }
+    };
+    if (t0 < t1) fetch(t0);
+    load_w_lds<C, 256>(Wl, Wg, transw, threadIdx.x);
+    __syncthreads();
+    float4 bv[4][4];
+#pragma unroll
+    for (int q = 0; q < 4; ++q)
+#pragma unroll
+        for (int e = 0; e < 4; ++e) bv[q][e] = ld4(Wl + (16 * q + 4 * kk + e) * C + 4 * j);
+    for (int t = t0; t < t1; ++t) {
+        float4 a[4];
+        const bool rowok = t * 16 + j < rm.M;
+#pragma unroll
+        for (int q = 0; q < 4; ++q) {
+            float4 v = an[q];
+            if (PRO == PRO_DPRE) {
+                v.x *= lrelu_grad_from_out(on[q].x); v.y *= lrelu_grad_from_out(on[q].y);
+                v.z *= lrelu_grad_from_out(on[q].z); v.w *= lrelu_grad_from_out(on[q].w);
+            }
+            if (!rowok) v = f4zero();
+            a[q] = v;
+            cs[q] = f4add(cs[q], v);
+        }
+        float4 rv[4], rv2[4];
+        size_t orow[4];
+#pragma unroll
+        for (int r = 0; r < 4; ++r) {
+            const int m = min(t * 16 + kk * 4 + r, rm.M - 1);
+            orow[r] = ((size_t)g * rm.rs_g + (size_t)m * rm.rs_m) * C + 4 * j;
+            if (EPI == EPI_RES_LRELU || EPI == EPI_ADD_DPRE) rv[r] = ld4(resid + orow[r]);
+            if (EPI == EPI_ADD_DPRE) rv2[r] = ld4(resid2 + orow[r]);
+        }
+        if (t + 1 < t1) fetch(t + 1);
+        SB();
+        f32x4 acc[4];
+#pragma unroll
+        for (int ct = 0; ct < 4; ++ct) acc[ct] = (f32x4){0.f, 0.f, 0.f, 0.f};
+#pragma unroll
+        for (int q = 0; q < 4; ++q) {
+            const float av[4] = {a[q].x, a[q].y, a[q].z, a[q].w};
+#pragma unroll
+            for (int e = 0; e < 4; ++e) {
+                acc[0] = __builtin_amdgcn_mfma_f32_16x16x4f32(av[e], bv[q][e].x, acc[0], 0, 0, 0);
+                acc[1] = __builtin_amdgcn_mfma_f32_16x16x4f32(av[e], bv[q][e].y, acc[1], 0, 0, 0);
+                acc[2] = __builtin_amdgcn_mfma_f32_16x16x4f32(av[e], bv[q][e].z, acc[2], 0, 0, 0);
+                acc[3] = __builtin_amdgcn_mfma_f32_16x16x4f32(av[e], bv[q][e].w, acc[3], 0, 0, 0);
+            }
+        }
+        SB();
+#pragma unroll
+        for (int r = 0; r < 4; ++r) {
+            if (t * 16 + kk * 4 + r < rm.M) {
+                float4 yv = f4add(make_float4(acc[0][r], acc[1][r], acc[2][r], acc[3][r]), bias4);
+                if (EPI == EPI_RES_LRELU) {
+                    yv = f4add(yv, rv[r]);
+                    yv.x = lrelu(yv.x); yv.y = lrelu(yv.y); yv.z = lrelu(yv.z); yv.w = lrelu(yv.w);
+                }
+                if (EPI == EPI_LRELU) { yv.x = lrelu(yv.x); yv.y = lrelu(yv.y); yv.z = lrelu(yv.z); yv.w = lrelu(yv.w); }
+                if (EPI == EPI_ADD_DPRE) {
+                    const float4 d = rv[r], o = rv2[r];
+                    yv.x = fmaf(d.x, lrelu_grad_from_out(o.x), yv.x); yv.y = fmaf(d.y, lrelu_grad_from_out(o.y), yv.y);
+                    yv.z = fmaf(d.z, lrelu_grad_from_out(o.z), yv.z); yv.w = fmaf(d.w, lrelu_grad_from_out(o.w), yv.w);
+                }
+                if (PUB) {
+                    const __amdgpu_buffer_rsrc_t rs = __builtin_amdgcn_make_buffer_rsrc(out, 0, (int)((size_t)rm.G * rm.M * C * 4), 0x00020000);
+                    st4_sc1(rs, (int)(orow[r] * 4), yv);
+                } else {
+                    st4(out + orow[r], yv);
+                }
+            }
+        }
+    }
+    if (colsum != nullptr) {
+#pragma unroll
+        for (int q = 0; q < 4; ++q) {
+            cs[q].x = group_sum<16>(cs[q].x); cs[q].y = group_sum<16>(cs[q].y);
+            cs[q].z = group_sum<16>(cs[q].z); cs[q].w = group_sum<16>(cs[q].w);
+            if (j == 0) st4(&csl[wave][16 * q + 4 * kk], cs[q]);
+        }
+        __syncthreads();
+        if (wave == 0) colsum[((size_t)y * rm.G + g) * C + lane] = (csl[0][lane] + csl[1][lane]) + (csl[2][lane] + csl[3][lane]);
+    }
+}
diff --git a/gpt-st_amd/csrc/hypertem.hip b/gpt-st_amd/csrc/hypertem.hip
--- a/gpt-st_amd/csrc/hypertem.hip
+++ b/gpt-st_amd/csrc/hypertem.hip
@@ -1,8 +1,19 @@
 #include "mfma_tile.h"
 #include "wgrad64.h"
 #include "kl_guest.h"
+#include "apply64_dev.h"
 GPTST_STAMP_TABLES(hypertem)
 GPTST_HANDOFF_COUNTER(hypertem)
+GPTST_HANDOFF_COUNTER(nodechain)
+#ifdef GPTST_STAMPS
+__device__ long long g_st_nc_wait[2048];
+extern "C" __attribute__((visibility("default"))) int gptst_stamps_nodechain_wait(long long* out) {
+    return hipMemcpyFromSymbol(out, HIP_SYMBOL(g_st_nc_wait), sizeof(long long) * 2048) == hipSuccess ? 0 : 1;
+}
+#define NC_STAMP_WAIT() do { if (blockIdx.x < 2048) g_st_nc_wait[blockIdx.x] = wall_clock64(); } while (0)
+#else
+#define NC_STAMP_WAIT() do { } while (0)
+#endif
 
 #define HT_T 12
 #ifndef HT_OCC
@@ -557,20 +568,14 @@
 #ifndef HTC_NW
 #define HTC_NW 4
 #endif
-template <int NSTAGE, int GUEST>
-__global__ __launch_bounds__(64 * HTC_NW, HTC_NW == 6 ? 3 : HT_OCC) void hypertem_chain_fwd_kernel(HtChain ch, int N, int B, KlGuest kg) {
+template <int NSTAGE, bool NODE>
+__device__ __forceinline__ void hypertem_chain_body(const HtChain& ch, int N, int B, int b, int tile, float* __restrict__ smem,
+                                                    const unsigned* cnt0, const unsigned* cnt1, unsigned want) {
     constexpr int C = 64, P = C + 4, GP = 145, NT = 16, NW = HTC_NW, NTH = 64 * NW, TPW = HT_T / NW;
     static_assert(HT_T % NW == 0 && (HT_T * NT * (C / 4)) % NTH == 0 && (NT * 144) % NTH == 0, "waves must divide the steps and the staging loops");
     constexpr int GK = NT * 144 / NTH, XK = HT_T * NT * (C / 4) / NTH;
-    extern __shared__ __attribute__((aligned(16))) float smem[];
     float* Xs = smem;
     float* Gs = Xs + HT_T * NT * P;
-    if constexpr (GUEST != 0) {
-        static_assert(NTH == 256, "the guest bodies are written for 256 threads");
-        if ((int)blockIdx.x >= kg.base) { kl_guest_run<GUEST>(kg, kg.v0 + (int)blockIdx.x - kg.base, smem); return; }
-    }
-    int b, tile;
-    if (!ht_work((N + NT - 1) / NT, B, b, tile)) return;
     const int n0 = tile * NT;
     const int tid = threadIdx.x, lane = tid & 63, wave = tid >> 6;
     const int j = lane & 15, kk = lane >> 4;
@@ -587,7 +592,33 @@
         b4 = ld4((b0) + ((size_t)b * HT_T + (tt)) * C + 4 * j);                                                    \
     } while (0)
 
-    {
+    if constexpr (NODE) {
+        HTC_LOAD_G(ch.st[0].G);
+        HTC_STORE_G();
+        unsigned* s_ok = reinterpret_cast<unsigned*>(Gs + NT * GP);
+        if (tid == 0) {
+            bool ok = gptst_wait_ge(cnt0, want, &g_handoff_lost_nodechain);
+            if (ok && cnt1 != nullptr) ok = gptst_wait_ge(cnt1, want, &g_handoff_lost_nodechain);
+            *s_ok = ok ? 1u : 0u;
+            NC_STAMP_WAIT();
+        }
+        __syncthreads();
+        const bool ok = *s_ok != 0u;
+        const __amdgpu_buffer_rsrc_t rs = __builtin_amdgcn_make_buffer_rsrc(const_cast<float*>(ch.X) + (size_t)b * HT_T * N * C, 0, HT_T * N * C * 4, 0x00020000);
+        float4 v[XK];
+#pragma unroll
+        for (int k = 0; k < XK; ++k) {
+            const int i = tid + k * NTH, t = i >> 8, nl = (i & 255) >> 4, c4 = i & 15;
+            v[k] = ld4_sc1(rs, ((t * N + min(n0 + nl, N - 1)) * C + 4 * c4) * 4);
+        }
+        const float bad = __int_as_float(0x7fc00000);
+#pragma unroll
+        for (int k = 0; k < XK; ++k) {
+            const int i = tid + k * NTH, t = i >> 8, nl = (i & 255) >> 4, c4 = i & 15;
+            if (!ok) v[k] = make_float4(bad, bad, bad, bad);
+            st4(Xs + (t * NT + nl) * P + 4 * c4, n0 + nl < N ? v[k] : f4zero());
+        }
+    } else {
         float4 v[XK];
 #pragma unroll
         for (int k = 0; k < XK; ++k) {
@@ -737,6 +768,52 @@
 #undef HTC_LOAD_W
 }
 
+template <int NSTAGE, int GUEST>
+__global__ __launch_bounds__(64 * HTC_NW, HTC_NW == 6 ? 3 : HT_OCC) void hypertem_chain_fwd_kernel(HtChain ch, int N, int B, KlGuest kg) {
+    extern __shared__ __attribute__((aligned(16))) float smem[];
+    if constexpr (GUEST != 0) {
+        static_assert(64 * HTC_NW == 256, "the guest bodies are written for 256 threads");
+        if ((int)blockIdx.x >= kg.base) { kl_guest_run<GUEST>(kg, kg.v0 + (int)blockIdx.x - kg.base, smem); return; }
+    }
+    int b, tile;
+    if (!ht_work((N + 15) / 16, B, b, tile)) return;
+    hypertem_chain_body<NSTAGE, false>(ch, N, B, b, tile, smem, nullptr, nullptr, 0u);
+}
+
+struct NodeRole {
+    const float* A; const float* W; const float* bias; const float* resid; float* out;
+    unsigned* cnt;
+    RowMap rm; int tpw, gy, nP;
+};
+
+template <int NSTAGE, int GUEST>
+__global__ __launch_bounds__(256, HT_OCC) void node_chain_fwd_kernel(NodeRole nr, HtChain ch, int N, int B, KlGuest kg) {
+    static_assert(HTC_NW == 4, "both roles are written for 256 threads");
+    extern __shared__ __attribute__((aligned(16))) float smem[];
+    const int L = blockIdx.x, ntl = (N + 15) / 16;
+    if (L < nr.nP) {
+        const int g = L % nr.rm.G, y = L / nr.rm.G;
+        GPTST_WG_BEGIN();
+        apply64_body<PRO_NONE, EPI_RES_LRELU, true>(nr.A, nullptr, nr.W, (long)64 * 64, 0, nr.bias, nr.resid, nullptr, nr.out, nullptr, nr.rm, nr.tpw, g, y, smem);
+        asm volatile("s_waitcnt vmcnt(0)" ::: "memory");
+        __syncthreads();
+        if (threadIdx.x == 0) { gptst_publish_fence(); __hip_atomic_fetch_add(nr.cnt + y * ntl + g / 16, 1u, __ATOMIC_RELAXED, __HIP_MEMORY_SCOPE_AGENT); }
+        GPTST_WG_END();
+        return;
+    }
+    if constexpr (GUEST != 0) {
+        if (L >= kg.base) { kl_guest_run<GUEST>(kg, kg.v0 + L - kg.base, smem); return; }
+    }
+    const int r = L - nr.nP, xcd = L & 7, slot = r >> 3;
+    const int b = xcd + 8 * (slot / ntl), tile = slot % ntl;
+    if (b >= B) return;
+    const int rps = 64 * nr.tpw, y0 = (HT_T * b) / rps, y1 = (HT_T * b + HT_T - 1) / rps;
+    const unsigned want = (unsigned)min(16, N - 16 * tile);
+    GPTST_WG_BEGIN();
+    hypertem_chain_body<NSTAGE, true>(ch, N, B, b, tile, smem, nr.cnt + y0 * ntl + tile, y1 != y0 ? nr.cnt + y1 * ntl + tile : nullptr, want);
+    GPTST_WG_END();
+}
+
 static int ht_chain_args(HtChain& ch, const float* X, int nstage, const void* Gs, const void* Wbts, const void* bbts, const void* Rs, const void* outs,
                          int B, int T, int N, int C) {
     if (!X || nstage < 1 || nstage > 3 || !Gs || !Wbts || !bbts || !Rs || !outs || T != HT_T || B <= 0 || N <= 0) return GPTST_EARG;
@@ -785,12 +862,33 @@
     return GPTST_EARG;
 }
 
+static int ht_guest_args(KlGuest& kg, int base, int nstage, int stage, const void* ops, int v0, int v1, int HS, int lda, float w, int B, int T, int N);
+
 extern "C" int gptst_hypertem_chain_fwd_kl(const float* X, int nstage, const void* Gs, const void* Wbts, const void* bbts, const void* Rs,
                                            const void* outs, int B, int T, int N, int C, int stage, const void* ops, int v0, int v1, int HS,
                                            int lda, float w, void* stream) {
     HtChain ch;
     const int rc = ht_chain_args(ch, X, nstage, Gs, Wbts, bbts, Rs, outs, B, T, N, C);
     if (rc != GPTST_OK) return rc;
+    KlGuest kg{};
+    const int rg = ht_guest_args(kg, ht_chain_grid(B, N), nstage, stage, ops, v0, v1, HS, lda, w, B, T, N);
+    if (rg != GPTST_OK) return rg;
+    const dim3 grid(kg.base + (v1 - v0));
+    const size_t sg = kl_guest_lds_bytes(stage), sh = ht_smem(16);
+    const int smem = (int)(sg > sh ? sg : sh);
+    hipStream_t st = (hipStream_t)stream;
+#define HTC_LAUNCH(G_) do {                                                                                                           \
+        static int done_ = 0;                                                                                                          \
+        if (!done_) { (void)hipFuncSetAttribute((const void*)hypertem_chain_fwd_kernel<2, G_>, hipFuncAttributeMaxDynamicSharedMemorySize, smem); done_ = 1; } \
+        hipLaunchKernelGGL((hypertem_chain_fwd_kernel<2, G_>), grid, dim3(64 * HTC_NW), smem, st, ch, N, B, kg);                           \
+    } while (0)
+    if (stage == 1) HTC_LAUNCH(1); else if (stage == 2) HTC_LAUNCH(2); else HTC_LAUNCH(3);
+#undef HTC_LAUNCH
+    GPTST_CHECK_LAUNCH();
+    return GPTST_OK;
+}
+
+static int ht_guest_args(KlGuest& kg, int base, int nstage, int stage, const void* ops, int v0, int v1, int HS, int lda, float w, int B, int T, int N) {
     if (!ops || stage < 1 || stage > 3) return GPTST_EARG;
     if (nstage != 2 || HTC_NW != 4 || HS <= 0 || HS > TL_MAXJ) return GPTST_ESHAPE;
     const int nv = gptst_kl_guest_blocks(stage, B, T, N);
@@ -798,8 +896,7 @@
     const float* const* p = (const float* const*)ops;
     const int np = stage == 1 ? 7 : stage == 2 ? 6 : 7;
     for (int i = 0; i < np; ++i) if (!p[i]) return GPTST_EARG;
-    KlGuest kg{};
-    kg.base = ht_chain_grid(B, N);
+    kg.base = base;
     kg.v0 = v0;
     if (stage == 1) {
         TailArgs& t = kg.tail;
@@ -815,17 +912,60 @@
         kg.dPre = p[0]; kg.src = p[1]; kg.lda = lda; kg.w1 = p[2]; kg.b1 = p[3]; kg.Wn = p[4]; kg.dWb = (float*)p[5]; kg.dinp = (float*)p[6];
         kg.BT = B * T; kg.N = N;
     }
-    const dim3 grid(kg.base + (v1 - v0));
-    const size_t sg = kl_guest_lds_bytes(stage), sh = ht_smem(16);
-    const int smem = (int)(sg > sh ? sg : sh);
+    return GPTST_OK;
+}
+
+extern "C" int gptst_node_chain_ok(int B, int T, int N, int C) {
+    return (B > 0 && N > 0 && T == HT_T && C == 64 && HTC_NW == 4 && (size_t)B * T * N * C * 4 < ((size_t)1 << 31)) ? 1 : 0;
+}
+
+extern "C" int gptst_node_chain_geometry(int B, int T, int N, int* out) {
+    if (!out || B <= 0 || T <= 0 || N <= 0) return GPTST_EARG;
+    int tpw;
+    const int gy = gptst_apply_wgrad_geometry(1, B * T, N, &tpw), ntl = (N + 15) / 16;
+    out[0] = tpw; out[1] = gy; out[2] = 64 * tpw; out[3] = ntl; out[4] = gy * ntl; out[5] = N * gy; out[6] = ht_chain_grid(B, N);
+    return GPTST_OK;
+}
+
+static size_t ht_node_smem() { return ht_smem(16) + 16; }
+
+extern "C" int gptst_node_chain_fwd(const float* A, const float* Wn, const float* bn, const float* resid, float* nout, void* cnt, int nstage,
+                                    const void* Gs, const void* Wbts, const void* bbts, const void* Rs, const void* outs, int B, int T, int N, int C,
+                                    int stage, const void* ops, int v0, int v1, int HS, int lda, float w, void* stream) {
+    if (!A || !Wn || !bn || !resid || !nout || !cnt) return GPTST_EARG;
+    HtChain ch;
+    const int rc = ht_chain_args(ch, nout, nstage, Gs, Wbts, bbts, Rs, outs, B, T, N, C);
+    if (rc != GPTST_OK) return rc;
+    if (!gptst_node_chain_ok(B, T, N, C) || nstage > 2) return GPTST_ESHAPE;
+    NodeRole nr{};
+    nr.A = A; nr.W = Wn; nr.bias = bn; nr.resid = resid; nr.out = nout; nr.cnt = (unsigned*)cnt;
+    nr.rm = make_rowmap(1, B * T, N);
+    nr.gy = gptst_apply_wgrad_geometry(1, B * T, N, &nr.tpw);
+    nr.nP = nr.rm.G * nr.gy;
+    KlGuest kg{};
+    int ng = 0;
+    size_t smem_b = ht_node_smem();
+    if (stage != 0) {
+        const int rg = ht_guest_args(kg, nr.nP + ht_chain_grid(B, N), nstage, stage, ops, v0, v1, HS, lda, w, B, T, N);
+        if (rg != GPTST_OK) return rg;
+        ng = v1 - v0;
+        const size_t sg = kl_guest_lds_bytes(stage);
+        if (sg > smem_b) smem_b = sg;
+    }
+    const dim3 grid(nr.nP + ht_chain_grid(B, N) + ng);
+    const int smem = (int)smem_b;
     hipStream_t st = (hipStream_t)stream;
-#define HTC_LAUNCH(G_) do {                                                                                                           \
+#define NC_LAUNCH(NS_, G_) do {                                                                                                        \
         static int done_ = 0;                                                                                                          \
-        if (!done_) { (void)hipFuncSetAttribute((const void*)hypertem_chain_fwd_kernel<2, G_>, hipFuncAttributeMaxDynamicSharedMemorySize, smem); done_ = 1; } \
-        hipLaunchKernelGGL((hypertem_chain_fwd_kernel<2, G_>), grid, dim3(64 * HTC_NW), smem, st, ch, N, B, kg);                           \
+        if (!done_) { (void)hipFuncSetAttribute((const void*)node_chain_fwd_kernel<NS_, G_>, hipFuncAttributeMaxDynamicSharedMemorySize, smem); done_ = 1; } \
+        hipLaunchKernelGGL((node_chain_fwd_kernel<NS_, G_>), grid, dim3(256), smem, st, nr, ch, N, B, kg);                            \
     } while (0)
-    if (stage == 1) HTC_LAUNCH(1); else if (stage == 2) HTC_LAUNCH(2); else HTC_LAUNCH(3);
-#undef HTC_LAUNCH
+    if (nstage == 1) NC_LAUNCH(1, 0);
+    else if (stage == 0) NC_LAUNCH(2, 0);
+    else if (stage == 1) NC_LAUNCH(2, 1);
+    else if (stage == 2) NC_LAUNCH(2, 2);
+    else NC_LAUNCH(2, 3);
+#undef NC_LAUNCH
     GPTST_CHECK_LAUNCH();
     return GPTST_OK;
 }
diff --git a/gpt-st_amd/csrc/loss_adam.hip b/gpt-st_amd/csrc/loss_adam.hip
--- a/gpt-st_amd/csrc/loss_adam.hip
+++ b/gpt-st_amd/csrc/loss_adam.hip
@@ -119,10 +119,11 @@
 __global__ __launch_bounds__(256) void adam_kernel(float* __restrict__ p, const float* __restrict__ g, float* __restrict__ m,
                                                    float* __restrict__ v, long nA, long nB, const float* __restrict__ hyper,
                                                    float* __restrict__ stats, const float* __restrict__ ws, int nws, float* __restrict__ stats_out,
-                                                   const unsigned* __restrict__ lost0, const unsigned* __restrict__ lost1, const unsigned* __restrict__ lost2) {
+                                                   const unsigned* __restrict__ lost0, const unsigned* __restrict__ lost1, const unsigned* __restrict__ lost2,
+                                                   const unsigned* __restrict__ lost3) {
     __shared__ float red[4];
     __shared__ float redB[4];
-    const unsigned nlost = (lost0 != nullptr ? *lost0 : 0u) + (lost1 != nullptr ? *lost1 : 0u) + (lost2 != nullptr ? *lost2 : 0u) +
+    const unsigned nlost = (lost0 != nullptr ? *lost0 : 0u) + (lost1 != nullptr ? *lost1 : 0u) + (lost2 != nullptr ? *lost2 : 0u) + (lost3 != nullptr ? *lost3 : 0u) +
                            ((lost0 != nullptr && stats[5] > 0.f) ? (unsigned)stats[5] : 0u);
     {
         float sA = (int)threadIdx.x < nws ? ws[2 * threadIdx.x] : 0.f, sB = (int)threadIdx.x < nws ? ws[2 * threadIdx.x + 1] : 0.f;
@@ -203,6 +204,7 @@
 GPTST_INTERNAL const unsigned* gptst_handoff_word_capmfma(void);
 GPTST_INTERNAL const unsigned* gptst_handoff_word_hypertem(void);
 GPTST_INTERNAL const unsigned* gptst_handoff_word_masksel(void);
+GPTST_INTERNAL const unsigned* gptst_handoff_word_nodechain(void);
 static int g_handoff_guard = 1;
 extern "C" int gptst_set_handoff_guard(int on) { g_handoff_guard = on ? 1 : 0; return GPTST_OK; }
 
@@ -217,8 +219,10 @@
     static const unsigned* w0 = gptst_handoff_word_capmfma();
     static const unsigned* w1 = gptst_handoff_word_hypertem();
     static const unsigned* w2 = gptst_handoff_word_masksel();
+    static const unsigned* w3 = gptst_handoff_word_nodechain();
     hipLaunchKernelGGL(adam_kernel, dim3(nb), dim3(256), 0, (hipStream_t)stream, p, g, m, v, nA, nB, hyper, stats, (const float*)ws, nbn, stats_out,
-                       g_handoff_guard ? w0 : nullptr, g_handoff_guard ? w1 : nullptr, g_handoff_guard ? w2 : nullptr);
-    GPTST_CHECK_LAUNCH();
-    return GPTST_OK;
-}
+                       g_handoff_guard ? w0 : nullptr, g_handoff_guard ? w1 : nullptr, g_handoff_guard ? w2 : nullptr,
+                       g_handoff_guard ? w3 : nullptr);
+    GPTST_CHECK_LAUNCH();
+    return GPTST_OK;
+}
diff --git a/gpt-st_amd/csrc/tails.hip b/gpt-st_amd/csrc/tails.hip
--- a/gpt-st_amd/csrc/tails.hip
+++ b/gpt-st_amd/csrc/tails.hip
@@ -118,9 +118,10 @@
 
 __global__ __launch_bounds__(256) void stats_fold_kernel(const float* __restrict__ sws, int rows, float* __restrict__ stats,
                                                          const unsigned* __restrict__ lost0, const unsigned* __restrict__ lost1,
-                                                         const unsigned* __restrict__ lost2) {
+                                                         const unsigned* __restrict__ lost2, const unsigned* __restrict__ lost3) {
     __shared__ float red[3][4];
-    if (threadIdx.x == 255) stats[5] = (float)((lost0 != nullptr ? *lost0 : 0u) + (lost1 != nullptr ? *lost1 : 0u) + (lost2 != nullptr ? *lost2 : 0u));
+    if (threadIdx.x == 255) stats[5] = (float)((lost0 != nullptr ? *lost0 : 0u) + (lost1 != nullptr ? *lost1 : 0u) + (lost2 != nullptr ? *lost2 : 0u) +
+                                                (lost3 != nullptr ? *lost3 : 0u));
     float s[3] = {0.f, 0.f, 0.f};
     for (int r = threadIdx.x; r < rows; r += 256) {
         const float4 v = ld4(sws + 4 * (size_t)r);
@@ -150,12 +151,14 @@
 GPTST_INTERNAL const unsigned* gptst_handoff_word_capmfma(void);
 GPTST_INTERNAL const unsigned* gptst_handoff_word_hypertem(void);
 GPTST_INTERNAL const unsigned* gptst_handoff_word_masksel(void);
+GPTST_INTERNAL const unsigned* gptst_handoff_word_nodechain(void);
 extern "C" int gptst_stats_fold(const float* sws, int rows, float* stats, void* stream) {
     if (!sws || !stats || rows <= 0) return GPTST_EARG;
     static const unsigned* w0 = gptst_handoff_word_capmfma();
     static const unsigned* w1 = gptst_handoff_word_hypertem();
     static const unsigned* w2 = gptst_handoff_word_masksel();
-    hipLaunchKernelGGL(stats_fold_kernel, dim3(1), dim3(256), 0, (hipStream_t)stream, sws, rows, stats, w0, w1, w2);
+    static const unsigned* w3 = gptst_handoff_word_nodechain();
+    hipLaunchKernelGGL(stats_fold_kernel, dim3(1), dim3(256), 0, (hipStream_t)stream, sws, rows, stats, w0, w1, w2, w3);
     GPTST_CHECK_LAUNCH();
     return GPTST_OK;
 }
diff --git a/gpt-st_amd/engine.py b/gpt-st_amd/engine.py
--- a/gpt-st_amd/engine.py
+++ b/gpt-st_amd/engine.py
@@ -389,6 +389,31 @@
         saved.append(HtSaved(xin, R.view(-1, C), o, G, Wbt))
         xin = o
     return saved, xin
+
+
+NODE_CHAIN = int(os.environ.get("GPTST_NODE_CHAIN", "0"))
+NODE_CHAIN_MAX_BT = 512
+
+
+def node_chain_on(site, dims):
+    B, T, N, C = dims
+    return bool(site is not None and (NODE_CHAIN >> site) & 1 and chain_fwd_ok(dims) and not CTX.NO_HANDOFFS and CTX.NODE_REDUCE is None
+                and B * T <= NODE_CHAIN_MAX_BT and ops.node_chain_ok(B, T, N, C))
+
+
+def cap_chain_fwd(p, pfx, x, dadj, dyn, Wn, bn, dims, num_route, HS, HT, stages, kl=None, first=False):
+    B, T, N, C = dims
+    rec, c, (s, v, Ht, Rt, Y) = cap_head_fwd(p, pfx, x, dadj, dyn, dims, num_route, HS, HT)
+    if first and kl is not None and kl.c1 is None:
+        kl.c1 = c
+    guest = kl.guest() if kl is not None and len(stages) == 2 else None
+    out, res = ops.node_chain_fwd(rec, Wn, bn, x, stages, dims, guest=guest, cnt=_zeros(x, ops.node_chain_geometry(B, T, N).cnt_words))
+    saved, xin = [], out
+    for (G, Wbt, _b), (R, o) in zip(stages, res):
+        o = o.view(-1, C)
+        saved.append(HtSaved(xin, R.view(-1, C), o, G, Wbt))
+        xin = o
+    return out, c, CapSaved(x, out, rec, c, s, v, Ht, Rt, dyn, Wn, Y), saved, xin
 
 
 def cap_core_bwd(p, g, pfx, saved, dout, dims, HS, HT, red, chain=False):
@@ -582,28 +607,41 @@
     return GenAll(sthcn, gd, jobs if defer else None)
 
 
-def sthcn_fwd(p, pfx, tidx, x, dims, num_route, gen=None, head=None, next_gen=None, kl=None):
+def sthcn_fwd(p, pfx, tidx, x, dims, num_route, gen=None, head=None, next_gen=None, kl=None, sites=None):
     if gen is None:
         gen = gen_all(p, tidx, dims, which=(pfx,), guide=False).sthcn[pfx]
     ht = gen.ht
-    cap = lambda i, x: cap_core_fwd(p, gen.cps[i], x, gen.dadj[i], gen.dyn[i], *gen.Wn[i], dims, num_route, gen.HS, gen.HT)
+    capargs = lambda i, x: (p, gen.cps[i], x, gen.dadj[i], gen.dyn[i], *gen.Wn[i], dims, num_route, gen.HS, gen.HT)
+    cap = lambda i, x: cap_core_fwd(*capargs(i, x))
     pairs = chain_fwd_ok(dims)
+    merged = [node_chain_on(st, dims) for st in (sites or (None, None))]
     nhead = None
     x, h1 = head if head is not None else hypertem_core_fwd(x, *ht(0), dims)
-    x, c1, sc1 = cap(0, x)
-    if pairs:
-        if kl is not None and kl.c1 is None:
-            kl.c1 = c1
-        (h2, h3), x = ht_chain_fwd(x, [ht(1), ht(2)], dims, kl)
-    else:
-        x, h2 = hypertem_core_fwd(x, *ht(1), dims)
-        x, h3 = hypertem_core_fwd(x, *ht(2), dims)
-    x, _, sc2 = cap(1, x)
-    if pairs and next_gen is not None:
-        (h4, h1n), xn = ht_chain_fwd(x, [ht(3), next_gen.ht(0)], dims, kl)
-        x, nhead = h4.out, (xn, h1n)
-    else:
-        x, h4 = hypertem_core_fwd(x, *ht(3), dims)
+    if merged[0]:
+        _, c1, sc1, (h2, h3), x = cap_chain_fwd(*capargs(0, x), [ht(1), ht(2)], kl, first=True)
+    else:
+        x, c1, sc1 = cap(0, x)
+        if pairs:
+            if kl is not None and kl.c1 is None:
+                kl.c1 = c1
+            (h2, h3), x = ht_chain_fwd(x, [ht(1), ht(2)], dims, kl)
+        else:
+            x, h2 = hypertem_core_fwd(x, *ht(1), dims)
+            x, h3 = hypertem_core_fwd(x, *ht(2), dims)
+    join = pairs and next_gen is not None
+    if merged[1]:
+        _, _, sc2, hs, xl = cap_chain_fwd(*capargs(1, x), [ht(3), next_gen.ht(0)] if join else [ht(3)], kl)
+        h4 = hs[0]
+        x = h4.out
+        if join:
+            nhead = (xl, hs[1])
+    else:
+        x, _, sc2 = cap(1, x)
+        if join:
+            (h4, h1n), xn = ht_chain_fwd(x, [ht(3), next_gen.ht(0)], dims, kl)
+            x, nhead = h4.out, (xn, h1n)
+        else:
+            x, h4 = hypertem_core_fwd(x, *ht(3), dims)
     return x, c1, SthcnSaved(h1, h2, h3, h4, sc1, sc2, gen.emb, gen, gen.slot), nhead
 
 
@@ -886,7 +924,7 @@
 
 
 def autoencoder_fwd(p, source, mask, dims, base, num_route, scaler_zeros, gen=None, tidx=None, lowrank_in=False, kl=None, head=True,
-                    decoder=True, join=True):
+                    decoder=True, join=True, node_chain=False):
     B, T, N, C = dims
     if tidx is None:
         tidx = source[:, :, 0, base:base + 2].contiguous()
@@ -901,10 +939,11 @@
     else:
         x0 = ops.lin_in(source, base + 2, base, p["encoder.dim_in_flow.weight"], p["encoder.dim_in_flow.bias"], C,
                         mask=mask, fill=scaler_zeros)
-    emb, c1, sv_e, dec_h1 = sthcn_fwd(p, ENC, tidx, x0, dims, num_route, gen=gen_e, head=first, next_gen=gen_d if join else None, kl=kl)
+    emb, c1, sv_e, dec_h1 = sthcn_fwd(p, ENC, tidx, x0, dims, num_route, gen=gen_e, head=first, next_gen=gen_d if join else None, kl=kl,
+                                         sites=(0, 1) if node_chain else None)
     if not decoder:
         return Forward(emb, c1, None, None, sv_e, None)
-    dec, _, sv_d, _ = sthcn_fwd(p, DEC, tidx, emb, dims, num_route, gen=gen_d, head=dec_h1, kl=kl)
+    dec, _, sv_d, _ = sthcn_fwd(p, DEC, tidx, emb, dims, num_route, gen=gen_d, head=dec_h1, kl=kl, sites=(2, 3) if node_chain else None)
     out = ops.rowdot(dec, p["decoder.dim_flow_out.weight"], p["decoder.dim_flow_out.bias"]) if head else None
     return Forward(emb, c1, dec, out, sv_e, sv_d)
 
diff --git a/gpt-st_amd/ops.py b/gpt-st_amd/ops.py
--- a/gpt-st_amd/ops.py
+++ b/gpt-st_amd/ops.py
@@ -313,6 +313,47 @@
         _call("gptst_hypertem_chain_fwd_kl", *chain, stage, _ptrs0(ts), v0, v1, HS, lda, float(w), tag="x%d+kl%d" % (len(stages), stage),
               nbytes=_nb(X, *Rs, *outs))
     return list(zip(Rs, outs))
+
+
+def node_chain_ok(B, T, N, C):
+    return _C.lib().value("gptst_node_chain_ok", B, T, N, C) == 1
+
+
+class NodeChainGeometry(NamedTuple):
+    tpw: int
+    gy: int
+    rows_per_split: int
+    node_tiles: int
+    cnt_words: int
+    node_wgs: int
+    slab_wgs: int
+
+
+def node_chain_geometry(B, T, N):
+    out = (ctypes.c_int * 7)()
+    _C.lib().call("gptst_node_chain_geometry", B, T, N, out)
+    return NodeChainGeometry(*out)
+
+
+def node_chain_fwd(A, Wn, bn, resid, stages, dims, want_R=True, guest=None, cnt=None):
+    B, T, N, C = dims
+    _chk(A, Wn, bn, resid, *[t for st in stages for t in st])
+    if cnt is None:
+        cnt = torch.zeros(node_chain_geometry(B, T, N).cnt_words, device=A.device, dtype=torch.float32)
+    nout = torch.empty_like(A)
+    f = lambda: torch.empty(B, T, N, C, device=A.device, dtype=torch.float32)
+    Rs = [f() if want_R else None for _ in stages]
+    outs = [f() for _ in stages]
+    chain = (_p(A), _p(Wn), _p(bn), _p(resid), _p(nout), _p(cnt), len(stages), _ptrs0([st[0] for st in stages]),
+             _ptrs0([st[1] for st in stages]), _ptrs0([st[2] for st in stages]), _ptrs0(Rs), _ptrs0(outs), B, T, N, C)
+    nb = _nb(A, Wn, bn, resid, nout, *Rs, *outs)
+    if guest is None:
+        _call("gptst_node_chain_fwd", *chain, 0, None, 0, 0, 0, 0, 0.0, tag="x%d" % len(stages), nbytes=nb)
+    else:
+        stage, ts, v0, v1, HS, lda, w = guest
+        _chk(*ts)
+        _call("gptst_node_chain_fwd", *chain, stage, _ptrs0(ts), v0, v1, HS, lda, float(w), tag="x%d+kl%d" % (len(stages), stage), nbytes=nb)
+    return nout, list(zip(Rs, outs))
 
 
 def kl_guest_blocks(stage, B, T, N):
diff --git a/gpt-st_amd/step.py b/gpt-st_amd/step.py
--- a/gpt-st_amd/step.py
+++ b/gpt-st_amd/step.py
@@ -180,7 +180,8 @@
             sws = self._tail_sws()
             kl = engine.KlCarry(p, sv_g, prob, src, dims, 0.1, sws)
         fw = engine.autoencoder_fwd(p, src, mask, dims, base, mdl.num_route, mdl.scaler_zeros, gen=gen, tidx=tidx,
-                                    lowrank_in=fused and engine.chain_ok(dims), kl=kl, head=not fused, join=self.join_enc_dec)
+                                    lowrank_in=fused and engine.chain_ok(dims), kl=kl, head=not fused, join=self.join_enc_dec,
+                                    node_chain=True)
         if fused and sws is None:
             sws = self._tail_sws()
         engine.step_bwd(p, g, src, mask, tidx, fw, prob, sv_g, dims, base, mdl.scaler_zeros, red, (self.std, self.mean, a.mape_thresh),
diff --git a/include/gptst_hip.h b/include/gptst_hip.h
--- a/include/gptst_hip.h
+++ b/include/gptst_hip.h
@@ -9,7 +9,7 @@
 #pragma GCC visibility push(default)
 #endif
 
-#define GPTST_ABI_VERSION 26
+#define GPTST_ABI_VERSION 27
 int gptst_abi_version(void);
 int gptst_set_deterministic(int on);
 int gptst_deterministic_state(void);
@@ -76,6 +76,11 @@
 int gptst_hypertem_chain_fwd_kl(const float* X, int nstage, const void* Gs, const void* Wbts, const void* bbts, const void* Rs, const void* outs,
                                 int B, int T, int N, int C, int stage, const void* ops, int v0, int v1, int HS, int lda, float w, void* stream);
 int gptst_kl_guest_blocks(int stage, int B, int T, int N);
+int gptst_node_chain_fwd(const float* A, const float* Wn, const float* bn, const float* resid, float* nout, void* cnt, int nstage,
+                         const void* Gs, const void* Wbts, const void* bbts, const void* Rs, const void* outs, int B, int T, int N, int C,
+                         int stage, const void* ops, int v0, int v1, int HS, int lda, float w, void* stream);
+int gptst_node_chain_ok(int B, int T, int N, int C);
+int gptst_node_chain_geometry(int B, int T, int N, int* out);
 
 int gptst_encin_ht1_fwd(const float* src, int lda, const float* mask, float fill, const float* w, const float* bi, const float* G,
                         const float* Wbt, const float* bbt, float* out, float* ab, float* wv, int B, int T, int N, int C, void* stream);
```
